# ducha-aiki/affnet

Hardware: AMD Instinct MI355X
Metric: keypoints/sec (detect+AffNet+OriNet+HardNet) per image, 2000 kp @1024x768 (higher is better)
Workload: dtype f32

## Files before the change

affnet_amd/SparseImgRepresenter.py:

```python
import ctypes as C

import torch
import torch.nn as nn

from . import _lib, engine
from ._lib import lib, check, ptr
from .architectures import _HipPatchNet
from .HandCraftedModules import AffineShapeEstimator, OrientationDetector, _HipHandCrafted
from .HardNet import HardTFeatNet
from .pytorch_sift import SIFTNet

_FOLLOW = (SIFTNet, HardTFeatNet)


class ScaleSpaceAffinePatchExtractor(nn.Module):
    def __init__(self, border=16, num_features=500, patch_size=32, mrSize=3.0, nlevels=3, num_Baum_iters=0,
                 init_sigma=1.6, th=None, RespNet=None, OriNet=None, AffNet=None, arith="fp32"):
        super(ScaleSpaceAffinePatchExtractor, self).__init__()
        self.arith = arith
        _lib.arith_code(arith)
        self.mrSize, self.PS, self.b = mrSize, patch_size, border
        self.num, self.nlevels = num_features, nlevels
        self.num_Baum_iters, self.init_sigma = num_Baum_iters, init_sigma
        self.th = th
        if th is not None:
            self.num = -1
        else:
            self.th = 0
        self.RespNet = RespNet
        if not 1 <= nlevels <= 6:
            raise NotImplementedError("nlevels must be 1..6 (levels per octave = nlevels + 2 <= 8)")
        self.OriNet = OriNet if OriNet is not None else OrientationDetector(patch_size=19)
        self.AffNet = AffNet if AffNet is not None else AffineShapeEstimator(patch_size=19)
        self.scale_pyr = self.sigmas = self.pix_dists = None
        self._ctx = None
        self._ctx_key = None
        self._fctx = self._fctx_key = self._pyr_ctx = None
        self.last_ids = None
        self.max_keep = 16384
        self.raw_div = 4
        self.lazy_shape_rows = -1
        self.shape_form = 1

        self.desc_form = 2

    def _context(self, x, allow_batch=False):
        engine.require_cuda(x, "image")
        if x.dim() != 4 or x.size(1) != 1 or x.size(0) < 1 or (x.size(0) != 1 and not allow_batch):
            raise ValueError("expected a (1,1,H,W) image; forward() is batch-size-1 like the reference "
                             "(HandCraftedModules.py:283-284) - use enqueue()/run_batch() for (B,1,H,W) batches")
        pre = int(1.5 * self.num) if self.num_Baum_iters > 0 else self.num
        key = (x.size(0), x.size(2), x.size(3), x.device, pre, self.num, float(self.th), self.mrSize, self.b, self.init_sigma,
               self.nlevels, self.max_keep, self.num_Baum_iters, self.raw_div, self.lazy_shape_rows)
        if self._ctx is not None and self._ctx_key == key and self._ctx.arith != _lib.arith_code(self.arith):
            self._ctx.set_arith(self.arith)
        if self._ctx is None or self._ctx_key != key:
            self._ctx = engine.Context(x.size(2), x.size(3), x.device, self.nlevels, self.init_sigma, self.b, self.mrSize,
                                       float(self.th), self.num, pre, self.max_keep, batch=x.size(0), baum_iters=self.num_Baum_iters, raw_div=self.raw_div,
                                       lazy_shape_rows=self.lazy_shape_rows, arith=self.arith)
            self._ctx_key = key
        if self._ctx.shape_form != int(self.shape_form):
            self._ctx.set_shape_form(self.shape_form)
        if self._ctx.desc_form != int(self.desc_form):
            self._ctx.set_desc_form(self.desc_form)
        return self._ctx

    def _publish_pyramid(self, ctx):
        self._pyr_ctx = ctx
        self.scale_pyr = ctx.pyramid_views()
        self.sigmas = [list(s) for s in ctx.plan.sigmas]
        self.pix_dists = [list(p) for p in ctx.plan.pix_dists]

    def _response_pyramid(self, ctx, img):
        dev = img.device
        st = engine.stream_of(dev)
        check(lib.affnet_pyramid_build(ctx.handle, ptr(img), st), ctx.handle, "affnet_pyramid_build")
        stride = lib.affnet_pyramid_image_stride(ctx.handle)
        base = lib.affnet_pyramid_level_offset(ctx.handle, 0, 0)
        resp = torch.zeros(ctx.batch * stride, dtype=torch.float32, device=dev)
        with torch.no_grad():
            for b in range(ctx.batch):
                pyr = ctx.pyramid_views(b)
                for o, (h, w) in enumerate(ctx.plan.sizes):
                    for l in range(ctx.plan.levels_per_octave):
                        off = b * stride + lib.affnet_pyramid_level_offset(ctx.handle, o, l) - base
                        r = self.RespNet(pyr[o][l], ctx.plan.sigmas[o][l])
                        resp[off:off + h * w].copy_(r.reshape(-1).to(dev, torch.float32))
        return resp

    @staticmethod
    def _native(slot):
        return slot is None or isinstance(slot, (_HipPatchNet, _HipHandCrafted))

    def enqueue(self, x, do_ori=False, desc=None, det_stream=None, input_ready=None):
        ctx = self._context(x, allow_batch=True)
        dev = x.device
        if not (self._native(self.AffNet) and self._native(self.OriNet)):
            raise NotImplementedError("the fused path needs the native AffNetFast / OriNetFast slots (foreign slots: forward())")
        img = x.contiguous().float()
        B, F = x.size(0), ctx.cap_final
        lafs = torch.empty(B, F, 2, 3, dtype=torch.float32, device=dev)
        resp = torch.empty(B, F, dtype=torch.float32, device=dev)
        ids = torch.empty(B, F, 3, dtype=torch.int32, device=dev)
        count = torch.zeros(B, dtype=torch.int32, device=dev)
        dsc = torch.empty(B, F, 128, dtype=torch.float32, device=dev) if desc is not None else None
        nets = self._nets(dev, do_ori, desc)
        follow = isinstance(desc, _FOLLOW)
        if isinstance(desc, HardTFeatNet):
            desc.check_usable()
        fused_dsc = None if follow else dsc
        if self.RespNet is not None:
            rmaps = self._response_pyramid(ctx, img)
            check(lib.affnet_detect_image_responses(ctx.handle, ptr(rmaps), engine.stream_of(dev)), ctx.handle, "affnet_detect_image_responses")
            rc = lib.affnet_describe_detected(ctx.handle, C.byref(nets), int(bool(do_ori)), ptr(lafs), ptr(resp), ptr(ids), ptr(fused_dsc),
                                              ptr(count), engine.stream_of(dev))
            check(rc, ctx.handle, "affnet_describe_detected")
        elif det_stream is None:
            rc = lib.affnet_extract_features(ctx.handle, C.byref(nets), ptr(img), int(bool(do_ori)), ptr(lafs), ptr(resp), ptr(ids),
                                             ptr(fused_dsc), ptr(count), engine.stream_of(dev))
            check(rc, ctx.handle, "affnet_extract_features")
        else:
            cur = torch.cuda.current_stream(dev)
            if input_ready is None:
                det_stream.wait_stream(cur)
            elif input_ready is not False:
                det_stream.wait_event(input_ready)
            if getattr(self, "_busy", None) is not None:
# ... 374 lines not shown
```

affnet_amd/_lib.py:

```python
import ctypes as C
import os

_HERE = os.path.dirname(os.path.abspath(__file__))
LIB_PATH = os.environ.get("AFFNET_HIP_LIB") or os.path.join(_HERE, "libaffnet_hip.so")
PROBES_LIB_PATH = os.path.join(_HERE, "libaffnet_hip_probes.so")

MAX_OCTAVES, MAX_LEVELS, MAX_TAPS = 16, 8, 37
NET_AFFNET, NET_ORINET, NET_HARDNET, NET_AFFNET_FULLCONV = 0, 1, 2, 3
ARITH_FP32_MFMA, ARITH_FP32_SPLIT3, ARITH_FP32_SPLIT2H = 0, 1, 2
ARITH_NAMES = {"fp32": ARITH_FP32_MFMA, "fp32_mfma": ARITH_FP32_MFMA, "fp32_split3": ARITH_FP32_SPLIT3, "split3": ARITH_FP32_SPLIT3,
               "fp32_split2h": ARITH_FP32_SPLIT2H, "split2h": ARITH_FP32_SPLIT2H}


def arith_code(arith):
    if arith is None:
        return ARITH_FP32_MFMA
    if isinstance(arith, str):
        if arith.lower() not in ARITH_NAMES:
            raise ValueError("arith must be one of %s" % sorted(ARITH_NAMES))
        return ARITH_NAMES[arith.lower()]
    if int(arith) not in (ARITH_FP32_MFMA, ARITH_FP32_SPLIT3, ARITH_FP32_SPLIT2H):
        raise ValueError("arith must be AFFNET_ARITH_FP32_MFMA (0), AFFNET_ARITH_FP32_SPLIT3 (1) or AFFNET_ARITH_FP32_SPLIT2H (2)")
    return int(arith)
SHAPE_FORM_DIRECT, SHAPE_FORM_WINOGRAD, SHAPE_FORM_POLYPHASE = 0, 1, 2
DESC_FORM_DIRECT, DESC_FORM_POLYPHASE, DESC_FORM_F43 = 0, 1, 2
OK, ERR_INVALID, ERR_HIP, ERR_CAPACITY, ERR_EMPTY = 0, -1, -2, -3, -4
VERIFY_AFFINE, VERIFY_HOMOGRAPHY, VERIFY_TILE, VERIFY_CHUNK = 0, 1, 128, 128
KNN_MAX_K = 8
IVF_MAX_PROBE = 8
EPI_MAX_ROUNDS, EPI_TILE, EPI_CHUNK, EPI_SOLVE_TILE = 64, 128, 128, 64
GUIDED_PLANAR, GUIDED_EPIPOLAR, GUIDED_MUTUAL = 0, 1, 1
VERIFY_FLAG_PAIR_RANGE = 8


class Config(C.Structure):
    _fields_ = [
        ("height", C.c_int32), ("width", C.c_int32), ("n_octaves", C.c_int32), ("levels_per_octave", C.c_int32),
        ("oct_h", C.c_int32 * MAX_OCTAVES), ("oct_w", C.c_int32 * MAX_OCTAVES),
        ("level_sigma", (C.c_float * MAX_LEVELS) * MAX_OCTAVES),
        ("level_sigma4", (C.c_float * MAX_LEVELS) * MAX_OCTAVES),
        ("level_sigma_px", (C.c_double * MAX_LEVELS) * MAX_OCTAVES),
        ("first_blur_taps", C.c_int32), ("first_blur", C.c_float * (MAX_TAPS * MAX_TAPS)),
        ("level_blur_taps", C.c_int32 * MAX_LEVELS),
        ("level_blur", (C.c_float * (MAX_TAPS * MAX_TAPS)) * MAX_LEVELS),
        ("level_blur0_taps", C.c_int32 * MAX_LEVELS),
        ("level_blur0", (C.c_float * (MAX_TAPS * MAX_TAPS)) * MAX_LEVELS),
        ("lazy_shape_rows", C.c_int32),
        ("onepass", C.c_int32),
        ("mr_size", C.c_float), ("threshold", C.c_float),
        ("num_features", C.c_int32), ("num_prefilter", C.c_int32),
        ("max_raw_per_octave_div", C.c_int32), ("max_keep", C.c_int32), ("batch", C.c_int32), ("baum_iters", C.c_int32),
        ("arith", C.c_int32),
    ]


class Nets(C.Structure):
    _fields_ = [("d_affnet", C.c_void_p), ("d_orinet", C.c_void_p), ("d_hardnet", C.c_void_p),
                ("h_orientation_window", C.c_void_p), ("h_baumberg_window", C.c_void_p)]


_P, _I, _SZ = C.c_void_p, C.c_int, C.c_size_t
SYMBOLS = {
    "affnet_config_fill": (_I, [C.POINTER(Config), _I, _I, _I, C.c_double, _I, C.c_double, C.c_double, _I, _I, _I, _I]),
    "affnet_ctx_create": (_I, [C.POINTER(_P), _I, C.POINTER(Config)]),
    "affnet_ctx_destroy": (None, [_P]),
    "affnet_last_error": (C.c_char_p, [_P]),
    "affnet_version": (C.c_char_p, []),
    "affnet_set_arith": (_I, [_P, _I]),
    "affnet_get_arith": (_I, [_P]),
    "affnet_set_shape_form": (_I, [_P, _I]),
    "affnet_get_shape_form": (_I, [_P]),
    "affnet_set_desc_form": (_I, [_P, _I]),
    "affnet_get_desc_form": (_I, [_P]),
    "affnet_workspace_bytes": (_SZ, [_P]),
    "affnet_bind_workspace": (_I, [_P, _P, _SZ]),
    "affnet_pyramid_level_offset": (C.c_int64, [_P, _I, _I]),
    "affnet_pyramid_image_stride": (C.c_int64, [_P]),
    "affnet_batch": (_I, [_P]),
    "affnet_capacity_prefilter": (_I, [_P]),
    "affnet_capacity_final": (_I, [_P]),
    "affnet_gauss_blur": (_I, [_P, _P, _P, _I, _I, C.POINTER(C.c_float), _I, _P]),
    "affnet_pyramid_build": (_I, [_P, _P, _P]),
    "affnet_hessian_response": (_I, [_P, _P, _P, _I, _I, C.c_float, _P]),
    "affnet_detect": (_I, [_P, _P, _P, _P, _P, _P]),
    "affnet_detect_responses": (_I, [_P, _P, _P, _P, _P, _P, _P]),
    "affnet_laf_grid_sample": (_I, [_P, _P, _I, _I, _P, _I, _I, _P, _P]),
    "affnet_pyr_grid_sample": (_I, [_P, _P, _P, _P, _I, _I, _P, _P]),
    "affnet_cnn32_packed_floats": (_SZ, [_I]),
    "affnet_cnn32_winograd_offset": (C.c_int64, [_I, _I]),
    "affnet_cnn32_pack_weights": (_I, [_I, C.POINTER(_P), C.POINTER(_P), C.POINTER(_P), _P, _P, _P, _P, _P]),
    "affnet_cnn32_forward": (_I, [_P, _I, _P, _P, _P, _I, _P, _P, _P]),
    "affnet_cnn32_forward_pyr": (_I, [_P, _I, _P, _P, _P, _P, _I, _P, _P, _P]),
    "affnet_local_norm": (_I, [_P, _P, _P, _I, _I, _P]),
    "affnet_fullconv_scratch_bytes": (_SZ, [_I, _I]),
    "affnet_fullconv_forward": (_I, [_P, _P, _P, _I, _I, _P, _P, _P]),
    "affnet_nms2d": (_I, [_P, _P, _P, _I, _I, C.c_float, _P]),
    "affnet_shape_filter_select": (_I, [_P, _P, _P, _P, _P, _P, _P, _P, _P, _P, _P]),
    "affnet_apply_rotation": (_I, [_P, _P, _P, _P, _I, _P]),
    "affnet_scale_lafs": (_I, [_P, _P, _P, _P, _I, _I, _I, _I, _P]),
    "affnet_lafs_to_ellipses": (_I, [_P, _P, _P, _I, _P, _P]),
    "affnet_ellipses_to_lafs": (_I, [_P, _P, _P, _I, _P, _P]),
    "affnet_level_select": (_I, [_P, _P, _P, _I, _I, _P, _P, _P]),
    "affnet_handcrafted_forward": (_I, [_P, _I, _P, _I, _P, _P, _P, _P]),
    "affnet_handcrafted_forward_pyr": (_I, [_P, _I, _P, _P, _P, _I, _P, _P, _P]),
    "affnet_sift_host_window": (_I, [_I, C.POINTER(C.c_float)]),
    "affnet_sift_forward": (_I, [_P, _P, _I, _P, C.c_float, _P, _P]),
    "affnet_sift_forward_pyr": (_I, [_P, _P, _P, _P, _I, _P, C.c_float, _P, _P]),
    "affnet_tfeat_packed_floats": (_SZ, []),
    "affnet_tfeat_pack_weights": (_I, [_P, _P, _P, _P, _P, _P, _P]),
    "affnet_tfeat_scratch_floats": (_SZ, [_I]),
    "affnet_tfeat_forward": (_I, [_P, _P, _P, _P, _I, _P, _P, _P]),
    "affnet_tfeat_forward_pyr": (_I, [_P, _P, _P, _P, _P, _I, _P, _P, _P]),
    "affnet_match_scratch_bytes": (_SZ, [_I, _I]),
    "affnet_distance_matrix": (_I, [_P, _P, _I, _P, _I, _I, _P, _P, _P]),
    "affnet_match_snn": (_I, [_P, _P, _I, _P, _I, _I, C.c_float, _P, _P, _P, _P, _P, _P, _P]),
    "affnet_reproject_lafs": (_I, [_P, _P, _I, C.POINTER(C.c_float), _P, _P]),
    "affnet_centre_nn": (_I, [_P, _P, _I, _P, _I, _P, _P, _P]),
    "affnet_verify_scratch_bytes": (_SZ, [_I]),
    "affnet_verify_score": (_I, [_P, _P, _I, _P, _I, _P, _P, _I, C.c_float, _P, _P, _P, _P]),
    "affnet_verify_matches": (_I, [_P, _P, _I, _P, _I, _P, _P, _I, C.c_float, _I, _I, _P, _P, _P, _P, _P, _P]),
    "affnet_match_many_scratch_bytes": (_SZ, [_I, _I, _I]),
    "affnet_match_snn_many": (_I, [_P, _P, _I, _P, _I, _I, _P, _I, _I, _I, C.c_float, _P, _P, _P, _P, _P, _P, _P]),
    "affnet_verify_many_scratch_bytes": (_SZ, [_I, _I]),
    "affnet_verify_matches_many": (_I, [_P, _P, _I, _P, _I, _P, _I, _P, _P, _I, C.c_float, _I, _I, _P, _P, _P, _P, _P, _P]),
    "affnet_epipolar_scratch_bytes": (_SZ, [_I, _I]),
    "affnet_epipolar_score": (_I, [_P, _P, _I, _P, _I, _P, _P, _I, C.c_float, _I, C.c_uint32, _P, _P, _P, _P, _P]),
    "affnet_epipolar_verify": (_I, [_P, _P, _I, _P, _I, _P, _P, _I, C.c_float, _I, C.c_uint32, _I, _P, _P, _P, _P, _P, _P]),
    "affnet_match_guided_scratch_bytes": (_SZ, [_I, _I, _I]),
    "affnet_match_guided": (_I, [_P, _P, _I, _P, _I, _I, _P, _P, _P, _I, C.c_float, C.c_float, C.c_float, _I, _I, _P, _P, _P, _P, _P, _P, _P]),
    "affnet_guided_mask": (_I, [_P, _P, _I, _P, _I, _P, _I, C.c_float, _P, _P, _P]),
    "affnet_knn_chunks": (_I, [_P, _I, _I]),
    "affnet_knn_scratch_bytes": (_SZ, [_I, _I, _I, _I]),
    "affnet_knn": (_I, [_P, _P, _I, _P, _I, _I, _I, _I, _I, _I, _P, _P, _P, _P]),
    "affnet_knn_vote": (_I, [_P, _P, _P, _I, _I, C.c_float, _P, _I, _I, _P, _P]),
    "affnet_quantize_desc": (_I, [_P, _P, _I, _I, C.c_float, _P, _P, _P]),
    "affnet_knn_q8_chunks": (_I, [_P, _I, _I]),
    "affnet_knn_q8_scratch_bytes": (_SZ, [_I, _I, _I, _I]),
    "affnet_knn_q8": (_I, [_P, _P, _P, _I, _P, _P, _I, _I, _I, _I, _I, _I, C.c_float, _P, _P, _P, _P, _P]),
    "affnet_ivf_sqnorm": (_I, [_P, _P, _I, _I, _P, _P]),
    "affnet_ivf_cell_means": (_I, [_P, _P, _I, _I, _P, _P, _I, _P, _P]),
    "affnet_ivf_scratch_bytes": (_SZ, [_I, _I, _I, _I]),
    "affnet_ivf_search": (_I, [_P, _P, _I, _P, _P, _P, _I, _P, _P, _I, _I, _I, _I, _I, _I, _P, _P, _P, _P, _P]),
    "affnet_ivf_q8_scratch_bytes": (_SZ, [_I, _I, _I, _I]),
    "affnet_ivf_search_q8": (_I, [_P, _P, _P, _P, _I, _P, _P, _P, _I, _P, _P, _I, _I, _I, _I, _I, _I, C.c_float, _P, _P, _P, _P, _P, _P]),
    "affnet_extract_features": (_I, [_P, C.POINTER(Nets), _P, _I, _P, _P, _P, _P, _P, _P]),
    "affnet_detect_image": (_I, [_P, _P, _P]),
    "affnet_detect_image_responses": (_I, [_P, _P, _P]),
    "affnet_detect_image_onepass": (_I, [_P, _P, _P, _P]),
    "affnet_detect_image_onepass_responses": (_I, [_P, _P, _P, _P]),
    "affnet_detected_list": (_I, [_P, _P, _P, _P, _P, _P]),
    "affnet_load_frames": (_I, [_P, _P, _I, _P, _P, _P, _I, _I, _P]),
    "affnet_describe_frames": (_I, [_P, C.POINTER(Nets), _P, _P, _P, _P, _I, _I, _P, _P, _P, _P, _P, _P]),
    "affnet_shape_iterate": (_I, [_P, _P, _P, _P, _P, _I, _P, _P]),
    "affnet_affmap_offset": (C.c_int64, [_P, _I]),
    "affnet_affmap_image_stride": (C.c_int64, [_P]),
    "affnet_describe_detected": (_I, [_P, C.POINTER(Nets), _I, _P, _P, _P, _P, _P, _P]),
    "affnet_graph_capture_extract": (_I, [_P, C.POINTER(Nets), _P, _I, _P, _P, _P, _P, _P, _P]),
    "affnet_graph_launch": (_I, [_P, _P]),
    "affnet_profile_enable": (_I, [_P, _I]),
    "affnet_profile_read": (_I, [_P, C.POINTER(C.c_double * 8), C.POINTER(C.c_int32)]),
    "affnet_read_counts": (_I, [_P, C.POINTER(C.c_int32 * 4), _P]),
    "affnet_counter_offset": (C.c_int64, [_P, _I]),
    "affnet_counter_stride": (C.c_int64, [_P]),
    "affnet_host_base_grid": (_I, [_I, C.POINTER(C.c_float)]),
}

DEBUG_SYMBOLS = {
    "affnet_cnn32_debug_timing": (_I, [_P, _P]),
    "affnet_cnn32_debug_layer": (_I, [_P, _I, _P, _P, _I, _P, _P]),
    "affnet_cnn32_debug_winograd_u": (_I, [_P, _I, _P, _I, _P, _P]),
    "affnet_selftest_mfma": (_I, [_P, _P, _P, _P]),
    "affnet_debug_split3_variant": (_I, [_P, _I]),
}

PROBE_SYMBOLS = {
    "affnet_cnn32_probe": (_I, [_P, _I, _I, _I, _I, _P, _P]),
    "affnet_split3_gemm": (_I, [_P, _P, _I, _I, _I, _I, _P, _P]),
    "affnet_split3_rate": (_I, [_I, _I, _I, _P, _P]),
    "affnet_debug_stream": (_I, [_P, _P, _SZ, _I, _I, _I, _P]),
    "affnet_probe_shape_offsets": (_I, [_P, C.POINTER(C.c_int64 * 3)]),
    "affnet_probe_affnet_wino_layer": (_I, [_P, _I, _P, _P, _I, _P, _P]),
    "affnet_probe_affnet_wino_partials": (_I, [_P, _P, _P, _I, _P, _P]),
    "affnet_probe_affnet_poly_layer": (_I, [_P, _I, _P, _P, _I, _P, _P]),
    "affnet_probe_affnet_poly_partials": (_I, [_P, _P, _P, _I, _P, _P]),
    "affnet_probe_trunk16_poly_u": (_I, [_P, _I, _P, _I, _P, _P]),
    "affnet_probe_hardnet_poly_layer": (_I, [_P, _P, _P, _I, _P, _P]),
    "affnet_probe_hardnet_poly_forward": (_I, [_P, _P, _P, _I, _P, _P, _P]),
    "affnet_probe_hardnet_poly_u": (_I, [_P, _P, _I, _P, _P]),
    "affnet_probe_hardnet_f43_layer": (_I, [_P, _P, _P, _I, _P, _P]),
    "affnet_probe_hardnet_f43_forward": (_I, [_P, _P, _P, _I, _P, _P, _P]),
    "affnet_probe_hardnet_f43_u": (_I, [_P, _P, _I, _P, _P]),
}


class AffnetHipError(RuntimeError):
    pass


class AffnetEmptyError(AffnetHipError):
    """AFFNET_ERR_EMPTY: no image of the call produced a detection (the reference raises in torch.cat([]),
    SparseImgRepresenter.py:100)."""


def _load():
    if not os.path.isfile(LIB_PATH):
        if os.path.basename(LIB_PATH) == os.path.basename(PROBES_LIB_PATH):
            raise ImportError("affnet_amd: %s is missing - the tools under tools/ need the probe build of the library: "
                              "AFFNET_PROBES=1 bash affnet_amd/csrc/build.sh" % LIB_PATH)
        raise ImportError(
            "affnet_amd: %s is missing - the HIP extension is the only implementation of this path "
            "(no CPU fallback). Build it: bash affnet_amd/csrc/build.sh" % LIB_PATH)
    lib = C.CDLL(LIB_PATH)
    for table in (SYMBOLS, DEBUG_SYMBOLS):
        for name, (res, args) in table.items():
            fn = getattr(lib, name)
            fn.restype, fn.argtypes = res, args
    for name, (res, args) in PROBE_SYMBOLS.items():
        if hasattr(lib, name):
            fn = getattr(lib, name)
            fn.restype, fn.argtypes = res, args
    return lib


lib = _load()


def check(rc, ctx=None, what=""):
    if rc != OK:
        msg = lib.affnet_last_error(ctx).decode() if ctx else ""
        if rc == ERR_EMPTY:
            raise AffnetEmptyError("%s: %s" % (what or "libaffnet_hip call", msg))
        raise AffnetHipError("%s failed (code %d): %s" % (what or "libaffnet_hip call", rc, msg))


def ptr(t):
    return None if t is None else C.c_void_p(t.data_ptr())


def current_stream(device):
    import torch
    return C.c_void_p(torch.cuda.current_stream(device).cuda_stream)
```

affnet_amd/csrc/cnn32.hip:

```cpp
#include "common.h"

static void aff_fill_pyr_src(const affnet_ctx* ctx, PyrSrc* s) {
    memset(s, 0, sizeof(*s));
    if (ctx->ws) aff_fill_pyr_table(ctx, &s->t);
    aff_base_grid(32, s->base);
}

static int cnn_check(affnet_ctx* ctx, const CnnCall& c, int* rows) {
    *rows = 0;
    if (c.kind < 0 || c.kind > 2) return aff_fail(ctx, AFFNET_ERR_INVALID, "cnn32: unknown net kind %d", c.kind);
    if (!c.packed || !c.out || c.n_max < 0 || (!c.patches && (!c.lafs || !c.ids))) return aff_fail(ctx, AFFNET_ERR_INVALID, "cnn32: null argument");
    if (!c.patches && !ctx->ws) return aff_fail(ctx, AFFNET_ERR_INVALID, "cnn32: sampling from the pyramid needs a bound workspace");
    if (c.dbg_layer < 0 && !c.scratch)
        return aff_fail(ctx, AFFNET_ERR_INVALID, "cnn32: d_scratch is required (HardNet n*(8192+512) floats, AffNet / OriNet n*144 floats)");
    if (c.dbg_layer >= 0 && ctx->arith != AFFNET_ARITH_FP32_MFMA)
        return aff_fail(ctx, AFFNET_ERR_INVALID, "cnn32: layer dumps exist for AFFNET_ARITH_FP32_MFMA only (context is in arithmetic mode %d)", ctx->arith);
    if (c.n_max == 0) return AFFNET_OK;
    if (c.kind == AFFNET_NET_HARDNET && c.n_max > 65535)
        return aff_fail(ctx, AFFNET_ERR_INVALID, "cnn32: n_max=%d (HardNet head: max 65535 rows per image)", c.n_max);
    const int row_count = c.row_count < 0 ? c.n_max - c.row_begin : c.row_count;
    if (c.row_begin < 0 || row_count < 0 || c.row_begin + row_count > c.n_max) return aff_fail(ctx, AFFNET_ERR_INVALID, "cnn32: bad row window");
    *rows = row_count;
    return AFFNET_OK;
}

TrunkKernel aff_trunk_kernel(int kind, int form, bool stamps) {
    typedef TrunkKernel (*Unit)(int, bool);
    static_assert(AFFNET_NET_AFFNET == 0 && AFFNET_NET_ORINET == 1 && AFFNET_NET_HARDNET == 2 && TRUNK_EXACT == 0 && TRUNK_WINO == 1 && TRUNK_SPLIT2 == 2 && TRUNK_SPLIT3 == 3 &&
                  TRUNK_WINO_F43 == 4 && TRUNK_WINO_POLY == 5 && TRUNK_FORMS == 6, "order of the table");
    static const Unit unit[3][TRUNK_FORMS] = {{aff_trunk_affnet, aff_trunk_affnet, aff_trunk_affnet, aff_trunk_affnet, nullptr, aff_trunk_affnet_poly},
                                              {aff_trunk_orinet, nullptr, aff_trunk_orinet, aff_trunk_orinet, nullptr, nullptr},
                                              {aff_trunk_hardnet, aff_trunk_hardnet_poly, aff_trunk_hardnet, aff_trunk_hardnet, aff_trunk_hardnet_f43, nullptr}};
    if (kind < 0 || kind > 2 || form < 0 || form >= TRUNK_FORMS || !unit[kind][form]) return nullptr;
    return unit[kind][form](form, stamps);
}

int aff_trunk_launch(affnet_ctx* ctx, const CnnCall& c, const NetLayout& L, dim3 grid, int wino, const int32_t* reeval, int shape_op) {
    int form = TRUNK_EXACT;
    if (ctx->arith != AFFNET_ARITH_FP32_MFMA) form = ctx->arith == AFFNET_ARITH_FP32_SPLIT2H ? TRUNK_SPLIT2 : TRUNK_SPLIT3;
    else if (c.kind == AFFNET_NET_AFFNET && wino) form = wino == 2 ? TRUNK_WINO_POLY : TRUNK_WINO;
    else if (c.kind == AFFNET_NET_HARDNET && c.desc_form != AFFNET_DESC_FORM_DIRECT) form = c.desc_form == AFFNET_DESC_FORM_F43 ? TRUNK_WINO_F43 : TRUNK_WINO;
    const bool stamps = ctx->dbg_time || c.dbg_layer >= 0;
    const TrunkKernel kernel = aff_trunk_kernel(c.kind, form, stamps);
    if (!kernel) return aff_fail(ctx, AFFNET_ERR_INVALID, "cnn32: no trunk kernel of net %d in form %d is built", c.kind, form);
    CnnArgs a;
    a.packed = c.packed; a.off = to_offsets(L, ctx->arith);
    a.reeval = reeval;
    const int rc = aff_derive_u(ctx, c.kind, form, c.packed, L, c.st, &a.wino_u);
    if (rc) return rc;
    a.patches = c.patches; a.lafs = c.lafs; a.ids = c.ids; a.count = c.count; a.n_max = c.n_max;
    a.out = (c.dbg_layer < 0) ? c.scratch : c.out;
    a.dbg_layer = c.dbg_layer; a.dbg_out = c.dbg_out; a.dbg_time = ctx->dbg_time;
    a.row_begin = c.row_begin; a.skip_cnt = c.skip_cnt; a.skip_n = c.skip_n;
    a.shape_cnt = (c.fuse && shape_op) ? c.fuse->cnt : nullptr; a.shape_op = shape_op;
    a.s3_alt = ctx->split3_variant;
    PyrSrc ps;
    aff_fill_pyr_src(ctx, &ps);
    hipLaunchKernelGGL(kernel, grid, dim3(512), 0, c.st, a, ps);
    AFF_LAUNCH_CHECK(ctx);
    return AFFNET_OK;
}

static int cnn_launch(affnet_ctx* ctx, const CnnCall& c) {
    int rows;
    int rc = cnn_check(ctx, c, &rows);
    if (rc || rows == 0) return rc;
    const NetLayout L = net_layout(c.kind);
    const int B = c.patches ? 1 : ctx->B;
    const bool form1 = c.wino_reeval && c.kind == AFFNET_NET_AFFNET && c.fuse && c.dbg_layer < 0 && ctx->arith == AFFNET_ARITH_FP32_MFMA;
    rc = aff_trunk_launch(ctx, c, L, dim3(rows, B), form1 ? c.wino_reeval : 0, nullptr, c.shape_op);
    if (rc) return rc;
    if (form1) {
        int32_t* flags = reinterpret_cast<int32_t*>(c.scratch + (size_t)B * c.n_max * HEAD_PART_AFF);
        rc = aff_margin_affnet(ctx, c, L, rows, B, flags);
        if (rc) return rc;
        rc = aff_trunk_launch(ctx, c, L, dim3(rows, B), 0, flags, 0);
        if (rc) return rc;
    }
    if (c.dbg_layer < 0 && c.kind != AFFNET_NET_HARDNET) {
        rc = c.kind == AFFNET_NET_AFFNET ? aff_finish_affnet(ctx, c, L, rows, B) : aff_finish_orinet(ctx, c, L, rows, B);
        if (rc) return rc;
    }
    if (c.mark_head) aff_prof_mark(ctx, 7, c.st);
    if (c.dbg_layer < 0 && c.kind == AFFNET_NET_HARDNET) return aff_hardnet_head(ctx, c, L, B);
    return AFFNET_OK;
}

extern "C" int affnet_cnn32_forward(affnet_ctx* ctx, int net_kind, const float* d_packed, const float* d_patches, const int32_t* d_count,
                                    int n_max, float* d_out, float* d_scratch, void* stream) {
    AFF_DEVICE(ctx);
    if (!ctx || !d_patches) return aff_fail(ctx, AFFNET_ERR_INVALID, "cnn32_forward: null argument");
    CnnCall c;
    c.kind = net_kind; c.packed = d_packed; c.patches = d_patches; c.count = d_count; c.n_max = n_max; c.out = d_out; c.scratch = d_scratch; c.st = (hipStream_t)stream;
    return cnn_launch(ctx, c);
}

extern "C" int affnet_cnn32_forward_pyr(affnet_ctx* ctx, int net_kind, const float* d_packed, const float* d_lafs, const int32_t* d_ids,
                                        const int32_t* d_count, int n_max, float* d_out, float* d_scratch, void* stream) {
    AFF_DEVICE(ctx);
    if (!ctx) return AFFNET_ERR_INVALID;
    CnnCall c;
    c.kind = net_kind; c.packed = d_packed; c.lafs = d_lafs; c.ids = d_ids; c.count = d_count; c.n_max = n_max; c.out = d_out; c.scratch = d_scratch; c.st = (hipStream_t)stream;
    return cnn_launch(ctx, c);
}

int aff_affnet_filter_rows(affnet_ctx* ctx, const float* packed, const float* resp, const float* lafs, const int32_t* ids, const int32_t* count,
                           float* out, float* scratch, int row_begin, int row_count, bool lazy, int shape_op, hipStream_t st) {
    ShapeFuse sf;
    sf.resp = resp; sf.lafs = lafs; sf.key = ctx->st_key; sf.good = ctx->st_good; sf.cnt = ctx->cnt;
    CnnCall c;
    c.kind = AFFNET_NET_AFFNET; c.packed = packed; c.lafs = lafs; c.ids = ids; c.count = count; c.n_max = ctx->cap_pre; c.out = out; c.scratch = scratch; c.st = st;
    c.row_begin = row_begin; c.row_count = row_count;
    c.skip_cnt = lazy ? ctx->cnt : nullptr; c.skip_n = ctx->cfg.num_features;
    c.fuse = &sf; c.shape_op = shape_op;
    c.wino_reeval = ctx->shape_form;
    return cnn_launch(ctx, c);
}

int aff_orinet_rotate(affnet_ctx* ctx, const float* packed, float* lafs, const int32_t* ids, const int32_t* count, int n_max, float* out, float* scratch,
                      hipStream_t st, const DenormSel* denorm) {
    CnnCall c;
    c.kind = AFFNET_NET_ORINET; c.packed = packed; c.lafs = lafs; c.ids = ids; c.count = count; c.n_max = n_max; c.out = out; c.scratch = scratch; c.st = st;
    c.rot_lafs = lafs; c.denorm = denorm;
    return cnn_launch(ctx, c);
}

int aff_hardnet_forward_pyr_marked(affnet_ctx* ctx, const float* packed, const float* lafs, const int32_t* ids, const int32_t* count,
                                   int n_max, float* out, float* scratch, hipStream_t st) {
    CnnCall c;
    c.kind = AFFNET_NET_HARDNET; c.packed = packed; c.lafs = lafs; c.ids = ids; c.count = count; c.n_max = n_max; c.out = out; c.scratch = scratch; c.st = st;
    c.mark_head = true;
    c.desc_form = ctx->cfg.onepass ? AFFNET_DESC_FORM_DIRECT : ctx->desc_form;
    return cnn_launch(ctx, c);
}

int aff_hardnet_poly_patches(affnet_ctx* ctx, const float* packed, const float* patches, int n, float* out, float* scratch, int dbg_layer, hipStream_t st, int form) {
    if (ctx->arith != AFFNET_ARITH_FP32_MFMA) return aff_fail(ctx, AFFNET_ERR_INVALID, "hardnet_poly: AFFNET_ARITH_FP32_MFMA only");
    CnnCall c;
    c.kind = AFFNET_NET_HARDNET; c.packed = packed; c.patches = patches; c.n_max = n; c.out = out; c.scratch = scratch; c.st = st;
    c.dbg_layer = dbg_layer; c.dbg_out = dbg_layer >= 0 ? out : nullptr;
    c.desc_form = form;
    return cnn_launch(ctx, c);
}

extern "C" int affnet_debug_split3_variant(affnet_ctx* ctx, int bits) {
    if (!ctx) return AFFNET_ERR_INVALID;
    ctx->split3_variant = bits;
    return AFFNET_OK;
}

extern "C" int affnet_cnn32_debug_timing(affnet_ctx* ctx, unsigned long long* d_stamps) {
    if (!ctx) return AFFNET_ERR_INVALID;
    ctx->dbg_time = d_stamps;
    return AFFNET_OK;
}

extern "C" int affnet_cnn32_debug_layer(affnet_ctx* ctx, int net_kind, const float* d_packed, const float* d_patch, int layer, float* d_out,
                                        void* stream) {
    AFF_DEVICE(ctx);
    if (!ctx || !d_patch || !d_out || layer < 0 || layer > 5) return aff_fail(ctx, AFFNET_ERR_INVALID, "cnn32_debug_layer: bad argument");
    CnnCall c;
    c.kind = net_kind; c.packed = d_packed; c.patches = d_patch; c.n_max = 1; c.out = d_out; c.st = (hipStream_t)stream;
    c.dbg_layer = layer; c.dbg_out = d_out;
    return cnn_launch(ctx, c);
}

extern "C" int affnet_cnn32_debug_winograd_u(affnet_ctx* ctx, int net_kind, const float* d_packed, int layer, float* d_out, void* stream) {
    AFF_DEVICE(ctx);
    if (!ctx || !d_packed || !d_out || (net_kind != AFFNET_NET_AFFNET && net_kind != AFFNET_NET_ORINET) || (layer != 1 && layer != 3 && layer != 5))
        return aff_fail(ctx, AFFNET_ERR_INVALID, "cnn32_debug_winograd_u: AffNet / OriNet, layer 1, 3 or 5");
    const float* u;
    const int rc = aff_derive_u(ctx, net_kind, net_kind == AFFNET_NET_AFFNET ? TRUNK_WINO : TRUNK_EXACT, d_packed, net_layout(net_kind), (hipStream_t)stream, &u);
    if (rc) return rc;
    return aff_copy_async(ctx, d_out, u + Wino16::offset(layer), (size_t)Wino16::floats(layer) * sizeof(float), (hipStream_t)stream);
}
```

affnet_amd/csrc/cnn_mfma.h:

```cpp
#pragma once
#include <math.h>
#include <stdlib.h>

#include <utility>

#include "common.h"
#include "weights_layout.h"

typedef float f32x4 __attribute__((ext_vector_type(4)));

typedef __attribute__((address_space(3))) const f32x4 LdsF4;
__device__ __forceinline__ unsigned lds_byte_addr(const float* p) {
    return (unsigned)(size_t)(__attribute__((address_space(3))) const float*)p;
}
__device__ __forceinline__ f32x4 lds_read4(unsigned byte_addr) { return *(LdsF4*)(size_t)byte_addr; }

typedef unsigned u32x4 __attribute__((ext_vector_type(4)));
__device__ __forceinline__ __amdgpu_buffer_rsrc_t weight_rsrc(const float* base, int n_floats) {
    return __builtin_amdgcn_make_buffer_rsrc(const_cast<float*>(base), 0, n_floats * 4, 0x00020000);
}
__device__ __forceinline__ f32x4 buf_read4(__amdgpu_buffer_rsrc_t r, int lane_byte_off, int uniform_byte_off) {
    return __builtin_bit_cast(f32x4, __builtin_amdgcn_raw_buffer_load_b128(r, lane_byte_off, uniform_byte_off, 0));
}

// ... 1126 lines not shown
    }
    __syncthreads();
#pragma unroll
    for (int k = 0; k < 18; ++k) *reinterpret_cast<f32x4*>(&act[((p * F43_XI + 18 * h + k) * 64 + lane) * 4]) = V[k];
    __syncthreads();
    const unsigned v0 = lds_byte_addr(act) + (18 * h * 64 + lane) * 16;
#pragma unroll
    for (int k = 0; k < 18; ++k) V[k] = lds_read4(v0 + k * 1024);
    f32x4 acc[18];
#pragma unroll
    for (int k = 0; k < 18; ++k) acc[k] = (f32x4){0.f, 0.f, 0.f, 0.f};
#pragma unroll 1
    for (int G = 0; G < NGRP; ++G) {
        const int Gn = G == NGRP - 1 ? G : G + 1;
        unsigned vb = v0 + Gn * F43_XI * 1024;
        asm("" : "+v"(vb));
        __builtin_amdgcn_sched_barrier(0);
#pragma unroll
        for (int k = 0; k < 18; k += 2) {
#pragma unroll
            for (int s4 = 0; s4 < 4; ++s4) {
                acc[k] = __builtin_amdgcn_mfma_f32_16x16x4f32(U[k][s4], V[k][s4], acc[k], 0, 0, 0);
                acc[k + 1] = __builtin_amdgcn_mfma_f32_16x16x4f32(U[k + 1][s4], V[k + 1][s4], acc[k + 1], 0, 0, 0);
            }
            U[k] = wino_load_u<CIN, COUT>(wrsrc, u_lane, k, Gn);
            U[k + 1] = wino_load_u<CIN, COUT>(wrsrc, u_lane, k + 1, Gn);
            V[k] = lds_read4(vb + k * 1024);
            V[k + 1] = lds_read4(vb + (k + 1) * 1024);
            __builtin_amdgcn_sched_barrier(0);
        }
    }
#pragma unroll
    for (int il = 0; il < 3; ++il)
#pragma unroll
        for (int e = 0; e < 4; ++e) {
            float yc[4];
            f43_at_axis(acc[6 * il][e], acc[6 * il + 1][e], acc[6 * il + 2][e], acc[6 * il + 3][e], acc[6 * il + 4][e], acc[6 * il + 5][e], yc[0], yc[1], yc[2], yc[3]);
#pragma unroll
            for (int c = 0; c < 4; ++c) t[il][c][e] = yc[c];
        }
}

__device__ __forceinline__ void f43_combine(float* lds, const f32x4 (&t)[3][4], f32x4 (&y)[8], int wave, int lane) {
    const int h = wave & 1;
    float* xw = lds + F43L::X + (wave * 8 * 64 + lane) * 4;
    const float* xr = lds + F43L::X + ((wave ^ 1) * 8 * 64 + lane) * 4;
    f32x4 k0[4], k1[4];
    if (h == 0) {
#pragma unroll
        for (int c = 0; c < 4; ++c) {
            const f32x4 p = t[1][c] + t[2][c], q = t[1][c] - t[2][c];
            k0[c] = t[0][c] + p; k1[c] = q;
            *reinterpret_cast<f32x4*>(&xw[c * 256]) = p;
            *reinterpret_cast<f32x4*>(&xw[(4 + c) * 256]) = q;
        }
    } else {
#pragma unroll
        for (int c = 0; c < 4; ++c) {
            const f32x4 r = t[0][c] + t[1][c], s = t[0][c] - t[1][c];
            k0[c] = 4.0f * r; k1[c] = 8.0f * s + t[2][c];
            *reinterpret_cast<f32x4*>(&xw[c * 256]) = r;
            *reinterpret_cast<f32x4*>(&xw[(4 + c) * 256]) = 2.0f * s;
        }
    }
    __syncthreads();
#pragma unroll
    for (int c = 0; c < 4; ++c) {
        const f32x4 o0 = *reinterpret_cast<const f32x4*>(&xr[c * 256]), o1 = *reinterpret_cast<const f32x4*>(&xr[(4 + c) * 256]);
        y[c] = k0[c] + o0;
        y[4 + c] = k1[c] + o1;
    }
}

template <typename LO>
__device__ __forceinline__ void f43_store_lds(float* act, f32x4 bias, const f32x4 (&y)[8], int wave, int lane) {
    const int m = lane & 15, oy = 4 * (m >> 2) + 2 * (wave & 1), ox = 4 * (m & 3);
#pragma unroll
    for (int k = 0; k < 8; ++k) {
        const f32x4 v = bias_relu(y[k], bias);
        *reinterpret_cast<f32x4*>(&act[((wave >> 1) * 4 + (lane >> 4)) * LO::PSG + ((oy + (k >> 2) + 1) * LO::WP + ox + (k & 3) + 1) * 4]) = v;
    }
}

template <int NW, int CIN, int COUT, int H, int NB>
__device__ __forceinline__ void wino_prefetch_u_row(const float* __restrict__ Wu, f32x4 (&U)[4], int wave, int lane) {
    const __amdgpu_buffer_rsrc_t r = weight_rsrc(Wu, 16 * CIN * COUT);
    const int u_lane = wino_u_lane<H, COUT, NB>(wave, 0, lane);
#pragma unroll
    for (int k = 0; k < 4; ++k) U[k] = wino_load_u<CIN, COUT>(r, u_lane, k, 0);
}

template <int NW, int CIN, int COUT, typename LI, int NB>
__device__ __forceinline__ void conv3x3_wino_mfma_rows(const float* act, const float* __restrict__ Wu, f32x4 (&U)[4], f32x4 (&y)[NB][4], int wave, int lane) {
    constexpr int H = LI::H, HT = H / 2, NGRP = CIN / 16, NSTEP = NB * 4 * NGRP;
    static_assert(H % 2 == 0 && (HT * HT) % 16 == 0 && COUT % 16 == 0 && CIN % 16 == 0, "Winograd tiling");
    static_assert((HT * HT / 16) * (COUT / 16) == NW * NB, "the waves' passes must tile the layer exactly");
    const int m = lane & 15, kq = lane >> 4;
    const __amdgpu_buffer_rsrc_t wrsrc = weight_rsrc(Wu, 16 * CIN * COUT);
    f32x4 t0[4], t1[4], acc[4];
#pragma unroll
    for (int s = 0; s < NSTEP; ++s) {
        const int q = s / (4 * NGRP), i = (s / NGRP) % 4, G = s % NGRP;
        const int sn = s + 1 < NSTEP ? s + 1 : s;
        const int qn = sn / (4 * NGRP), in = (sn / NGRP) % 4, Gn = sn % NGRP;
        int ty, tx, cb;
        wino_tile<H, COUT, NB>(wave, q, m, ty, tx, cb);
        const int u_next = wino_u_lane<H, COUT, NB>(wave, qn, lane);
        unsigned ab = lds_byte_addr(act) + (((4 * G + kq) * LI::PSG + (2 * ty * LI::WP + 2 * tx) * 4) * 4);
        asm("" : "+v"(ab));
        f32x4 da[4], db[4], V[4];
        wino_read_rows<LI>(ab, i, da, db);
        wino_transform_row(i, da, db, V);
        if (G == 0) {
#pragma unroll
            for (int k = 0; k < 4; ++k) acc[k] = (f32x4){0.f, 0.f, 0.f, 0.f};
        }
        __builtin_amdgcn_sched_barrier(0);
#pragma unroll
        for (int k = 0; k < 4; k += 2) {
#pragma unroll
            for (int s4 = 0; s4 < 4; ++s4) {
                acc[k] = __builtin_amdgcn_mfma_f32_16x16x4f32(U[k][s4], V[k][s4], acc[k], 0, 0, 0);
                acc[k + 1] = __builtin_amdgcn_mfma_f32_16x16x4f32(U[k + 1][s4], V[k + 1][s4], acc[k + 1], 0, 0, 0);
            }
            U[k] = wino_load_u<CIN, COUT>(wrsrc, u_next, 4 * in + k, Gn);
            U[k + 1] = wino_load_u<CIN, COUT>(wrsrc, u_next, 4 * in + k + 1, Gn);
            __builtin_amdgcn_sched_barrier(0);
        }
        if (G == NGRP - 1) {
#pragma unroll
            for (int j = 0; j < 4; ++j)
#pragma unroll
                for (int e = 0; e < 4; ++e) {
                    if (i == 0) t0[j][e] = acc[j][e];
                    else if (i == 1) { t0[j][e] = wadd(t0[j][e], acc[j][e]); t1[j][e] = acc[j][e]; }
                    else if (i == 2) { t0[j][e] = wadd(t0[j][e], acc[j][e]); t1[j][e] = wsub(t1[j][e], acc[j][e]); }
                    else t1[j][e] = wsub(t1[j][e], acc[j][e]);
                }
            if (i == 3) {
#pragma unroll
                for (int e = 0; e < 4; ++e) {
                    y[q][0][e] = wadd(wadd(t0[0][e], t0[1][e]), t0[2][e]);
                    y[q][1][e] = wsub(wsub(t0[1][e], t0[2][e]), t0[3][e]);
                    y[q][2][e] = wadd(wadd(t1[0][e], t1[1][e]), t1[2][e]);
                    y[q][3][e] = wsub(wsub(t1[1][e], t1[2][e]), t1[3][e]);
                }
            }
        }
    }
}

struct Wino5 {
    static constexpr int X = 16 * LayC4::PSG, X_FLOATS = 8 * 4 * 256;
    static constexpr int HEAD = 0;
    static constexpr int U_HALF = 8 * 4 * 16 * 64 * 4;
};
__device__ __forceinline__ void wino5_prefetch_u(const float* __restrict__ Wu, f32x4 (&U)[4], int wave, int lane) {
    const __amdgpu_buffer_rsrc_t r = weight_rsrc(Wu, 16 * 64 * 64);
    const int u_lane = ((lane >> 4) * 64 + (wave >> 1) * 16 + (lane & 15)) * 16 + (wave & 1) * Wino5::U_HALF;
#pragma unroll
    for (int k = 0; k < 4; ++k) U[k] = wino_load_u<64, 64>(r, u_lane, k, 0);
}

template <int NW, typename LI>
__device__ __forceinline__ void conv3x3_wino_mfma_half_rows(const float* act, const float* __restrict__ Wu, f32x4 (&U)[4], f32x4 (&acc)[2][4], int wave, int lane) {
    constexpr int CIN = 64, COUT = 64, NGRP = CIN / 16, NSTEP = 2 * NGRP;
// ... 36 lines not shown
}

__device__ __forceinline__ void wino5_combine(float* lds, const f32x4 (&acc)[2][4], f32x4 (&y)[2], int wave, int lane) {
    const int h = wave & 1;
    float* xw = lds + Wino5::X + (wave * 4 * 64 + lane) * 4;
    const float* xr = lds + Wino5::X + ((wave ^ 1) * 4 * 64 + lane) * 4;
    if (h == 0) {
#pragma unroll
        for (int j = 0; j < 4; ++j) *reinterpret_cast<f32x4*>(&xw[j * 256]) = acc[1][j];
    } else {
#pragma unroll
        for (int j = 0; j < 4; ++j) *reinterpret_cast<f32x4*>(&xw[j * 256]) = acc[0][j];
    }
    __syncthreads();
    f32x4 o[4], t[4];
#pragma unroll
    for (int j = 0; j < 4; ++j) o[j] = *reinterpret_cast<const f32x4*>(&xr[j * 256]);
    if (h == 0) {
#pragma unroll
        for (int j = 0; j < 4; ++j)
#pragma unroll
            for (int e = 0; e < 4; ++e) t[j][e] = wadd(wadd(acc[0][j][e], acc[1][j][e]), o[j][e]);
    } else {
#pragma unroll
        for (int j = 0; j < 4; ++j)
#pragma unroll
            for (int e = 0; e < 4; ++e) t[j][e] = wsub(wsub(o[j][e], acc[0][j][e]), acc[1][j][e]);
    }
#pragma unroll
    for (int e = 0; e < 4; ++e) {
        y[0][e] = wadd(wadd(t[0][e], t[1][e]), t[2][e]);
        y[1][e] = wsub(wsub(t[1][e], t[2][e]), t[3][e]);
    }
}

template <int ROW, int PIX, int GRP>
__device__ __forceinline__ void wino5_store_lds(float* dst, f32x4 bias, const f32x4 (&y)[2], int wave, int lane) {
    const int m = lane & 15, oy = 2 * (m >> 2) + (wave & 1), ox = 2 * (m & 3);
#pragma unroll
    for (int k = 0; k < 2; ++k) {
        const f32x4 v = bias_relu(y[k], bias);
        *reinterpret_cast<f32x4*>(&dst[(oy * ROW + ox + k) * PIX + ((wave >> 1) * 4 + (lane >> 4)) * GRP]) = v;
    }
}

template <int NW, int H, int COUT, int NB>
__device__ __forceinline__ void wino_bias(const float* __restrict__ bias, f32x4 (&bv)[NB], int wave, int lane) {
#pragma unroll
    for (int q = 0; q < NB; ++q) {
        int ty, tx, cb;
        wino_tile<H, COUT, NB>(wave, q, lane & 15, ty, tx, cb);
        bv[q] = *reinterpret_cast<const f32x4*>(&bias[cb * 16 + 4 * (lane >> 4)]);
    }
}

template <int COUT, typename LO, int NB>
__device__ __forceinline__ void wino_store_lds(float* act, const f32x4 (&bias)[NB], const f32x4 (&y)[NB][4], int wave, int lane) {
    const int g = lane >> 4;
#pragma unroll
    for (int q = 0; q < NB; ++q) {
        int ty, tx, cb;
        wino_tile<LO::H, COUT, NB>(wave, q, lane & 15, ty, tx, cb);
#pragma unroll
        for (int k = 0; k < 4; ++k) {
            const int oy = 2 * ty + (k >> 1), ox = 2 * tx + (k & 1);
            const f32x4 v = bias_relu(y[q][k], bias[q]);
            *reinterpret_cast<f32x4*>(&act[(cb * 4 + g) * LO::PSG + ((oy + 1) * LO::WP + ox + 1) * 4]) = v;
        }
    }
}

template <int COUT, int H, int NB>
__device__ __forceinline__ void wino_store_global(float* __restrict__ dst, const f32x4 (&bias)[NB], const f32x4 (&y)[NB][4], int wave, int lane) {
    const int g = lane >> 4;
#pragma unroll
    for (int q = 0; q < NB; ++q) {
        int ty, tx, cb;
        wino_tile<H, COUT, NB>(wave, q, lane & 15, ty, tx, cb);
#pragma unroll
        for (int k = 0; k < 4; ++k) {
            const int p = (2 * ty + (k >> 1)) * H + 2 * tx + (k & 1);
            const f32x4 v = bias_relu(y[q][k], bias[q]);
            *reinterpret_cast<f32x4*>(dst + p * COUT + cb * 16 + 4 * g) = v;
        }
    }
}

constexpr int poly_row_np(int r) { return (r < 3 || (r >= 6 && r < 8)) ? 3 : 2; }
constexpr int poly_row_xi0(int r) { return r < 3 ? 3 * r : (r < 6 ? 9 + 2 * (r - 3) : (r < 8 ? 15 + 3 * (r - 6) : 21 + 2 * (r - 8))); }
constexpr bool poly_row_oddy(int r) { return r < 6; }
constexpr int poly_row_yi(int r) { return r < 3 ? r : (r < 6 ? r - 3 : (r < 8 ? r - 6 : r - 8)); }
constexpr int poly_row_ra(int r) { return poly_row_oddy(r) ? (poly_row_yi(r) == 0 ? 0 : 2) : 1 + 2 * poly_row_yi(r); }
constexpr int poly_row_rb(int r) { return (poly_row_oddy(r) && poly_row_yi(r) != 1) ? (poly_row_yi(r) == 0 ? 2 : 4) : -1; }
constexpr int poly_row_reads(int r) { return poly_row_np(r) * (poly_row_rb(r) >= 0 ? 2 : 1); }
constexpr int poly_row_valu(int r) { return 4 * ((poly_row_rb(r) >= 0 ? poly_row_np(r) : 0) + (poly_row_np(r) == 3 ? 2 : 0)); }

template <int... I, typename F>
__device__ __forceinline__ void static_for_seq(std::integer_sequence<int, I...>, F&& f) { (f(IntC<I>{}), ...); }
template <int N, typename F>
__device__ __forceinline__ void static_for(F&& f) { static_for_seq(std::make_integer_sequence<int, N>{}, f); }

template <typename LI, int R>
__device__ __forceinline__ void poly_read_row(unsigned ab, f32x4 (&da)[3], f32x4 (&db)[3]) {
    constexpr int NC = poly_row_np(R), C0 = NC == 3 ? 0 : 1, RA = poly_row_ra(R), RB = poly_row_rb(R);
#pragma unroll
    for (int c = 0; c < NC; ++c) {
        da[c] = lds_read4(ab + (RA * LI::WP + C0 + 2 * c) * 16);
        if constexpr (RB >= 0) db[c] = lds_read4(ab + (RB * LI::WP + C0 + 2 * c) * 16);
    }
}

template <int R>
__device__ __forceinline__ void poly_transform_row(const f32x4 (&da)[3], const f32x4 (&db)[3], f32x4 (&V)[3]) {
    constexpr int NC = poly_row_np(R), RB = poly_row_rb(R);
#pragma unroll
    for (int e = 0; e < 4; ++e) {
        float t[3];
#pragma unroll
        for (int c = 0; c < NC; ++c) t[c] = RB >= 0 ? wsub(da[c][e], db[c][e]) : da[c][e];
        if constexpr (NC == 3) { V[0][e] = wsub(t[0], t[1]); V[1][e] = t[1]; V[2][e] = wsub(t[1], t[2]); }
        else { V[0][e] = t[0]; V[1][e] = t[1]; }
    }
}

template <int NW, int CIN, int COUT, int HOUT, int NB, int NCB>
__device__ __forceinline__ void poly_prefetch_u(const float* __restrict__ Wu, f32x4 (&Ua)[NCB][3], f32x4 (&Ub)[NCB][3], int wave, int lane) {
    constexpr int NGRP = CIN / 16;
    const __amdgpu_buffer_rsrc_t r = weight_rsrc(Wu, POLY_XI * CIN * COUT);
    const int u_lane = wino_u_lane<HOUT, COUT, NB>(wave, 0, lane);
    constexpr int R1 = 1 / NGRP, G1 = 1 % NGRP;
#pragma unroll
    for (int k = 0; k < 3; ++k)
#pragma unroll
        for (int c = 0; c < NCB; ++c) {
            Ua[c][k] = wino_load_u<CIN, COUT>(r, u_lane, k, 0, c);
            if (k < poly_row_np(R1)) Ub[c][k] = wino_load_u<CIN, COUT>(r, u_lane, poly_row_xi0(R1) + k, G1, c);
        }
}

template <int NW, int CIN, int COUT, typename LI, int NB, int NCB>
__device__ __forceinline__ void conv3x3_poly_mfma_rows(const float* act, const float* __restrict__ Wu, f32x4 (&Ua)[NCB][3], f32x4 (&Ub)[NCB][3], f32x4 (&y)[NB][4],
                                                       int wave, int lane) {
    constexpr int HOUT = LI::H / 2, HT = HOUT / 2, NGRP = CIN / 16, NSTEP = (NB / NCB) * 10 * NGRP;
    static_assert(LI::H % 4 == 0 && (HT * HT) % 16 == 0 && COUT % 16 == 0 && CIN % 16 == 0, "polyphase tiling");
    static_assert((HT * HT / 16) * (COUT / 16) == NW * NB, "the waves' passes must tile the layer exactly");
    static_assert((NCB == 1 || NCB == 2) && NB % NCB == 0 && (COUT / 16) % NCB == 0 && NSTEP % 2 == 0, "the passes of a unit must share their tile block");
    const int m = lane & 15, kq = lane >> 4;
    const __amdgpu_buffer_rsrc_t wrsrc = weight_rsrc(Wu, POLY_XI * CIN * COUT);
    f32x4 t0[NCB][5], t1[NCB][5], acc[NCB][3], Va[3], Vb[3];
    auto window_addr = [&](int u, int G) {
        int ty, tx, cb;
        wino_tile<HOUT, COUT, NB>(wave, NCB * u, m, ty, tx, cb);
        unsigned ab = lds_byte_addr(act) + (((4 * G + kq) * LI::PSG + (4 * ty * LI::WP + 4 * tx) * 4) * 4);
        asm("" : "+v"(ab));
        return ab;
    };
    auto step = [&](auto sc, const f32x4 (&V)[3], f32x4 (&Vn)[3], f32x4 (&U)[NCB][3]) {
        constexpr int S = decltype(sc)::v;
        constexpr int u = S / (10 * NGRP), R = (S / NGRP) % 10, G = S % NGRP;
        constexpr bool more = S + 1 < NSTEP;
        constexpr int Sn = more ? S + 1 : S, un = Sn / (10 * NGRP), Rn = (Sn / NGRP) % 10, Gn = Sn % NGRP;
        constexpr int S2 = S + 2 < NSTEP ? S + 2 : S, u2 = S2 / (10 * NGRP), R2 = (S2 / NGRP) % 10, G2 = S2 % NGRP;
        constexpr int NP = poly_row_np(R), NP2 = poly_row_np(R2), XI2 = poly_row_xi0(R2);
        constexpr int NM = NP * 4 * NCB, NRn = more ? poly_row_reads(Rn) : 0, VPM = NCB == 2 ? 2 : 4, NVM = more ? (poly_row_valu(Rn) + VPM - 1) / VPM : 0;
        static_assert(NM >= NRn + NVM, "the next step's reads and transform fit between this step's MFMAs");
        const int u_next = wino_u_lane<HOUT, COUT, NB>(wave, NCB * u2, lane);
// ... 181 lines not shown
```

affnet_amd/csrc/cnn_trunk.h:

```cpp
#pragma once
#include <math.h>

#include <type_traits>

#include "common.h"

#include "cnn_mfma.h"

template <int TM>
__device__ __forceinline__ void head_partials(const float* __restrict__ hw, const f32x4 (&bias)[1], const f32x4 (&acc)[TM][1],
                                              float* __restrict__ part, int wave, int lane) {
    constexpr int MT = 4, MG = MT / TM;
    const int mg = wave % MG, ng = wave / MG;
    const int n = lane & 15, g = lane >> 4;
    const int c4 = ng * 16 + 4 * g;
    f32x4 v[TM];
#pragma unroll
    for (int i = 0; i < TM; ++i) v[i] = bias_relu(acc[i][0], bias[0]);
    const __amdgpu_buffer_rsrc_t r = weight_rsrc(hw, 3 * 4096);
    f32x4 w[3][TM];
#pragma unroll
    for (int o = 0; o < 3; ++o)
#pragma unroll
        for (int i = 0; i < TM; ++i) w[o][i] = buf_read4(r, (n * 64 + c4) * 4, (o * 4096 + (mg * TM + i) * 16 * 64) * 4);
// ... 62 lines not shown
    }
}
template <int TM>
__device__ __forceinline__ void ori_head_pbase(const OriHeadLane& L, int (&pbase)[TM]) {
#pragma unroll
    for (int i = 0; i < TM; ++i) {
        const int p = (L.mg * TM + i) * 16 + L.n;
        pbase[i] = ((p >> 3) * 10 + (p & 7)) * ORI_HP + L.c4;
    }
}
template <int TM>
__device__ __forceinline__ void ori_head_reduce(const f32x4 (&w)[2][TM], const int (&pbase)[TM], float* __restrict__ part, const float* act, int wave, int lane) {
    __syncthreads();
#pragma unroll
    for (int q = 0; q < 9; ++q) {
        float s0 = 0.f, s1 = 0.f;
#pragma unroll
        for (int i = 0; i < TM; ++i) {
            const f32x4 av = *reinterpret_cast<const f32x4*>(&act[pbase[i] + ((q / 3) * 10 + q % 3) * ORI_HP]);
#pragma unroll
            for (int j = 0; j < 4; ++j) { s0 = fmaf(av[j], w[0][i][j], s0); s1 = fmaf(av[j], w[1][i][j], s1); }
        }
        s0 = wave_sum(s0);
        s1 = wave_sum(s1);
        if (lane == 0) { part[wave * 18 + q] = s0; part[wave * 18 + 9 + q] = s1; }
    }
}
template <int TM, int NTHR>
__device__ __forceinline__ void head_partials_ori_lds(const float* __restrict__ hw, const f32x4 (&bias)[1], const f32x4 (&acc)[TM][1],
                                                      float* __restrict__ part, float* act, int wave, int lane, int tid) {
    constexpr int MT = 4, MG = MT / TM;
    const int mg = wave % MG, ng = wave / MG;
    const int n = lane & 15, g = lane >> 4;
    const int c4 = ng * 16 + 4 * g;
    f32x4 v[TM];
#pragma unroll
    for (int i = 0; i < TM; ++i) v[i] = bias_relu(acc[i][0], bias[0]);
    const __amdgpu_buffer_rsrc_t r = weight_rsrc(hw, 2 * 4096);
    f32x4 w[2][TM];
#pragma unroll
    for (int o = 0; o < 2; ++o)
#pragma unroll
        for (int i = 0; i < TM; ++i) w[o][i] = buf_read4(r, (n * 64 + c4) * 4, (o * 4096 + (mg * TM + i) * 16 * 64) * 4);
    __syncthreads();
    ori_head_zero_halo<NTHR>(act, tid);
    int pbase[TM];
#pragma unroll
    for (int i = 0; i < TM; ++i) {
        const int p = (mg * TM + i) * 16 + n;
        pbase[i] = ((p >> 3) * 10 + (p & 7)) * ORI_HP + c4;
        *reinterpret_cast<f32x4*>(&act[pbase[i] + 11 * ORI_HP]) = v[i];
    }
    ori_head_reduce<TM>(w, pbase, part, act, wave, lane);
}

#define CNN_STAMP(k)                                                                                     \
    do {                                                                                                 \
        if (STAMPS && a.dbg_time && lane == 0) a.dbg_time[((size_t)pidx * NW + wave) * 32 + (k)] = __builtin_readcyclecounter(); \
    } while (0)

template <int CB>
struct TrunkLds {
    static constexpr int ACT = (CB / 4) * LayC0::PSG;
    static constexpr int PATCH = WP32 * WP32;
    static constexpr int RED = 256;
    static constexpr int TOTAL = ACT + PATCH + RED;
};

template <int KIND, int NW>
struct TrunkShape {
    static constexpr int CB = (KIND == AFFNET_NET_HARDNET) ? 32 : 16;
    static constexpr int NTHR = NW * 64;
    static constexpr int T1M = (CB == 16) ? 8 : 64 / NW, T1N = CB / 16;
    static constexpr int T2M = (CB == 16) ? 4 : 64 / NW, T2N = 1;
    static constexpr int T4M = (CB == 16) ? 2 : 32 / NW, T4N = 1;
    static constexpr int AREG = (NW == 8 && CB == 32) ? 128 : 48;
    static constexpr int G2 = pick_groups(CB, T2M, T2N, 32, AREG), G3 = pick_groups(2 * CB, T2M, T2N, 32, AREG);
    static constexpr int G4 = pick_groups(2 * CB, T4M, T4N, 32, AREG), G5 = pick_groups(4 * CB, T4M, T4N, 32, AREG);
};

template <int KIND, int S3>
struct TrunkTraits {
    static_assert(S3 == TRUNK_EXACT || S3 == TRUNK_SPLIT2 || S3 == TRUNK_SPLIT3 || (S3 == TRUNK_WINO && KIND != AFFNET_NET_ORINET) ||
                  (S3 == TRUNK_WINO_F43 && KIND == AFFNET_NET_HARDNET) || (S3 == TRUNK_WINO_POLY && KIND == AFFNET_NET_AFFNET), "no such trunk form of this net (common.h: TRUNK_*)");
    static constexpr bool EXACT = S3 != TRUNK_SPLIT2 && S3 != TRUNK_SPLIT3;
    static constexpr bool WINO13 = (S3 == TRUNK_EXACT && KIND == AFFNET_NET_ORINET) || ((S3 == TRUNK_WINO || S3 == TRUNK_WINO_POLY) && KIND == AFFNET_NET_AFFNET);
    static constexpr bool POLY16 = (S3 == TRUNK_EXACT && KIND == AFFNET_NET_ORINET) || (S3 == TRUNK_WINO_POLY && KIND == AFFNET_NET_AFFNET);
    static constexpr bool POLY = (S3 == TRUNK_WINO || S3 == TRUNK_WINO_F43) && KIND == AFFNET_NET_HARDNET, F43_3 = S3 == TRUNK_WINO_F43 && KIND == AFFNET_NET_HARDNET;
};

template <int C, typename L, int NTHR>
__device__ __forceinline__ void dump_planes(const float* act, float* dst) {
    constexpr int H = L::H;
    for (int i = threadIdx.x; i < C * H * H; i += NTHR) {
        const int c = i / (H * H), r = i - c * H * H, y = r / H, x = r - y * H;
        dst[i] = act[L::at(c, y, x)];
    }
}

template <int CB>
struct SplitLays {
    typedef LayQ<16, 32, 34, CB, 0, 3> LQH;
    typedef LayQ<16, 32, 34, CB, 16, 3> LQH2;
    using LR0 = LayR<32, 32, 34, CB, 0>;
    using LR0H = LayR<16, 32, 34, CB, 0, 34>;
    using LR1 = LayR<32, 32, 34, CB, 16>;
    using LR1H = LayR<16, 32, 34, CB, 16, 34>;
    static_assert(LR0::BYTES <= TrunkLds<CB>::ACT * 4 && LR1::BYTES <= TrunkLds<CB>::ACT * 4 && LR0H::GS == LR0::GS && LR1H::GS == LR1::GS, "whole-patch split layouts");
    static_assert(LQH::BYTES <= TrunkLds<CB>::ACT * 4 && LQH2::BYTES <= TrunkLds<CB>::ACT * 4, "pre-split layouts must fit the activation buffer");
};

template <int KIND, int NW, bool STAMPS, int S3 = 0>
__global__ __launch_bounds__(NW * 64, (KIND == AFFNET_NET_HARDNET) ? NW / 4 : 4) void cnn32_trunk_kernel(CnnArgs a, PyrSrc ps) {
    using F = TrunkTraits<KIND, S3>;
    constexpr bool EXACT = F::EXACT, WINO13 = F::WINO13, POLY16 = F::POLY16, POLY = F::POLY, F43_3 = F::F43_3;
    using S = TrunkShape<KIND, NW>;
    constexpr int CB = S::CB, NTHR = S::NTHR;
    static_assert((CB / 4) * LayC1::PSG <= TrunkLds<CB>::ACT && (CB / 2) * LayC3::PSG <= TrunkLds<CB>::ACT, "LDS layout");
    __shared__ __attribute__((aligned(16))) float lds[TrunkLds<CB>::TOTAL];
    float* act = lds;
    float* patch = lds + TrunkLds<CB>::ACT;
    float* red = patch + TrunkLds<CB>::PATCH;
    const int n = a.count ? min(a.count[blockIdx.y], a.n_max) : a.n_max;
    const int prow = blockIdx.x + a.row_begin;
    if (KIND == AFFNET_NET_AFFNET && a.shape_cnt && blockIdx.x == 0 && threadIdx.x == 0) {
        int32_t* c = a.shape_cnt + (size_t)blockIdx.y * CNT_TOTAL;
        if (a.shape_op == 1) { c[CNT_SURVIVED] = 0; c[CNT_SURVIVED1] = 0; c[CNT_AFF_EVAL] = 0; c[CNT_AFF_REEVAL] = 0; }
        else if (a.shape_op == 2) c[CNT_SURVIVED1] = c[CNT_SURVIVED];
    }
    if (prow >= n || lazy_skip(a.skip_cnt, a.skip_n, blockIdx.y, CNT_SURVIVED)) return;
    const size_t pidx = (size_t)blockIdx.y * a.n_max + prow;
    if (KIND == AFFNET_NET_AFFNET && a.reeval && a.reeval[pidx] == 0) return;
    const int tid = threadIdx.x, wave = tid >> 6, lane = tid & 63;
    if (KIND == AFFNET_NET_HARDNET) __builtin_amdgcn_s_setprio(3);
    CNN_STAMP(0);
    if (STAMPS && a.dbg_time && lane == 0) {
        a.dbg_time[((size_t)pidx * NW + wave) * 32 + 14] = __builtin_amdgcn_s_getreg((31 << 11) | 4);
        a.dbg_time[((size_t)pidx * NW + wave) * 32 + 15] = __builtin_amdgcn_s_getreg((31 << 11) | 20);
    }
    float w0[3][S::T1N];
    f32x4 bias0[S::T1N];
    conv0_load_w<NW, CB, S::T1M, S::T1N>(a.packed + a.off.w[0], a.packed + a.off.b[0], w0, bias0, wave, lane);
    f32x4 b1[1][S::T1N];
    f32x4 Ur[4];
    if constexpr (S3 == TRUNK_EXACT && KIND == AFFNET_NET_AFFNET) prefetch_b0<NW, CB, 32, S::T1M, S::T1N, 1>(a.packed + a.off.w[1], b1, wave, lane);
    if constexpr (WINO13) wino_prefetch_u_row<NW, CB, CB, 32, Wino16::NB1>(a.wino_u, Ur, wave, lane);

    constexpr int PPT = 1024 / NTHR;
    constexpr int RPT = 32 / PPT;
    float v[PPT];
    if (a.patches) {
        const float* src = a.patches + pidx * 1024;
#pragma unroll
        for (int q = 0; q < PPT; ++q) v[q] = src[tid + q * NTHR];
    } else {
        int o = a.ids[3 * pidx], l = a.ids[3 * pidx + 1];
        o = o < 0 ? 0 : (o >= ps.t.n_octaves ? ps.t.n_octaves - 1 : o);
        l = l < 0 ? 0 : (l >= ps.t.n_levels ? ps.t.n_levels - 1 : l);
        const float* img = ps.t.lvl[o][l] + blockIdx.y * ps.t.img_stride;
        const int h = ps.t.h[o], w = ps.t.w[o];
        const float* L = a.lafs + 6 * pidx;
        const float m = (float)(h < w ? h : w);
        const float t00 = L[0] * m, t01 = L[1] * m, t02 = L[2] * (float)w;
        const float t10 = L[3] * m, t11 = L[4] * m, t12 = L[5] * (float)h;
#pragma unroll
        for (int q = 0; q < PPT; ++q)
            v[q] = aff_sample_bilinear(img, h, w, t00, t01, t02, t10, t11, t12, ps.base[tid & 31], ps.base[(tid >> 5) + q * RPT]);
    }
    CNN_STAMP(16);
    if (tid < 4 * 33) {
        const int e = tid;
        const int y = e < 34 ? 0 : (e < 68 ? 33 : 1 + ((e - 68) >> 1)), x = e < 34 ? e : (e < 68 ? e - 34 : ((e - 68) & 1) * 33);
        patch[y * WP32 + x] = 0.0f;
    }
    if constexpr (EXACT) zero_halo<LayC0, NTHR>(act, CB);
    else if constexpr (S3 == TRUNK_SPLIT2) zero_halo_q<typename SplitLays<CB>::LR0, NTHR>(act);
    else zero_halo_q<typename SplitLays<CB>::LQH, NTHR>(act);
    float sum = 0.f;
#pragma unroll
    for (int q = 0; q < PPT; ++q) sum += v[q];
    const float mean = block_sum<NW>(sum, red) * (1.0f / 1024.0f);
    CNN_STAMP(17);
    float sq = 0.f;
#pragma unroll
    for (int q = 0; q < PPT; ++q) { v[q] -= mean; sq += v[q] * v[q]; }
    const float var = block_sum<NW>(sq, red + NW) * (1.0f / 1023.0f);
    const float sd = sqrtf(var) + 1e-7f;
    CNN_STAMP(18);
#pragma unroll
    for (int q = 0; q < PPT; ++q) patch[((tid >> 5) + q * RPT + 1) * WP32 + (tid & 31) + 1] = v[q] / sd;
    __syncthreads();
    CNN_STAMP(1);

    if constexpr (EXACT && KIND == AFFNET_NET_HARDNET) {
        constexpr int T1M = S::T1M, T1N = S::T1N, T2M = S::T2M, T2N = S::T2N, T4M = S::T4M, T4N = S::T4N;
        constexpr int NB1 = (16 * 16 / 16) * (CB / 16) / NW, NB3 = (8 * 8 / 16) * (2 * CB / 16) / NW, NB5 = (4 * 4 / 16) * (4 * CB / 16) / NW;
        constexpr int NBP2 = (8 * 8 / 16) * (2 * CB / 16) / NW, NBP4 = (4 * 4 / 16) * (4 * CB / 16) / NW;

// ... 32 lines not shown
            zero_halo<LayC1, NTHR>(act, CB);
            wino_store_lds<CB, LayC1, NB1>(act, bw, y, wave, lane);
            CNN_STAMP(22);
            __syncthreads();
            CNN_STAMP(4);
        }
        if (STAMPS && a.dbg_layer == 1) { dump_planes<CB, LayC1, NTHR>(act, a.dbg_out); return; }

        if constexpr (POLY) {
            f32x4 y[NBP2][4], bw[NBP2];
            __builtin_amdgcn_s_setprio(0);
            conv3x3_poly_mfma_rows<NW, CB, 2 * CB, LayC1, NBP2, 2>(act, a.wino_u + Poly32::offset(2), P2a, P2b, y, wave, lane);
            __builtin_amdgcn_s_setprio(3);
            CNN_STAMP(5);
            if constexpr (F43_3) f43_prefetch_u<2 * CB, 2 * CB>(a.wino_u + F43::BASE + F43::offset(3), Uf, wave, lane);
            else wino_prefetch_u_pair<NW, 2 * CB, 2 * CB, 16, NB3>(a.packed + a.off.w_wino[1], Up, wave, lane);
            wino_bias<NW, 16, 2 * CB, NBP2>(a.packed + a.off.b[2], bw, wave, lane);
            __syncthreads();
            zero_halo<LayC2, NTHR>(act, 2 * CB);
            wino_store_lds<2 * CB, LayC2, NBP2>(act, bw, y, wave, lane);
            __syncthreads();
            CNN_STAMP(6);
        } else {
            f32x4 acc[T2M][T2N];
            __builtin_amdgcn_s_setprio(0);
            conv3x3_mfma<NW, CB, 2 * CB, LayC1, 2, T2M, T2N, S::G2>(act, a.packed + a.off.w[2], b2, acc, wave, lane);
            __builtin_amdgcn_s_setprio(3);
            CNN_STAMP(5);
            wino_prefetch_u_pair<NW, 2 * CB, 2 * CB, 16, NB3>(a.packed + a.off.w_wino[1], Up, wave, lane);
            __syncthreads();
            zero_halo<LayC2, NTHR>(act, 2 * CB);
            store_tiles_lds<2 * CB, LayC2, T2M, T2N>(act, bias2, acc, wave, lane);
            __syncthreads();
            CNN_STAMP(6);
        }
        if (STAMPS && a.dbg_layer == 2) { dump_planes<2 * CB, LayC2, NTHR>(act, a.dbg_out); return; }

        f32x4 b4[S::G4][T4N];
        f32x4 bias4[T4N];
        f32x4 P4a[1][3], P4b[1][3];
        if constexpr (F43_3) {
            static_assert(F43L::V_FLOATS <= TrunkLds<CB>::ACT && F43L::X + F43L::X_FLOATS <= F43L::V_FLOATS, "conv3: V of the layer fits the activation buffer");
            f32x4 tf[3][4], y[8];
            __builtin_amdgcn_s_setprio(0);
            conv3x3_f43_mfma_shared_v<NW, 2 * CB, 2 * CB, LayC2>(act, a.wino_u + F43::BASE + F43::offset(3), Uf, tf, wave, lane);
            __builtin_amdgcn_s_setprio(3);
            CNN_STAMP(23);
            poly_prefetch_u<NW, 2 * CB, 4 * CB, 8, NBP4, 1>(a.wino_u + Poly32::offset(4), P4a, P4b, wave, lane);
            const f32x4 bf = *reinterpret_cast<const f32x4*>(&a.packed[a.off.b[3] + (wave >> 1) * 16 + 4 * (lane >> 4)]);
            __syncthreads();
            f43_combine(act, tf, y, wave, lane);
            CNN_STAMP(7);
            __syncthreads();
            zero_halo<LayC3, NTHR>(act, 2 * CB);
            f43_store_lds<LayC3>(act, bf, y, wave, lane);
            __syncthreads();
            CNN_STAMP(8);
        } else {
            f32x4 y[NB3][4], bw[NB3];
            __builtin_amdgcn_s_setprio(0);
            conv3x3_wino_mfma_pair_rows<NW, 2 * CB, 2 * CB, LayC2, NB3>(act, a.packed + a.off.w_wino[1], Up, y, wave, lane);
            __builtin_amdgcn_s_setprio(3);
            CNN_STAMP(7);
            if constexpr (POLY) poly_prefetch_u<NW, 2 * CB, 4 * CB, 8, NBP4, 1>(a.wino_u + Poly32::offset(4), P4a, P4b, wave, lane);
            else {
                prefetch_b0<NW, 4 * CB, 8, T4M, T4N, S::G4>(a.packed + a.off.w[4], b4, wave, lane);
                prefetch_bias<NW, 8, T4M, T4N>(a.packed + a.off.b[4], bias4, wave, lane);
            }
            wino_bias<NW, 16, 2 * CB, NB3>(a.packed + a.off.b[3], bw, wave, lane);
            __syncthreads();
            zero_halo<LayC3, NTHR>(act, 2 * CB);
            wino_store_lds<2 * CB, LayC3, NB3>(act, bw, y, wave, lane);
            __syncthreads();
            CNN_STAMP(8);
        }
        if (STAMPS && a.dbg_layer == 3) { dump_planes<2 * CB, LayC3, NTHR>(act, a.dbg_out); return; }

        if constexpr (POLY) {
            f32x4 y[NBP4][4], bw[NBP4];
            __builtin_amdgcn_s_setprio(0);
            conv3x3_poly_mfma_rows<NW, 2 * CB, 4 * CB, LayC3, NBP4, 1>(act, a.wino_u + Poly32::offset(4), P4a, P4b, y, wave, lane);
            __builtin_amdgcn_s_setprio(3);
            CNN_STAMP(9);
            wino_prefetch_u<NW, 4 * CB, 4 * CB, 8, NB5>(a.packed + a.off.w_wino[2], Uw, wave, lane);
            wino_bias<NW, 8, 4 * CB, NBP4>(a.packed + a.off.b[4], bw, wave, lane);
            __syncthreads();
            zero_halo<LayC4, NTHR>(act, 4 * CB);
            wino_store_lds<4 * CB, LayC4, NBP4>(act, bw, y, wave, lane);
            __syncthreads();
            CNN_STAMP(10);
        } else {
            f32x4 acc[T4M][T4N];
            __builtin_amdgcn_s_setprio(0);
            conv3x3_mfma<NW, 2 * CB, 4 * CB, LayC3, 2, T4M, T4N, S::G4>(act, a.packed + a.off.w[4], b4, acc, wave, lane);
            __builtin_amdgcn_s_setprio(3);
            CNN_STAMP(9);
            wino_prefetch_u<NW, 4 * CB, 4 * CB, 8, NB5>(a.packed + a.off.w_wino[2], Uw, wave, lane);
            __syncthreads();
            zero_halo<LayC4, NTHR>(act, 4 * CB);
            store_tiles_lds<4 * CB, LayC4, T4M, T4N>(act, bias4, acc, wave, lane);
            __syncthreads();
            CNN_STAMP(10);
        }
        if (STAMPS && a.dbg_layer == 4) { dump_planes<4 * CB, LayC4, NTHR>(act, a.dbg_out); return; }

        f32x4 y[NB5][4], bw[NB5];
        __builtin_amdgcn_s_setprio(0);
        static_assert(NB5 == 1 && (4 * CB / 16) * 4096 <= TrunkLds<CB>::ACT, "conv5: one pass per wave, V of the layer fits the activation buffer");
        conv3x3_wino_mfma_shared_v<NW, 4 * CB, 4 * CB, LayC4>(act, a.packed + a.off.w_wino[2], Uw, y, wave, lane);
        __builtin_amdgcn_s_setprio(3);
        CNN_STAMP(11);
        wino_bias<NW, 8, 4 * CB, NB5>(a.packed + a.off.b[5], bw, wave, lane);
        if (!STAMPS || a.dbg_layer < 0) {
            wino_store_global<4 * CB, 8, NB5>(a.out + pidx * (64 * 4 * CB), bw, y, wave, lane);
            CNN_STAMP(13);
            return;
        }
        __syncthreads();
        wino_store_lds<4 * CB, LayC5, NB5>(act, bw, y, wave, lane);
        __syncthreads();
        CNN_STAMP(12);
        if (STAMPS && a.dbg_layer == 5) { dump_planes<4 * CB, LayC5, NTHR>(act, a.dbg_out); return; }
    } else if constexpr (EXACT) {
        constexpr int T1M = S::T1M, T1N = S::T1N, T2M = S::T2M, T2N = S::T2N, T4M = S::T4M, T4N = S::T4N;
        static_assert(NW == 8 && CB == 16, "Wino16 describes the 16-channel trunks on 8 waves");
        constexpr int NB1 = Wino16::NB1, NB3 = Wino16::NB3;
        static_assert(WINO13 || T1M * 8 > S::AREG, "conv1: two A sets of T1M float4 do not fit -> rolling single set (conv3x3_mfma_roll)");
        f32x4 b4[S::G4][T4N];
        f32x4 bias4[T4N];
        f32x4 bias1[T1N];
        f32x4 b3[S::G3][T2N];
        f32x4 bias3[T2N];
        f32x4 Upa[3], Upb[3];
        static_assert(!POLY16 || WINO13, "the polyphase stride-2 layers sit between the Winograd stride-1 layers");
        {
            f32x4 acc[T1M][T1N];
            conv0_mfma<NW, CB, T1M, T1N>(patch, w0, bias0, acc, wave, lane);
            CNN_STAMP(19);
            if constexpr (!WINO13) prefetch_bias<NW, 32, T1M, T1N>(a.packed + a.off.b[1], bias1, wave, lane);
            store_tiles_lds<CB, LayC0, T1M, T1N, false>(act, bias0, acc, wave, lane);
            CNN_STAMP(20);
            __syncthreads();
        }
        if (STAMPS && a.dbg_layer == 0) { dump_planes<CB, LayC0, NTHR>(act, a.dbg_out); return; }
        CNN_STAMP(2);

        f32x4 b2[S::G2][T2N];
        f32x4 bias2[T2N];
        if constexpr (WINO13) {
            f32x4 y[NB1][4], bw[NB1];
            conv3x3_wino_mfma_rows<NW, CB, CB, LayC0, NB1>(act, a.wino_u, Ur, y, wave, lane);
            CNN_STAMP(3);
            if constexpr (POLY16) poly16_prefetch_u<CB, 2 * CB>(a.wino_u + Wino16::offset(2), Upa, Upb, wave & 1, 0, lane);
            else {
                prefetch_b0<NW, 2 * CB, 16, T2M, T2N, S::G2>(a.packed + a.off.w[2], b2, wave, lane);
                prefetch_bias<NW, 16, T2M, T2N>(a.packed + a.off.b[2], bias2, wave, lane);
            }
            wino_bias<NW, 32, CB, NB1>(a.packed + a.off.b[1], bw, wave, lane);
            __syncthreads();
            CNN_STAMP(21);
            zero_halo<LayC1, NTHR>(act, CB);
            wino_store_lds<CB, LayC1, NB1>(act, bw, y, wave, lane);
            CNN_STAMP(22);
            __syncthreads();
            CNN_STAMP(4);
        } else {
            f32x4 acc[T1M][T1N];
            conv3x3_mfma_roll<NW, CB, CB, LayC0, 1, T1M, T1N>(act, a.packed + a.off.w[1], b1, acc, wave, lane);
            CNN_STAMP(3);
            prefetch_b0<NW, 2 * CB, 16, T2M, T2N, S::G2>(a.packed + a.off.w[2], b2, wave, lane);
            prefetch_bias<NW, 16, T2M, T2N>(a.packed + a.off.b[2], bias2, wave, lane);
            __syncthreads();
            CNN_STAMP(21);
            zero_halo<LayC1, NTHR>(act, CB);
            store_tiles_lds<CB, LayC1, T1M, T1N>(act, bias1, acc, wave, lane);
            CNN_STAMP(22);
            __syncthreads();
            CNN_STAMP(4);
        }
        if (STAMPS && a.dbg_layer == 1) { dump_planes<CB, LayC1, NTHR>(act, a.dbg_out); return; }

        if constexpr (POLY16) {
            f32x4 y[1][4], bw[1];
            int ty, tx, cb;
            wino_tile<16, 2 * CB, 1>(wave, 0, lane & 15, ty, tx, cb);
            static_assert((16 / 2) * (16 / 2) / 16 * (2 * CB / 16) == NW, "conv2: one unit per wave");
            conv3x3_poly16_mfma_rows<CB, 2 * CB, LayC1>(act, a.wino_u + Wino16::offset(2), Upa, Upb, y[0], ty, tx, cb, 0, lane);
            CNN_STAMP(5);
            wino_prefetch_u_row<NW, 2 * CB, 2 * CB, 16, NB3>(a.wino_u + Wino16::offset(3), Ur, wave, lane);
            wino_bias<NW, 16, 2 * CB, 1>(a.packed + a.off.b[2], bw, wave, lane);
            __syncthreads();
            zero_halo<LayC2, NTHR>(act, 2 * CB);
            wino_store_lds<2 * CB, LayC2, 1>(act, bw, y, wave, lane);
            __syncthreads();
            CNN_STAMP(6);
        } else {
            f32x4 acc[T2M][T2N];
            conv3x3_mfma<NW, CB, 2 * CB, LayC1, 2, T2M, T2N, S::G2>(act, a.packed + a.off.w[2], b2, acc, wave, lane);
            CNN_STAMP(5);
            if constexpr (WINO13) wino_prefetch_u_row<NW, 2 * CB, 2 * CB, 16, NB3>(a.wino_u + Wino16::offset(3), Ur, wave, lane);
            else {
                prefetch_b0<NW, 2 * CB, 16, T2M, T2N, S::G3>(a.packed + a.off.w[3], b3, wave, lane);
                prefetch_bias<NW, 16, T2M, T2N>(a.packed + a.off.b[3], bias3, wave, lane);
            }
            __syncthreads();
// ... 389 lines not shown
```

affnet_amd/csrc/common.h:

```cpp
#pragma once
#include <hip/hip_runtime.h>
#include <stdint.h>
#include <stdio.h>
#include <string.h>

#include <string>
#include <type_traits>
#include <vector>

#include "../../include/affnet_hip.h"
#include "../../include/affnet_hip_debug.h"
#include "weights_layout.h"

#define AFF_WAVE 64

enum {
    CNT_RAW0 = 0,
    CNT_CAND = AFFNET_MAX_OCTAVES,
    CNT_OVERFLOW,
    CNT_SEL,
    CNT_EQ_TAKEN,
    CNT_SEL_MODE,
    CNT_SEL_THRESH,
    CNT_SEL_NEED_EQ,
    CNT_DET,
    CNT_SHAPED,
    CNT_SURVIVED,
    CNT_CAND2,
    CNT_AFF_EVAL,
    CNT_SURVIVED1,
    CNT_SEL_EQ_TOTAL,
    CNT_SEL_TIE_LO, CNT_SEL_TIE_HI,
    CNT_AFF_REEVAL,
    CNT_POS0 = AFFNET_MAX_OCTAVES + 24,
    CNT_HYP0 = AFFNET_MAX_OCTAVES + 24 + (AFFNET_MAX_LEVELS - 2) * AFFNET_MAX_OCTAVES,
    CNT_TOTAL = AFFNET_MAX_OCTAVES + 24 + (AFFNET_MAX_LEVELS - 2) * AFFNET_MAX_OCTAVES + 8 * AFFNET_MAX_OCTAVES
};

#define OVF_FRAMES_COUNT 16
#define OVF_FRAMES_NONFINITE 32

#define SEL_HIST_BINS 2048

struct RawMax {
    int32_t pix;
    int32_t lvl;
    float val;
    float s, y, x;
    float prev[2];
};

struct OctaveGeom {
    int32_t h, w;
    int64_t pyr_off;
    int64_t map_off;
    int64_t raw_off;
    int32_t raw_cap;
};

struct affnet_ctx {
    int device = 0;
    affnet_config cfg;
    int B = 1;
    size_t pyr_stride = 0;
    size_t map_stride = 0;
    size_t raw_stride = 0;
    std::string err;
    OctaveGeom oct[AFFNET_MAX_OCTAVES];
    size_t off_pyr = 0, off_map = 0, off_raw = 0, off_cnt = 0, off_hist = 0, off_cand = 0, off_sel = 0, off_stage = 0;
    size_t off_affmap = 0, off_dense = 0, off_cand2 = 0, off_lvltab = 0;
    size_t aff_stride = 0;
    size_t aff_off[AFFNET_MAX_OCTAVES] = {0};
    size_t dense_stride = 0;
    float* affmap = nullptr; float* dense = nullptr;
    float* cand2_resp = nullptr; float* cand2_syx = nullptr; int32_t* cand2_ids = nullptr;
    int32_t* lvltab = nullptr;
    size_t ws_bytes = 0;
    size_t pyr_floats = 0, map_bytes = 0, raw_total = 0, cand_cap = 0;
    int cap_pre = 0, cap_final = 0;
    char* ws = nullptr;
    float* pyr = nullptr;
    uint8_t* omap = nullptr;
    RawMax* raw = nullptr;
    int32_t* cnt = nullptr;
    uint32_t* sel_hist = nullptr;
    float* cand_resp = nullptr; float* cand_syx = nullptr; int32_t* cand_ids = nullptr;
    float* sel_resp = nullptr; float* sel_syx = nullptr; int32_t* sel_ids = nullptr;
    float* st_det_resp = nullptr; float* st_det_lafs = nullptr; int32_t* st_det_ids = nullptr;
    int32_t* st_det_count = nullptr;
    float* st_A = nullptr; float* st_key = nullptr; int32_t* st_good = nullptr;
    float* st_A2 = nullptr; float* st_lafs_iter = nullptr;
    float* st_R = nullptr; float* st_lafs_norm = nullptr; int32_t* st_lvl_ids = nullptr;
    float* st_hard_scratch = nullptr;
    float* st_lafs_shaped = nullptr;
    int32_t* st_rank = nullptr;
    bool prof_on = false;
    std::vector<hipEvent_t> prof_ev;
    int prof_calls = 0;
    unsigned long long* dbg_time = nullptr;
    int shape_form = AFFNET_SHAPE_FORM_WINOGRAD;
    int arith = AFFNET_ARITH_FP32_MFMA;
    int split3_variant = 0;
    hipGraph_t graph = nullptr;
    hipGraphExec_t graph_exec = nullptr;
    float* derived_u = nullptr;
    int desc_form = AFFNET_DESC_FORM_F43;
    ~affnet_ctx() {
        if (derived_u) (void)hipFree(derived_u);
        if (graph_exec) (void)hipGraphExecDestroy(graph_exec);
        if (graph) (void)hipGraphDestroy(graph);
        for (auto& e : prof_ev) (void)hipEventDestroy(e);
    }
};

struct AffDeviceGuard {
    int prev = -1;
    bool switched = false;
    explicit AffDeviceGuard(const affnet_ctx* ctx) {
        if (!ctx) return;
        if (hipGetDevice(&prev) != hipSuccess) { (void)hipGetLastError(); prev = -1; return; }
        if (prev != ctx->device) switched = hipSetDevice(ctx->device) == hipSuccess;
    }
    ~AffDeviceGuard() {
        if (switched) (void)hipSetDevice(prev);
    }
    AffDeviceGuard(const AffDeviceGuard&) = delete;
    AffDeviceGuard& operator=(const AffDeviceGuard&) = delete;
};
#define AFF_DEVICE(ctx) AffDeviceGuard aff_device_guard_(ctx)

#define PROF_RING 256
#define PROF_EVENTS (AFFNET_PROFILE_STAGES + 2)

#define AFF_HIP(ctx, expr)                                                                         \
    do {                                                                                           \
        hipError_t e_ = (expr);                                                                    \
        if (e_ != hipSuccess)                                                                      \
            return aff_fail(ctx, AFFNET_ERR_HIP, "%s failed: %s (%s:%d)", #expr, hipGetErrorString(e_), \
                            __FILE__, __LINE__);                                                   \
    } while (0)

#define AFF_LAUNCH_CHECK(ctx)                                                                      \
    do {                                                                                           \
        hipError_t e_ = hipGetLastError();                                                         \
        if (e_ != hipSuccess)                                                                      \
            return aff_fail(ctx, AFFNET_ERR_HIP, "kernel launch failed: %s (%s:%d)",                \
                            hipGetErrorString(e_), __FILE__, __LINE__);                            \
    } while (0)

struct AffZeroSegs {
    unsigned char* p[8];
    size_t bytes[8];
    int n = 0;
    bool overflow = false;
    void add(void* ptr, size_t nbytes) {
        if (!ptr || !nbytes) return;
        if (n >= 8) { overflow = true; return; }
        p[n] = (unsigned char*)ptr; bytes[n] = nbytes; ++n;
    }
};

static inline size_t aff_align(size_t x, size_t a = 256) { return (x + a - 1) / a * a; }
static inline int aff_cdiv(int a, int b) { return (a + b - 1) / b; }

struct AffPairRow { int row1, n1, row2, n2; };
__device__ __forceinline__ bool aff_pair_row(const int32_t* __restrict__ pairs, int p, int rows1, int rows2, int n1_max, int n2_max, AffPairRow& r) {
    r.row1 = pairs[4 * (size_t)p]; r.n1 = pairs[4 * (size_t)p + 1]; r.row2 = pairs[4 * (size_t)p + 2]; r.n2 = pairs[4 * (size_t)p + 3];
    return r.row1 >= 0 && r.n1 >= 0 && r.row2 >= 0 && r.n2 >= 0 && (long long)r.row1 + r.n1 <= rows1 && (long long)r.row2 + r.n2 <= rows2 &&
           r.n1 <= n1_max && r.n2 <= n2_max;
}

struct PyrTable {
    const float* lvl[AFFNET_MAX_OCTAVES][AFFNET_MAX_LEVELS];
    int h[AFFNET_MAX_OCTAVES], w[AFFNET_MAX_OCTAVES];
    int n_octaves, n_levels;
    size_t img_stride;
};

struct LevelTable { double sig[AFFNET_MAX_OCTAVES * AFFNET_MAX_LEVELS]; int n_oct, n_lvl; };
struct DenormSel {
    float* out_px; int32_t* ids; float* lafs_norm;
    float c_a, c_x, c_y, ps, ca, cx, cy;
    LevelTable lt;
};


#define HEAD_PART_AFF 32
#define HEAD_PART_ORI 144
#define HEAD_KSPLIT 4
#define HEAD_KC 128
#define HEAD_AS (HEAD_KC + 4)

struct PyrSrc {
    PyrTable t;
    float base[32];
};

struct CnnArgs {
    const float* packed;
    NetOffsets off;
    const float* wino_u;
    const int32_t* reeval;
    const float* patches;
    const float* lafs;
    const int32_t* ids;
    const int32_t* count;
    int n_max;
    float* out;
    int dbg_layer;
    int s3_alt;
    float* dbg_out;
    unsigned long long* dbg_time;
    int row_begin;
    const int32_t* skip_cnt;
    int skip_n;
    int32_t* shape_cnt;
    int shape_op;
};

constexpr int TRUNK_EXACT = 0;
constexpr int TRUNK_WINO = 1;
constexpr int TRUNK_SPLIT2 = 2;
constexpr int TRUNK_SPLIT3 = 3;
constexpr int TRUNK_WINO_F43 = 4;
constexpr int TRUNK_WINO_POLY = 5;
constexpr int TRUNK_FORMS = 6;

__device__ __forceinline__ bool lazy_skip(const int32_t* skip_cnt, int skip_n, int image, int which = CNT_SURVIVED1) {
    if (!skip_cnt) return false;
    const int32_t* c = skip_cnt + (size_t)image * CNT_TOTAL;
    return c[CNT_SEL_MODE] == 1 && c[which] >= skip_n;
}

struct ShapeFuse {
    const float* resp; const float* lafs; float* key; int32_t* good; int32_t* cnt;
};

struct CnnCall {
    int kind = -1;
    const float* packed = nullptr;
    const float* patches = nullptr;
    const float* lafs = nullptr; const int32_t* ids = nullptr;
    const int32_t* count = nullptr; int n_max = 0;
    float* out = nullptr; float* scratch = nullptr;
    hipStream_t st = nullptr;
    int dbg_layer = -1; float* dbg_out = nullptr;
    bool mark_head = false;
    int row_begin = 0, row_count = -1;
    const int32_t* skip_cnt = nullptr; int skip_n = 0;
    const ShapeFuse* fuse = nullptr; int shape_op = 0;
    int desc_form = AFFNET_DESC_FORM_DIRECT;
    int wino_reeval = 0;
    float* rot_lafs = nullptr; const DenormSel* denorm = nullptr;
};

typedef void (*TrunkKernel)(CnnArgs, PyrSrc);

int aff_fail(affnet_ctx* ctx, int code, const char* fmt, ...);
int aff_zero_async(affnet_ctx* ctx, void* dst, size_t bytes, hipStream_t st);
int aff_zero_multi_async(affnet_ctx* ctx, const AffZeroSegs& z, hipStream_t st);
int aff_copy_async(affnet_ctx* ctx, void* dst, const void* src, size_t bytes, hipStream_t st);
int aff_copy2d_async(affnet_ctx* ctx, void* dst, size_t dpitch, const void* src, size_t spitch, size_t width_bytes, size_t rows, hipStream_t st);
void aff_base_grid(int ps, float* base);

void aff_prof_mark(affnet_ctx* ctx, int idx, hipStream_t st);

int aff_detect_impl(affnet_ctx* ctx, const float* d_responses, float* d_resp, float* d_lafs, int32_t* d_ids, int32_t* d_count, void* stream);
int aff_detect_onepass_impl(affnet_ctx* ctx, const float* d_packed_fullconv, const float* d_responses, hipStream_t st);

int aff_fullconv_launch(affnet_ctx* ctx, const float* packed, const float* img, size_t img_stride, int h, int w, float* out, size_t out_stride,
                        float* scratch, size_t scratch_stride, int B, hipStream_t st);

int aff_handcrafted_launch(affnet_ctx* ctx, int kind, const float* patches, const float* lafs, const int32_t* ids, const int32_t* count,
                           int n_max, const float* h_weights, float* out, float* out_angle, hipStream_t st);

void aff_fill_pyr_table(const affnet_ctx* ctx, PyrTable* t);
int aff_shape_select(affnet_ctx* ctx, const float* d_resp_in, const float* d_lafs_in, const int32_t* d_ids_in, const float* d_A,
                     const int32_t* d_count_in, float* d_resp_out, float* d_lafs_out, int32_t* d_ids_out, int32_t* d_count_out, hipStream_t st);
int aff_shape_iterate(affnet_ctx* ctx, const float* A, float* base, const float* lafs, const int32_t* count, int mode, float* lafs_out,
                      hipStream_t st);
void aff_denorm_sel_fill(affnet_ctx* ctx, int ps, float* d_lafs_px, int32_t* d_ids, float* d_lafs_norm, DenormSel* ds);
int aff_denorm_level_select(affnet_ctx* ctx, const float* d_lafs_norm_in, float* d_lafs_px, const int32_t* d_count, int n_max, int ps, int32_t* d_ids,
                            float* d_lafs_norm, hipStream_t st);

int aff_affnet_filter_rows(affnet_ctx* ctx, const float* packed, const float* resp, const float* lafs, const int32_t* ids, const int32_t* count,
                           float* out, float* scratch, int row_begin, int row_count, bool lazy, int shape_op, hipStream_t st);
int aff_orinet_rotate(affnet_ctx* ctx, const float* packed, float* lafs, const int32_t* ids, const int32_t* count, int n_max, float* out, float* scratch,
                      hipStream_t st, const DenormSel* denorm);
int aff_hardnet_forward_pyr_marked(affnet_ctx* ctx, const float* packed, const float* lafs, const int32_t* ids, const int32_t* count,
                                   int n_max, float* out, float* scratch, hipStream_t st);

int aff_hardnet_poly_patches(affnet_ctx* ctx, const float* packed, const float* patches, int n, float* out, float* scratch, int dbg_layer, hipStream_t st,
                             int form = AFFNET_DESC_FORM_POLYPHASE);
TrunkKernel aff_trunk_kernel(int kind, int form, bool stamps);
int aff_trunk_launch(affnet_ctx* ctx, const CnnCall& c, const NetLayout& L, dim3 grid, int wino, const int32_t* reeval, int shape_op);

TrunkKernel aff_trunk_affnet(int form, bool stamps), aff_trunk_affnet_poly(int form, bool stamps), aff_trunk_orinet(int form, bool stamps);
TrunkKernel aff_trunk_hardnet(int form, bool stamps), aff_trunk_hardnet_poly(int form, bool stamps), aff_trunk_hardnet_f43(int form, bool stamps);
int aff_derived_u_ensure(affnet_ctx* ctx);
int aff_derive_u(affnet_ctx* ctx, int kind, int form, const float* packed, const NetLayout& L, hipStream_t st, const float** region);

int aff_finish_affnet(affnet_ctx* ctx, const CnnCall& c, const NetLayout& L, int rows, int B);
int aff_margin_affnet(affnet_ctx* ctx, const CnnCall& c, const NetLayout& L, int rows, int B, int32_t* flags);
int aff_finish_orinet(affnet_ctx* ctx, const CnnCall& c, const NetLayout& L, int rows, int B);
int aff_hardnet_head(affnet_ctx* ctx, const CnnCall& c, const NetLayout& L, int B);

void aff_sqnorm_launch(hipStream_t st, const float* x, int n, int dim, float* out);
void aff_knn_merge_launch(hipStream_t st, const float* part_d, const int32_t* part_i, int n1, int n_lists, int k, float* out_d, int32_t* out_i);
void aff_knn_q8_merge_launch(hipStream_t st, const int32_t* part_d, const int32_t* part_i, int n1, int n_lists, int k, float scale, int32_t* out_d2,
                             float* out_f, int32_t* out_i);

struct AffSkip { int lo, hi; };
static inline AffSkip aff_skip_range(int skip_row, int skip_n, int n2) {
    const long long lo64 = skip_row < 0 ? 0 : skip_row, hi64 = (long long)skip_row + skip_n;
    return {(int)(lo64 < n2 ? lo64 : n2), (int)(hi64 < 0 ? 0 : (hi64 < n2 ? hi64 : n2))};
}

static inline int aff_topk_cap(int k) { return k == 1 ? 1 : (k == 2 ? 2 : (k <= 4 ? 4 : 8)); }
template <typename F>
static inline void aff_topk_dispatch(int k, F f) {
    switch (aff_topk_cap(k)) {
        case 1: f(std::integral_constant<int, 1>()); break;
        case 2: f(std::integral_constant<int, 2>()); break;
        case 4: f(std::integral_constant<int, 4>()); break;
        default: f(std::integral_constant<int, 8>()); break;
    }
}

static inline int aff_chunk_choice(const affnet_ctx* ctx, long long row_blocks, long long units, int workgroups_per_cu, int min_units, int max_chunks) {
    int cus = 256;
    if (ctx) {
        int v = 0;
        if (hipDeviceGetAttribute(&v, hipDeviceAttributeMultiprocessorCount, ctx->device) == hipSuccess && v > 0) cus = v;
        else (void)hipGetLastError();
    }
    const long long want = ((long long)workgroups_per_cu * cus + row_blocks - 1) / row_blocks, most = units / min_units;
    long long nc = want < most ? want : most;
    if (nc > max_chunks) nc = max_chunks;
    return nc < 1 ? 1 : (int)nc;
}

struct AffTile {
    int x0, y0, tw, th;
};

__device__ __forceinline__ AffTile aff_tile_box(float t00, float t01, float t02, float t10, float t11, float t12, int ps, int cap) {
    const float um = (float)(ps - 1) / (float)ps;
    const float hx = (fabsf(t00) + fabsf(t01)) * um, hy = (fabsf(t10) + fabsf(t11)) * um;
    const float cx = t02 - 0.5f, cy = t12 - 0.5f;
    AffTile t;
    t.tw = 0; t.th = 0; t.x0 = 0; t.y0 = 0;
    if (!(hx < 4096.0f && hy < 4096.0f && fabsf(cx) < 1.0e6f && fabsf(cy) < 1.0e6f)) return t;
    const int x0 = (int)floorf(cx - hx) - 1, x1 = (int)floorf(cx + hx) + 2;
    const int y0 = (int)floorf(cy - hy) - 1, y1 = (int)floorf(cy + hy) + 2;
    const int tw = x1 - x0 + 1, th = y1 - y0 + 1;
    if (tw * th > cap || tw * th > 2 * ps * ps) return t;
    t.x0 = x0; t.y0 = y0; t.tw = tw; t.th = th;
    return t;
}

template <int NTHR>
__device__ __forceinline__ void aff_tile_load(float* tile, const AffTile t, const float* __restrict__ img, int h, int w, int tid) {
    const int n = t.tw * t.th;
    for (int i = tid; i < n; i += NTHR) {
        const int ty = i / t.tw, tx = i - ty * t.tw;
        const int gy = t.y0 + ty, gx = t.x0 + tx;
        tile[i] = (gy >= 0 && gy < h && gx >= 0 && gx < w) ? img[(size_t)gy * w + gx] : 0.0f;
    }
}

__device__ __forceinline__ float aff_sample_bilinear(const float* __restrict__ img, int h, int w,
                                                     float t00, float t01, float t02, float t10,
                                                     float t11, float t12, float u, float v) {
    float gx = fmaf(1.0f, t02, fmaf(v, t01, u * t00));
    float gy = fmaf(1.0f, t12, fmaf(v, t11, u * t10));
    const float fw = (float)w, fh = (float)h;
    gx = 2.0f * gx / fw - 1.0f;
    gy = 2.0f * gy / fh - 1.0f;
    const float ix = fmaf(gx + 1.0f, fw * 0.5f, -0.5f);
    const float iy = fmaf(gy + 1.0f, fh * 0.5f, -0.5f);
    const float x0f = floorf(ix), y0f = floorf(iy);
// ... 46 lines not shown
```

affnet_amd/csrc/context.hip:

```cpp
#include <stdarg.h>

#include "common.h"

int aff_fail(affnet_ctx* ctx, int code, const char* fmt, ...) {
    char buf[1024];
    va_list ap;
    va_start(ap, fmt);
    vsnprintf(buf, sizeof(buf), fmt, ap);
    va_end(ap);
    if (ctx) ctx->err = buf;
    return code;
}

__global__ __launch_bounds__(256) void aff_zero_kernel(unsigned char* __restrict__ p, size_t bytes) {
    const size_t head = ((16 - ((size_t)p & 15)) & 15) < bytes ? ((16 - ((size_t)p & 15)) & 15) : bytes;
    const size_t n16 = (bytes - head) / 16, tail0 = head + n16 * 16;
    uint4* q = reinterpret_cast<uint4*>(p + head);
    for (size_t i = (size_t)blockIdx.x * 256 + threadIdx.x; i < n16; i += (size_t)gridDim.x * 256) q[i] = make_uint4(0u, 0u, 0u, 0u);
    if (blockIdx.x == 0) {
        for (size_t i = threadIdx.x; i < head; i += 256) p[i] = 0;
        for (size_t i = tail0 + threadIdx.x; i < bytes; i += 256) p[i] = 0;
    }
}

// ... 120 lines not shown
        g.h = c.oct_h[o]; g.w = c.oct_w[o];
        g.pyr_off = (int64_t)pyr; pyr += (size_t)c.levels_per_octave * g.h * g.w;
        g.map_off = (int64_t)mapb; mapb += aff_align((size_t)g.h * g.w, 16);
        int cap = (int)((size_t)g.h * g.w / div); if (cap < 256) cap = 256;
        g.raw_off = (int64_t)raw; g.raw_cap = cap; raw += cap;
    }
    ctx->B = c.batch > 0 ? c.batch : 1;
    const size_t B = (size_t)ctx->B;
    ctx->pyr_floats = pyr; ctx->map_bytes = mapb; ctx->raw_total = raw; ctx->cand_cap = raw;
    ctx->pyr_stride = aff_align(pyr * sizeof(float)) / sizeof(float);
    ctx->map_stride = aff_align(mapb);
    ctx->raw_stride = raw;
    const int keep = c.max_keep > 0 ? c.max_keep : 65536;
    ctx->cap_pre = c.num_prefilter > 0 ? c.num_prefilter : keep;
    ctx->cap_final = c.num_features > 0 ? c.num_features : ctx->cap_pre;
    if (ctx->cap_final > ctx->cap_pre) ctx->cap_final = ctx->cap_pre;
    size_t off = 0;
    ctx->off_pyr = off; off += B * ctx->pyr_stride * sizeof(float);
    ctx->off_map = off; off += B * ctx->map_stride;
    ctx->off_raw = off; off += aff_align(B * raw * sizeof(RawMax));
    ctx->off_cnt = off; off += aff_align(B * CNT_TOTAL * sizeof(int32_t));
    ctx->off_hist = off; off += aff_align(B * SEL_HIST_BINS * sizeof(uint32_t));
    ctx->off_cand = off; off += aff_align(B * ctx->cand_cap * 7 * sizeof(float));
    ctx->off_sel = off; off += aff_align(B * (size_t)ctx->cap_pre * 7 * sizeof(float));
    ctx->off_stage = off;
    const size_t P = B * (size_t)ctx->cap_pre, F = B * (size_t)ctx->cap_final;
    off += aff_align(P * 10 * sizeof(float));
    off += aff_align(P * 4 * sizeof(float));
    off += aff_align(P * 10 * sizeof(float));
    off += aff_align(P * 2 * sizeof(float));
    off += aff_align(P * sizeof(int32_t));
    off += aff_align(B * sizeof(int32_t));
    off += aff_align(F * 6 * sizeof(float));
    off += aff_align(F * 4 * sizeof(float));
    off += aff_align(F * 9 * sizeof(float));
    {
        const size_t hard = F * (8192 + 4 * 128), aff = P * 144;
        off += aff_align((hard > aff ? hard : aff) * sizeof(float));
    }
    if (c.onepass) {
        if (c.num_prefilter != c.num_features) { *out = ctx; return aff_fail(ctx, AFFNET_ERR_INVALID, "onepass: num_prefilter must equal num_features"); }
        size_t aff = 0;
        for (int o = 0; o < c.n_octaves; ++o) {
            if (c.oct_h[o] < 34 || c.oct_w[o] < 34) {
                *out = ctx;
                return aff_fail(ctx, AFFNET_ERR_INVALID, "onepass: octave %d is %dx%d, LocalNorm2d(33) needs >= 34 px in this library (17 in the reference: use "
                                "border >= 15 like its scripts, so that the pyramid stops earlier)", o, c.oct_w[o], c.oct_h[o]);
            }
            ctx->aff_off[o] = aff; aff += aff_align((size_t)4 * c.oct_h[o] * c.oct_w[o] * sizeof(float)) / sizeof(float);
        }
        ctx->aff_stride = aff;
        ctx->dense_stride = affnet_fullconv_scratch_bytes(c.oct_h[0], c.oct_w[0]) / sizeof(float);
        ctx->off_affmap = off; off += aff_align(B * aff * sizeof(float));
        ctx->off_dense = off; off += aff_align(B * ctx->dense_stride * sizeof(float));
        ctx->off_cand2 = off; off += aff_align(B * ctx->cand_cap * 7 * sizeof(float));
        ctx->off_lvltab = off; off += aff_align(B * (size_t)AFFNET_MAX_OCTAVES * AFFNET_MAX_LEVELS * 4 * sizeof(int32_t));
    }
    ctx->ws_bytes = off;
    *out = ctx;
    return AFFNET_OK;
}

extern "C" void affnet_ctx_destroy(affnet_ctx* ctx) { delete ctx; }

extern "C" int affnet_set_arith(affnet_ctx* ctx, int arith) {
    if (!ctx) return AFFNET_ERR_INVALID;
    if (arith < AFFNET_ARITH_FP32_MFMA || arith > AFFNET_ARITH_FP32_SPLIT2H) return aff_fail(ctx, AFFNET_ERR_INVALID, "arith=%d (AFFNET_ARITH_*)", arith);
    ctx->arith = arith;
    ctx->cfg.arith = arith;
    return AFFNET_OK;
}
extern "C" int affnet_get_arith(const affnet_ctx* ctx) { return ctx ? ctx->arith : AFFNET_ERR_INVALID; }

extern "C" int affnet_set_shape_form(affnet_ctx* ctx, int form) {
    if (!ctx) return AFFNET_ERR_INVALID;
    if (form != AFFNET_SHAPE_FORM_DIRECT && form != AFFNET_SHAPE_FORM_WINOGRAD && form != AFFNET_SHAPE_FORM_POLYPHASE) return aff_fail(ctx, AFFNET_ERR_INVALID, "shape form=%d (AFFNET_SHAPE_FORM_*)", form);
    ctx->shape_form = form;
    return AFFNET_OK;
}
extern "C" int affnet_get_shape_form(const affnet_ctx* ctx) { return ctx ? ctx->shape_form : AFFNET_ERR_INVALID; }

extern "C" int affnet_set_desc_form(affnet_ctx* ctx, int form) {
    if (!ctx) return AFFNET_ERR_INVALID;
    if (form != AFFNET_DESC_FORM_DIRECT && form != AFFNET_DESC_FORM_POLYPHASE && form != AFFNET_DESC_FORM_F43) return aff_fail(ctx, AFFNET_ERR_INVALID, "descriptor form=%d (AFFNET_DESC_FORM_*)", form);
    ctx->desc_form = form;
    return AFFNET_OK;
}
extern "C" int affnet_get_desc_form(const affnet_ctx* ctx) { return ctx ? ctx->desc_form : AFFNET_ERR_INVALID; }

extern "C" size_t affnet_workspace_bytes(const affnet_ctx* ctx) { return ctx ? ctx->ws_bytes : 0; }

extern "C" int affnet_capacity_prefilter(const affnet_ctx* ctx) { return ctx ? ctx->cap_pre : 0; }
extern "C" int affnet_capacity_final(const affnet_ctx* ctx) { return ctx ? ctx->cap_final : 0; }

extern "C" int64_t affnet_pyramid_level_offset(const affnet_ctx* ctx, int octave, int level) {
    if (!ctx || octave < 0 || octave >= ctx->cfg.n_octaves || level < 0 || level >= ctx->cfg.levels_per_octave) return -1;
    const OctaveGeom& g = ctx->oct[octave];
    return (int64_t)(ctx->off_pyr / sizeof(float)) + g.pyr_off + (int64_t)level * g.h * g.w;
}

extern "C" int64_t affnet_pyramid_image_stride(const affnet_ctx* ctx) { return ctx ? (int64_t)ctx->pyr_stride : 0; }

extern "C" int64_t affnet_counter_offset(const affnet_ctx* ctx, int which) {
    if (!ctx || ctx->ws_bytes == 0 || which < 0 || which > 4) return -1;
    const int idx = which == 0 ? CNT_OVERFLOW : (which == 1 ? CNT_DET : (which == 2 ? CNT_SHAPED : (which == 3 ? CNT_AFF_EVAL : CNT_AFF_REEVAL)));
    return (int64_t)(ctx->off_cnt / sizeof(int32_t)) + idx;
}
extern "C" int64_t affnet_counter_stride(const affnet_ctx* ctx) { return ctx ? (int64_t)CNT_TOTAL : 0; }

extern "C" int64_t affnet_affmap_offset(const affnet_ctx* ctx, int octave) {
    if (!ctx || !ctx->cfg.onepass || octave < 0 || octave >= ctx->cfg.n_octaves) return -1;
    return (int64_t)(ctx->off_affmap / sizeof(float)) + (int64_t)ctx->aff_off[octave];
}
extern "C" int64_t affnet_affmap_image_stride(const affnet_ctx* ctx) { return (ctx && ctx->cfg.onepass) ? (int64_t)ctx->aff_stride : 0; }
extern "C" int affnet_batch(const affnet_ctx* ctx) { return ctx ? ctx->B : 0; }

extern "C" int affnet_bind_workspace(affnet_ctx* ctx, void* d_workspace, size_t bytes) {
    if (!ctx) return AFFNET_ERR_INVALID;
    if (!d_workspace || bytes < ctx->ws_bytes)
        return aff_fail(ctx, AFFNET_ERR_INVALID, "workspace too small: %zu < %zu", bytes, ctx->ws_bytes);
    if (((uintptr_t)d_workspace & 255) != 0) return aff_fail(ctx, AFFNET_ERR_INVALID, "workspace must be 256-byte aligned");
    {
        hipPointerAttribute_t at;
        if (hipPointerGetAttributes(&at, d_workspace) == hipSuccess) {
            if (at.type == hipMemoryTypeDevice && at.device != ctx->device)
                return aff_fail(ctx, AFFNET_ERR_INVALID, "workspace belongs to device %d, the context to device %d", at.device, ctx->device);
        } else {
            (void)hipGetLastError();
        }
    }
    char* b = (char*)d_workspace;
    ctx->ws = b;
    ctx->pyr = (float*)(b + ctx->off_pyr);
    ctx->omap = (uint8_t*)(b + ctx->off_map);
    ctx->raw = (RawMax*)(b + ctx->off_raw);
    ctx->cnt = (int32_t*)(b + ctx->off_cnt);
    ctx->sel_hist = (uint32_t*)(b + ctx->off_hist);
    const size_t B = (size_t)ctx->B;
    float* cand = (float*)(b + ctx->off_cand);
    const size_t CC = B * ctx->cand_cap;
    ctx->cand_resp = cand; ctx->cand_syx = cand + CC; ctx->cand_ids = (int32_t*)(cand + 4 * CC);
    float* sel = (float*)(b + ctx->off_sel);
    const size_t P = B * (size_t)ctx->cap_pre, F = B * (size_t)ctx->cap_final;
    ctx->sel_resp = sel; ctx->sel_syx = sel + P; ctx->sel_ids = (int32_t*)(sel + 4 * P);
    char* s = b + ctx->off_stage;
    ctx->st_det_resp = (float*)s; ctx->st_det_lafs = (float*)s + P; ctx->st_det_ids = (int32_t*)((float*)s + 7 * P);
    s += aff_align(P * 10 * sizeof(float));
    ctx->st_A = (float*)s; s += aff_align(P * 4 * sizeof(float));
    ctx->st_A2 = (float*)s; ctx->st_lafs_iter = (float*)s + 4 * P; s += aff_align(P * 10 * sizeof(float));
    ctx->st_key = (float*)s; ctx->st_good = (int32_t*)((float*)s + P); s += aff_align(P * 2 * sizeof(float));
    ctx->st_rank = (int32_t*)s; s += aff_align(P * sizeof(int32_t));
    ctx->st_det_count = (int32_t*)s; s += aff_align(B * sizeof(int32_t));
    ctx->st_lafs_shaped = (float*)s; s += aff_align(F * 6 * sizeof(float));
    ctx->st_R = (float*)s; s += aff_align(F * 4 * sizeof(float));
    ctx->st_lafs_norm = (float*)s; ctx->st_lvl_ids = (int32_t*)((float*)s + 6 * F); s += aff_align(F * 9 * sizeof(float));
    ctx->st_hard_scratch = (float*)s;
    if (ctx->cfg.onepass) {
        ctx->affmap = (float*)(b + ctx->off_affmap);
        ctx->dense = (float*)(b + ctx->off_dense);
        float* c2 = (float*)(b + ctx->off_cand2);
        ctx->cand2_resp = c2; ctx->cand2_syx = c2 + CC; ctx->cand2_ids = (int32_t*)(c2 + 4 * CC);
        ctx->lvltab = (int32_t*)(b + ctx->off_lvltab);
    }
    return AFFNET_OK;
}

extern "C" int affnet_read_counts(affnet_ctx* ctx, int32_t out[4], void* stream) {
// ... 24 lines not shown
```

affnet_amd/csrc/debug.hip:

```cpp
#include "common.h"

#include "../../include/affnet_hip_probes.h"

template <typename T>
__global__ __launch_bounds__(256) void stream_read_kernel(const T* __restrict__ src, float* __restrict__ dst, size_t n_items) {
    float acc = 0.f;
    for (size_t i = (size_t)blockIdx.x * 256 + threadIdx.x; i < n_items; i += (size_t)gridDim.x * 256) {
        const T v = src[i];
        const float* f = reinterpret_cast<const float*>(&v);
#pragma unroll
        for (int k = 0; k < (int)(sizeof(T) / 4); ++k) acc += f[k];
    }
    if (acc == 123.456f) dst[blockIdx.x] = acc;
    if (threadIdx.x == 0 && blockIdx.x == 0) dst[0] = acc;
}

template <typename T>
__global__ __launch_bounds__(256) void stream_write_kernel(T* __restrict__ dst, size_t n_items) {
    T v;
    float* f = reinterpret_cast<float*>(&v);
#pragma unroll
    for (int k = 0; k < (int)(sizeof(T) / 4); ++k) f[k] = (float)(threadIdx.x + k);
    for (size_t i = (size_t)blockIdx.x * 256 + threadIdx.x; i < n_items; i += (size_t)gridDim.x * 256) dst[i] = v;
}
// ... 51 lines not shown
    if (ctx->arith != AFFNET_ARITH_FP32_MFMA) return aff_fail(ctx, AFFNET_ERR_INVALID, "probe_affnet_wino: AFFNET_ARITH_FP32_MFMA only");
    CnnCall c;
    c.kind = AFFNET_NET_AFFNET; c.packed = d_packed; c.patches = d_patches; c.n_max = n; c.st = st;
    c.out = d_out; c.scratch = d_out;
    c.dbg_layer = layer; c.dbg_out = d_out;
    return aff_trunk_launch(ctx, c, net_layout(AFFNET_NET_AFFNET), dim3(n, 1), poly ? 2 : 1, nullptr, 0);
}

extern "C" int affnet_probe_affnet_wino_layer(affnet_ctx* ctx, int net_kind, const float* d_packed, const float* d_patch, int layer, float* d_out, void* stream) {
    AFF_DEVICE(ctx);
    if (!ctx || !d_packed || !d_patch || !d_out || net_kind != AFFNET_NET_AFFNET || layer < 0 || layer > 5)
        return aff_fail(ctx, AFFNET_ERR_INVALID, "probe_affnet_wino_layer: AffNet, layer 0 .. 5");
    return probe_affnet_wino(ctx, d_packed, d_patch, 1, d_out, layer, (hipStream_t)stream);
}

extern "C" int affnet_probe_affnet_wino_partials(affnet_ctx* ctx, const float* d_packed, const float* d_patches, int n, float* d_partials, void* stream) {
    AFF_DEVICE(ctx);
    if (!ctx || !d_packed || !d_patches || !d_partials || n < 1 || n > 65535) return aff_fail(ctx, AFFNET_ERR_INVALID, "probe_affnet_wino_partials: bad argument");
    return probe_affnet_wino(ctx, d_packed, d_patches, n, d_partials, -1, (hipStream_t)stream);
}

extern "C" int affnet_probe_affnet_poly_layer(affnet_ctx* ctx, int net_kind, const float* d_packed, const float* d_patch, int layer, float* d_out, void* stream) {
    AFF_DEVICE(ctx);
    if (!ctx || !d_packed || !d_patch || !d_out || net_kind != AFFNET_NET_AFFNET || layer < 0 || layer > 5)
        return aff_fail(ctx, AFFNET_ERR_INVALID, "probe_affnet_poly_layer: AffNet, layer 0 .. 5");
    return probe_affnet_wino(ctx, d_packed, d_patch, 1, d_out, layer, (hipStream_t)stream, true);
}

extern "C" int affnet_probe_affnet_poly_partials(affnet_ctx* ctx, const float* d_packed, const float* d_patches, int n, float* d_partials, void* stream) {
    AFF_DEVICE(ctx);
    if (!ctx || !d_packed || !d_patches || !d_partials || n < 1 || n > 65535) return aff_fail(ctx, AFFNET_ERR_INVALID, "probe_affnet_poly_partials: bad argument");
    return probe_affnet_wino(ctx, d_packed, d_patches, n, d_partials, -1, (hipStream_t)stream, true);
}

static int probe_derived_u(affnet_ctx* ctx, int kind, int form, const float* d_packed, int offset, int floats, float* d_out, void* stream) {
    const float* u;
    const int rc = aff_derive_u(ctx, kind, form, d_packed, net_layout(kind), (hipStream_t)stream, &u);
    if (rc) return rc;
    return aff_copy_async(ctx, d_out, u + offset, (size_t)floats * sizeof(float), (hipStream_t)stream);
}

extern "C" int affnet_probe_trunk16_poly_u(affnet_ctx* ctx, int net_kind, const float* d_packed, int layer, float* d_out, void* stream) {
    AFF_DEVICE(ctx);
    if (!ctx || !d_packed || !d_out || (net_kind != AFFNET_NET_AFFNET && net_kind != AFFNET_NET_ORINET) || (layer != 2 && layer != 4))
        return aff_fail(ctx, AFFNET_ERR_INVALID, "probe_trunk16_poly_u: AffNet / OriNet, layer 2 or 4");
    return probe_derived_u(ctx, net_kind, net_kind == AFFNET_NET_AFFNET ? TRUNK_WINO_POLY : TRUNK_EXACT, d_packed, Wino16::offset(layer), Wino16::floats(layer), d_out, stream);
}

extern "C" int affnet_probe_hardnet_poly_layer(affnet_ctx* ctx, const float* d_packed, const float* d_patch, int layer, float* d_out, void* stream) {
    AFF_DEVICE(ctx);
    if (!ctx || !d_packed || !d_patch || !d_out || layer < 0 || layer > 5) return aff_fail(ctx, AFFNET_ERR_INVALID, "probe_hardnet_poly_layer: layer 0 .. 5");
    return aff_hardnet_poly_patches(ctx, d_packed, d_patch, 1, d_out, nullptr, layer, (hipStream_t)stream);
}

extern "C" int affnet_probe_hardnet_poly_forward(affnet_ctx* ctx, const float* d_packed, const float* d_patches, int n, float* d_out, float* d_scratch, void* stream) {
    AFF_DEVICE(ctx);
    if (!ctx || !d_packed || !d_patches || !d_out || !d_scratch || n < 1 || n > 65535) return aff_fail(ctx, AFFNET_ERR_INVALID, "probe_hardnet_poly_forward: bad argument");
    return aff_hardnet_poly_patches(ctx, d_packed, d_patches, n, d_out, d_scratch, -1, (hipStream_t)stream);
}

extern "C" int affnet_probe_hardnet_poly_u(affnet_ctx* ctx, const float* d_packed, int layer, float* d_out, void* stream) {
    AFF_DEVICE(ctx);
    if (!ctx || !d_packed || !d_out || (layer != 2 && layer != 4)) return aff_fail(ctx, AFFNET_ERR_INVALID, "probe_hardnet_poly_u: layer 2 or 4");
    return probe_derived_u(ctx, AFFNET_NET_HARDNET, TRUNK_WINO, d_packed, Poly32::offset(layer), Poly32::floats(layer), d_out, stream);
}

extern "C" int affnet_probe_hardnet_f43_layer(affnet_ctx* ctx, const float* d_packed, const float* d_patch, int layer, float* d_out, void* stream) {
    AFF_DEVICE(ctx);
    if (!ctx || !d_packed || !d_patch || !d_out || layer < 0 || layer > 5) return aff_fail(ctx, AFFNET_ERR_INVALID, "probe_hardnet_f43_layer: layer 0 .. 5");
    return aff_hardnet_poly_patches(ctx, d_packed, d_patch, 1, d_out, nullptr, layer, (hipStream_t)stream, AFFNET_DESC_FORM_F43);
}

extern "C" int affnet_probe_hardnet_f43_forward(affnet_ctx* ctx, const float* d_packed, const float* d_patches, int n, float* d_out, float* d_scratch, void* stream) {
    AFF_DEVICE(ctx);
    if (!ctx || !d_packed || !d_patches || !d_out || !d_scratch || n < 1 || n > 65535) return aff_fail(ctx, AFFNET_ERR_INVALID, "probe_hardnet_f43_forward: bad argument");
    return aff_hardnet_poly_patches(ctx, d_packed, d_patches, n, d_out, d_scratch, -1, (hipStream_t)stream, AFFNET_DESC_FORM_F43);
}

extern "C" int affnet_probe_hardnet_f43_u(affnet_ctx* ctx, const float* d_packed, int layer, float* d_out, void* stream) {
    AFF_DEVICE(ctx);
    if (!ctx || !d_packed || !d_out || (layer != 1 && layer != 3)) return aff_fail(ctx, AFFNET_ERR_INVALID, "probe_hardnet_f43_u: layer 1 or 3");
    return probe_derived_u(ctx, AFFNET_NET_HARDNET, TRUNK_WINO_F43, d_packed, F43::BASE + F43::offset(layer), F43::floats(layer), d_out, stream);
}
```

affnet_amd/csrc/derive_u.hip:

```cpp
#include "common.h"

__global__ __launch_bounds__(256) void derive_u_kernel(const float* __restrict__ packed, NetOffsets off, DerivedTable t, float* __restrict__ U) {
    derive_u_pair(t, blockIdx.x * 256 + threadIdx.x, packed, off.w, U);
}

int aff_derived_u_ensure(affnet_ctx* ctx) {
    if (ctx->derived_u) return AFFNET_OK;
    AFF_HIP(ctx, hipMalloc((void**)&ctx->derived_u, (size_t)DerivedU::FLOATS * sizeof(float)));
    return AFFNET_OK;
}

static DerivedTable table_of(int kind, int form) {
    if (kind == AFFNET_NET_HARDNET) return form == TRUNK_WINO ? derived_hardnet_poly() : (form == TRUNK_WINO_F43 ? derived_hardnet_form2() : DerivedTable{});
    const bool wino = kind == AFFNET_NET_ORINET ? form == TRUNK_EXACT : (form == TRUNK_WINO || form == TRUNK_WINO_POLY);
    return wino ? derived_trunk16() : DerivedTable{};
}

int aff_derive_u(affnet_ctx* ctx, int kind, int form, const float* packed, const NetLayout& L, hipStream_t st, const float** region) {
    *region = nullptr;
    const DerivedTable t = table_of(kind, form);
    if (t.n == 0) return AFFNET_OK;
    const int rc = aff_derived_u_ensure(ctx);
    if (rc) return rc;
    float* dst = ctx->derived_u + DerivedU::region(kind);
    hipLaunchKernelGGL(derive_u_kernel, dim3(t.pairs / 256), dim3(256), 0, st, packed, to_offsets(L), t, dst);
    AFF_LAUNCH_CHECK(ctx);
    *region = dst;
    return AFFNET_OK;
}
```

affnet_amd/csrc/pack_check.cpp:

```cpp
#include <math.h>
#include <stdio.h>
#include <string.h>

#include <initializer_list>
#include <memory>

#include "../../include/affnet_hip.h"
#include "weights_layout.h"

#define CHECK(cond) do { if (!(cond)) { fprintf(stderr, "pack_check: line %d: %s\n", __LINE__, #cond); return 1; } } while (0)

struct State {
    std::unique_ptr<float[]> conv[6], mean[6], var[6], head_w, head_b, hbm, hbv, out;
    const float *conv_p[6], *mean_p[6], *var_p[6];
    size_t conv_n[6], total;
};

static uint32_t lcg = 12345u;
static float rnd() { lcg = lcg * 1664525u + 1013904223u; return (float)(lcg >> 8) / (float)(1 << 24) - 0.5f; }
static std::unique_ptr<float[]> filled(size_t n, float scale, float offset) {
    std::unique_ptr<float[]> p(new float[n]);
    for (size_t i = 0; i < n; ++i) p[i] = rnd() * scale + offset;
    return p;
}

static void make_state(int kind, State& s) {
    const int cb = kind == AFFNET_NET_HARDNET ? 32 : 16, ch[7] = {1, cb, cb, 2 * cb, 2 * cb, 4 * cb, 4 * cb};
    for (int i = 0; i < 6; ++i) {
        s.conv_n[i] = (size_t)ch[i + 1] * ch[i] * 9;
        s.conv[i] = filled(s.conv_n[i], 0.2f, 0.f); s.mean[i] = filled(ch[i + 1], 1.f, 0.f); s.var[i] = filled(ch[i + 1], 1.f, 1.f);
        s.conv_p[i] = s.conv[i].get(); s.mean_p[i] = s.mean[i].get(); s.var_p[i] = s.var[i].get();
    }
    const int no = kind == AFFNET_NET_ORINET ? 2 : 3;
    if (kind == AFFNET_NET_HARDNET) { s.head_w = filled((size_t)128 * 128 * 64, 0.02f, 0.f); s.hbm = filled(128, 1.f, 0.f); s.hbv = filled(128, 1.f, 1.f); }
    else { s.head_w = filled((size_t)no * 64 * 64, 0.1f, 0.f); s.head_b = filled(no, 1.f, 0.f); }
    s.total = affnet_cnn32_packed_floats(kind);
    s.out.reset(new float[s.total]);
}

static int pack(int kind, State& s) {
    return affnet_cnn32_pack_weights(kind, s.conv_p, s.mean_p, s.var_p, s.head_w.get(), s.head_b.get(), s.hbm.get(), s.hbv.get(), s.out.get());
}

static int check_kind(int kind) {
    State s;
    make_state(kind, s);
    CHECK(s.total > 0 && pack(kind, s) == AFFNET_OK);
    size_t nonfinite = 0;
    for (size_t i = 0; i < s.total; ++i) nonfinite += !isfinite(s.out[i]);
    CHECK(nonfinite == 0);
    int64_t want = -1;
    for (int layer = -1; layer <= 6; ++layer) {
        const bool has = kind == AFFNET_NET_HARDNET && (layer == 1 || layer == 3 || layer == 5);
        const int64_t got = affnet_cnn32_winograd_offset(kind, layer);
        if (!has) { CHECK(got == -1); continue; }
        if (want < 0) want = (int64_t)s.total - 16 * (32 * 32 + 64 * 64 + 128 * 128);
        CHECK(got == want);
        want += 16 * (layer == 1 ? 32 * 32 : layer == 3 ? 64 * 64 : 128 * 128);
    }
    CHECK(affnet_cnn32_winograd_offset(-1, 1) == -1 && affnet_cnn32_winograd_offset(4, 1) == -1 && affnet_cnn32_packed_floats(-1) == 0 && affnet_cnn32_packed_floats(4) == 0);
    float* const o = s.out.get();
    const float *hw = s.head_w.get(), *hb = s.head_b.get(), *m = s.hbm.get(), *v = s.hbv.get();
    CHECK(affnet_cnn32_pack_weights(kind, nullptr, s.mean_p, s.var_p, hw, hb, m, v, o) == AFFNET_ERR_INVALID);
    CHECK(affnet_cnn32_pack_weights(kind, s.conv_p, nullptr, s.var_p, hw, hb, m, v, o) == AFFNET_ERR_INVALID);
    CHECK(affnet_cnn32_pack_weights(kind, s.conv_p, s.mean_p, nullptr, hw, hb, m, v, o) == AFFNET_ERR_INVALID);
    CHECK(affnet_cnn32_pack_weights(kind, s.conv_p, s.mean_p, s.var_p, nullptr, hb, m, v, o) == AFFNET_ERR_INVALID);
    CHECK(affnet_cnn32_pack_weights(kind, s.conv_p, s.mean_p, s.var_p, hw, hb, m, v, nullptr) == AFFNET_ERR_INVALID);
    CHECK(affnet_cnn32_pack_weights(-1, s.conv_p, s.mean_p, s.var_p, hw, hb, m, v, o) == AFFNET_ERR_INVALID);
    CHECK(affnet_cnn32_pack_weights(4, s.conv_p, s.mean_p, s.var_p, hw, hb, m, v, o) == AFFNET_ERR_INVALID);
    if (kind == AFFNET_NET_HARDNET) {
        CHECK(affnet_cnn32_pack_weights(kind, s.conv_p, s.mean_p, s.var_p, hw, hb, nullptr, v, o) == AFFNET_ERR_INVALID);
        CHECK(affnet_cnn32_pack_weights(kind, s.conv_p, s.mean_p, s.var_p, hw, hb, m, nullptr, o) == AFFNET_ERR_INVALID);
    } else {
        CHECK(affnet_cnn32_pack_weights(kind, s.conv_p, s.mean_p, s.var_p, hw, nullptr, m, v, o) == AFFNET_ERR_INVALID);
    }
    int edges = 0;
    const float saved = s.conv[3][7], saved_var = s.var[2][1];
    for (const float x : {INFINITY, NAN}) { s.conv[3][7] = x; CHECK(pack(kind, s) == AFFNET_OK); ++edges; }
    s.conv[3][7] = saved;
    s.var[2][1] = 0.f; CHECK(pack(kind, s) == AFFNET_OK); ++edges;
    s.var[2][1] = saved_var;
    for (const float scale : {0.f, 1e-30f, 1e30f}) {
        for (int i = 0; i < 6; ++i)
            for (size_t j = 0; j < s.conv_n[i]; ++j) s.conv[i][j] = scale * ((j & 1) ? -1.f : 1.f);
        CHECK(pack(kind, s) == AFFNET_OK); ++edges;
    }
    printf("kind %d: %zu floats packed, %d edge cases and the rejected arguments as documented\n", kind, s.total, edges);
    return 0;
}

static_assert(Wino16::offset(1) == 0 && Wino16::offset(3) == 4096 && Wino16::offset(5) == 20480 && Wino16::offset(2) == 86016 && Wino16::offset(4) == 98816 && Wino16::FLOATS == 150016 && Wino16::PAIRS == 7936, "Wino16");
static_assert(Poly32::offset(2) == 0 && Poly32::offset(4) == 51200 && Poly32::FLOATS == 256000 && Poly32::PAIRS == 10240, "Poly32");
static_assert(F43::BASE == 256000 && F43::offset(1) == 0 && F43::offset(3) == 36864 && F43::FLOATS == 184320 && F43::PAIRS == 5120, "F43");

static int check_derived(const char* name, int kind, const DerivedTable& t, int want_sections, size_t want_floats) {
    const NetLayout L = net_layout(kind); const NetOffsets off = to_offsets(L);
    CHECK(L.total == affnet_cnn32_packed_floats(kind) && t.n == want_sections && t.n <= DERIVED_MAX && (size_t)t.floats == want_floats && t.pairs % 256 == 0);
    const std::unique_ptr<float[]> blob = filled(L.total, 0.2f, 0.f), U(new float[want_floats]), want(new float[want_floats]);
    const std::unique_ptr<unsigned char[]> owned(new unsigned char[want_floats]());
    const float sentinel = -12345.f;
    for (size_t i = 0; i < want_floats; ++i) U[i] = sentinel;
    size_t pairs = 0, floats = 0;
    for (int i = 0; i < t.n; ++i) {
        const DerivedSection& s = t.s[i];
        const int xi = s.family == DERIVED_WINO ? 16 : s.family == DERIVED_POLY ? 25 : 36;
        CHECK(s.layer >= 1 && s.layer <= 5 && s.cin == L.cin[s.layer] && s.cout == L.cout[s.layer] && (size_t)s.pair0 == pairs && s.family >= 0 && s.family <= DERIVED_F43);
        for (int c = 0; c < s.cin; ++c)
            for (int n = 0; n < s.cout; ++n, ++pairs) {
                float g[9], u[36];
                for (int tap = 0; tap < 9; ++tap) g[tap] = blob[L.w_off[s.layer] + w_tap_index(tap, c, n, s.cin, s.cout)];
                if (s.family == DERIVED_WINO) wino_weight_transform(g, u);
                else if (s.family == DERIVED_POLY) poly_weight_transform(g, u);
                else f43_weight_transform(g, u);
                const size_t e = s.pair0 + w_tap_index(0, c, n, s.cin, s.cout);
                CHECK(e < (size_t)t.pairs);
                for (int p = 0; p < xi; ++p, ++floats) {
                    const size_t d = s.dst + w_tap_index(p, c, n, s.cin, s.cout);
                    CHECK(d < want_floats && !owned[d] && U[d] == sentinel);
                    owned[d] = 1; want[d] = u[p];
                }
                derive_u_pair(t, (int)e, blob.get(), off.w, U.get());
            }
    }
    for (int e = t.pairs; e < t.pairs + 256; ++e) derive_u_pair(t, e, blob.get(), off.w, U.get());
    CHECK(pairs == (size_t)t.pairs && floats == want_floats && memcmp(U.get(), want.get(), want_floats * sizeof(float)) == 0);
    printf("derived %s: %d sections, %d pairs, %zu floats: every float written once, by its own pair, with its transform\n", name, t.n, t.pairs, want_floats);
    return 0;
}

static int check_regions() {
    const size_t t16 = derived_trunk16().floats, poly = derived_hardnet_poly().floats, f43 = derived_hardnet_f43().floats;
    CHECK(DerivedU::AFFNET == 0 && DerivedU::ORINET == t16 && DerivedU::HARDNET == 2 * t16 && DerivedU::HARDNET_F43 == 2 * t16 + poly && DerivedU::FLOATS == 2 * t16 + poly + f43);
    CHECK(DerivedU::region(AFFNET_NET_AFFNET) == DerivedU::AFFNET && DerivedU::region(AFFNET_NET_ORINET) == DerivedU::ORINET && DerivedU::region(AFFNET_NET_HARDNET) == DerivedU::HARDNET);
    CHECK(derived_hardnet_form2().floats == poly + f43);
    return 0;
}

int main() {
    for (int kind = 0; kind <= AFFNET_NET_AFFNET_FULLCONV; ++kind)
        if (check_kind(kind)) return 1;
    if (check_derived("AffNet", AFFNET_NET_AFFNET, derived_trunk16(), 5, 150016) || check_derived("OriNet", AFFNET_NET_ORINET, derived_trunk16(), 5, 150016) ||
        check_derived("HardNet polyphase", AFFNET_NET_HARDNET, derived_hardnet_poly(), 2, 256000) || check_derived("HardNet F(4x4, 3x3)", AFFNET_NET_HARDNET, derived_hardnet_f43(), 2, 184320) ||
        check_derived("HardNet form 2", AFFNET_NET_HARDNET, derived_hardnet_form2(), 4, 256000 + 184320) || check_regions())
        return 1;
    return 0;
}
```

affnet_amd/csrc/weights_layout.h:

```cpp
#pragma once
#include <stddef.h>
#include <stdint.h>

#include "../../include/affnet_hip.h"

#ifdef __HIPCC__
#define AFF_HOST_DEVICE __host__ __device__
#else
#define AFF_HOST_DEVICE
#endif

#define HEAD_K 8192
#define H2_TAIL 4
#define S3_LAYER_MASK 0x3E

constexpr size_t w_tap_index(int p, int c, int n, int cin, int cout) {
    return ((((size_t)p * (cin / 16) + c / 16) * 4 + (c / 4) % 4) * cout + n) * 4 + c % 4;
}

constexpr size_t w_split_index(int tap, int c, int term, int n, int cin, int cout, int terms) {
    const int step = cin == 16 ? tap / 2 : tap * (cin / 32) + c / 32;
    const int kq = cin == 16 ? (tap % 2) * 2 + c / 8 : (c % 32) / 8;
    return ((((size_t)step * terms + term) * 4 + kq) * cout + n) * 8 + c % 8;
}
// ... 87 lines not shown
    size_t off = 0;
    L.c1_w = off; off += (size_t)TFEAT_K1 * 32;
    L.c1_b = off; off += 32;
    L.c2_w = off; off += (size_t)36 * 32 * 64;
    L.c2_b = off; off += 64;
    L.head_w = off; off += (size_t)TFEAT_HEAD_K * 128;
    L.head_b = off; off += 128;
    L.total = off;
    return L;
}

AFF_HOST_DEVICE inline void wino_g_axis(float g0, float g1, float g2, float* o, int stride) {
    const float s = g0 + g2;
    o[0] = g0; o[stride] = 0.5f * (s + g1); o[2 * stride] = 0.5f * (s - g1); o[3 * stride] = g2;
}
AFF_HOST_DEVICE inline void wino_weight_transform(const float g[9], float U[16]) {
    float t[12];
#pragma unroll
    for (int ky = 0; ky < 3; ++ky) wino_g_axis(g[3 * ky], g[3 * ky + 1], g[3 * ky + 2], t + 4 * ky, 1);
#pragma unroll
    for (int j = 0; j < 4; ++j) wino_g_axis(t[j], t[4 + j], t[8 + j], U + j, 4);
}

#define POLY_XI 25
AFF_HOST_DEVICE inline void poly_weight_transform(const float g[9], float U[POLY_XI]) {
    float t[3][3];
#pragma unroll
    for (int ky = 0; ky < 3; ++ky) { t[ky][0] = g[3 * ky]; t[ky][1] = g[3 * ky] + g[3 * ky + 2]; t[ky][2] = g[3 * ky + 2]; }
#pragma unroll
    for (int j = 0; j < 3; ++j) {
        const float s = t[0][j] + t[2][j];
        U[j] = t[0][j]; U[3 + j] = s; U[6 + j] = t[2][j];
        U[15 + j] = t[1][j]; U[18 + j] = t[1][j];
    }
    const float se = g[1] + g[7];
#pragma unroll
    for (int j = 0; j < 2; ++j) {
        U[9 + j] = g[1]; U[11 + j] = se; U[13 + j] = g[7];
        U[21 + j] = g[4]; U[23 + j] = g[4];
    }
}

#define F43_XI 36
AFF_HOST_DEVICE inline void f43_g_axis(float g0, float g1, float g2, float* o, int stride) {
    const float c6 = 1.0f / 6.0f, c12 = 1.0f / 12.0f, c24 = 1.0f / 24.0f;
    const float s = g0 + g2;
    const float p = c24 * g0 + c6 * g2, q = c12 * g1;
    o[0] = 0.25f * g0; o[stride] = -c6 * (s + g1); o[2 * stride] = -c6 * (s - g1);
    o[3 * stride] = p + q; o[4 * stride] = p - q; o[5 * stride] = g2;
}
AFF_HOST_DEVICE inline void f43_weight_transform(const float g[9], float U[F43_XI]) {
    float t[18];
#pragma unroll
    for (int ky = 0; ky < 3; ++ky) f43_g_axis(g[3 * ky], g[3 * ky + 1], g[3 * ky + 2], t + 6 * ky, 1);
#pragma unroll
    for (int j = 0; j < 6; ++j) f43_g_axis(t[j], t[6 + j], t[12 + j], U + j, 6);
}

enum { DERIVED_WINO = 0, DERIVED_POLY = 1, DERIVED_F43 = 2 };
constexpr int derived_xi(int family) { return family == DERIVED_WINO ? 16 : (family == DERIVED_POLY ? POLY_XI : F43_XI); }
struct DerivedSection {
    int layer, cin, cout;
    int family;
    int pair0;
    int dst;
};
constexpr int derived_floats(const DerivedSection& s) { return derived_xi(s.family) * s.cin * s.cout; }
#define DERIVED_MAX 5
struct DerivedTable {
    int n, pairs, floats;
    DerivedSection s[DERIVED_MAX];
};
constexpr DerivedTable derived_add(DerivedTable t, int cb, int layer, int family) {
    const DerivedSection s = {layer, cb << ((layer - 1) / 2), cb << (layer / 2), family, t.pairs, t.floats};
    t.s[t.n++] = s; t.pairs += s.cin * s.cout; t.floats += derived_floats(s);
    return t;
}
constexpr DerivedTable derived_trunk16() {
    return derived_add(derived_add(derived_add(derived_add(derived_add(DerivedTable{}, 16, 1, DERIVED_WINO), 16, 3, DERIVED_WINO), 16, 5, DERIVED_WINO), 16, 2, DERIVED_POLY), 16, 4, DERIVED_POLY);
}
constexpr DerivedTable derived_hardnet_poly() { return derived_add(derived_add(DerivedTable{}, 32, 2, DERIVED_POLY), 32, 4, DERIVED_POLY); }
constexpr DerivedTable derived_hardnet_f43() { return derived_add(derived_add(DerivedTable{}, 32, 1, DERIVED_F43), 32, 3, DERIVED_F43); }
constexpr DerivedTable derived_hardnet_form2() { return derived_add(derived_add(derived_hardnet_poly(), 32, 1, DERIVED_F43), 32, 3, DERIVED_F43); }
constexpr DerivedSection derived_layer(const DerivedTable& t, int layer) {
    for (int i = 0; i < t.n; ++i)
        if (t.s[i].layer == layer) return t.s[i];
    return DerivedSection{-1, 0, 0, 0, 0, 0};
}
constexpr DerivedSection derived_section(const DerivedTable& t, int e) {
    DerivedSection s = t.s[0];
    for (int i = 1; i < DERIVED_MAX; ++i)
        if (i < t.n && e >= t.s[i].pair0) s = t.s[i];
    return s;
}
constexpr bool derived_by_workgroups(const DerivedTable& t, int i = 0) {
    return i == t.n || (t.s[i].pair0 % 256 == 0 && t.s[i].cin * t.s[i].cout % 256 == 0 && derived_by_workgroups(t, i + 1));
}
static_assert(derived_by_workgroups(derived_trunk16()) && derived_by_workgroups(derived_hardnet_poly()) && derived_by_workgroups(derived_hardnet_f43()) &&
              derived_by_workgroups(derived_hardnet_form2()), "a 256-thread workgroup of derive_u_kernel stays within one section");

template <DerivedTable (*T)()>
struct DerivedView {
    static constexpr int FLOATS = T().floats, PAIRS = T().pairs;
    static constexpr int offset(int layer) { return derived_layer(T(), layer).dst; }
    static constexpr int floats(int layer) { return derived_floats(derived_layer(T(), layer)); }
};
struct Wino16 : DerivedView<derived_trunk16> { static constexpr int NB1 = 2, NB3 = 1; };
typedef DerivedView<derived_hardnet_poly> Poly32;
struct F43 : DerivedView<derived_hardnet_f43> { static constexpr int BASE = Poly32::FLOATS; };
static_assert(derived_hardnet_form2().s[2].dst == F43::BASE + F43::offset(1) && derived_hardnet_form2().s[3].dst == F43::BASE + F43::offset(3) &&
              derived_hardnet_form2().floats == F43::BASE + F43::FLOATS, "form 2's table = Poly32 with F43 at F43::BASE");

struct DerivedU {
    static constexpr int AFFNET = 0, ORINET = AFFNET + Wino16::FLOATS;
    static constexpr int HARDNET = ORINET + Wino16::FLOATS;
    static constexpr int HARDNET_F43 = HARDNET + F43::BASE;
    static constexpr int FLOATS = HARDNET_F43 + F43::FLOATS;
    static constexpr int region(int kind) { return kind == AFFNET_NET_AFFNET ? AFFNET : (kind == AFFNET_NET_ORINET ? ORINET : HARDNET); }
};
static_assert(DerivedU::AFFNET == 0 && DerivedU::ORINET - DerivedU::AFFNET == derived_trunk16().floats && DerivedU::HARDNET - DerivedU::ORINET == derived_trunk16().floats &&
              DerivedU::FLOATS - DerivedU::HARDNET == derived_hardnet_form2().floats && DerivedU::FLOATS == 2 * Wino16::FLOATS + Poly32::FLOATS + F43::FLOATS,
              "the regions are disjoint, in this order, and fill the buffer");
static_assert(DerivedU::ORINET % 64 == 0 && DerivedU::HARDNET % 64 == 0 && DerivedU::HARDNET_F43 % 64 == 0, "every region starts on a 256-byte boundary, as an allocation of its own would");
static_assert(w_tap_index(7, 21, 13, 32, 64) == 7 * 32 * 64 + w_tap_index(0, 21, 13, 32, 64) && w_tap_index(35, 63, 63, 64, 64) == 35 * 64 * 64 + w_tap_index(0, 63, 63, 64, 64),
              "a position is a plane of cin * cout floats");
AFF_HOST_DEVICE inline void derive_u_pair(const DerivedTable& t, int e, const float* packed, const int (&w_off)[6], float* U) {
    if (e >= t.pairs) return;
    const DerivedSection s = derived_section(t, e & ~255);
    const int plane = s.cin * s.cout;
    const float* src = packed + w_off[s.layer] + (e - s.pair0);
    float* dst = U + s.dst + (e - s.pair0);
    float g[9];
#pragma unroll
    for (int tap = 0; tap < 9; ++tap) g[tap] = src[(size_t)tap * plane];
    float u[F43_XI];
    if (s.family == DERIVED_WINO) wino_weight_transform(g, u);
    else if (s.family == DERIVED_POLY) poly_weight_transform(g, u);
    else f43_weight_transform(g, u);
#pragma unroll
    for (int xi = 0; xi < F43_XI; ++xi)
        if (xi < derived_xi(s.family)) dst[(size_t)xi * plane] = u[xi];
}
```

affnet_amd/engine.py:

```python
import ctypes as C

import numpy as np
import torch

from . import _lib
from ._lib import lib, check, ptr
from .host_plan import PyramidPlan

_UTILITY = {}


def require_cuda(t, what="tensor"):
    if not (isinstance(t, torch.Tensor) and t.is_cuda):
        raise RuntimeError("affnet_amd: %s must live on the MI355X (tensor.cuda()); this implementation has no CPU path" % what)


def utility_ctx(device, arith=0):
    idx = device.index if device.index is not None else torch.cuda.current_device()
    key = (idx, _lib.arith_code(arith))
    if key not in _UTILITY:
        h = C.c_void_p()
        check(lib.affnet_ctx_create(C.byref(h), idx, None), None, "affnet_ctx_create(utility)")
        check(lib.affnet_set_arith(h, key[1]), h, "affnet_set_arith")
        _UTILITY[key] = h
    h = _UTILITY[key]
    if lib.affnet_get_arith(h) != key[1]:
        check(lib.affnet_set_arith(h, key[1]), h, "affnet_set_arith")
    return h


def stream_of(device):
    return C.c_void_p(torch.cuda.current_stream(device).cuda_stream)


class Context(object):

    def __init__(self, height, width, device, n_levels, init_sigma, border, mr_size, threshold,
                 num_features, num_prefilter, max_keep=16384, batch=1, baum_iters=0, raw_div=4, onepass=False, lazy_shape_rows=-1, arith=0):
        self.plan = PyramidPlan(height, width, n_levels, init_sigma, border)
        self.batch = int(batch)
        self.onepass = bool(onepass)
        self.cfg = self.plan.fill_config(mr_size, threshold, num_features, num_prefilter, max_keep, raw_div=raw_div, batch=self.batch, baum_iters=baum_iters,
                                         onepass=onepass, lazy_shape_rows=lazy_shape_rows, arith=arith)
        self.arith = _lib.arith_code(arith)
        self.shape_form = _lib.SHAPE_FORM_WINOGRAD
        self.desc_form = _lib.DESC_FORM_F43
        self.device = device
        self.handle = C.c_void_p()
        idx = device.index if device.index is not None else torch.cuda.current_device()
        rc = lib.affnet_ctx_create(C.byref(self.handle), idx, C.byref(self.cfg))
        check(rc, self.handle, "affnet_ctx_create")
        nbytes = lib.affnet_workspace_bytes(self.handle)
        self.workspace = torch.empty(nbytes, dtype=torch.uint8, device=device)
        check(lib.affnet_bind_workspace(self.handle, ptr(self.workspace), nbytes), self.handle, "affnet_bind_workspace")
        self.cap_pre = lib.affnet_capacity_prefilter(self.handle)
        self.cap_final = lib.affnet_capacity_final(self.handle)
        self._ws_f32 = self.workspace.view(torch.float32)

    def set_arith(self, arith):
        self.arith = _lib.arith_code(arith)
        check(lib.affnet_set_arith(self.handle, self.arith), self.handle, "affnet_set_arith")

    def set_shape_form(self, form):
        check(lib.affnet_set_shape_form(self.handle, int(form)), self.handle, "affnet_set_shape_form")
        self.shape_form = int(form)

    def set_desc_form(self, form):
        check(lib.affnet_set_desc_form(self.handle, int(form)), self.handle, "affnet_set_desc_form")
        self.desc_form = int(form)

    def pyramid_views(self, image=0):
        pyr = []
        base = image * lib.affnet_pyramid_image_stride(self.handle)
        for o, (h, w) in enumerate(self.plan.sizes):
            levels = []
            for l in range(self.plan.levels_per_octave):
                off = base + lib.affnet_pyramid_level_offset(self.handle, o, l)
                levels.append(self._ws_f32[off:off + h * w].view(1, 1, h, w))
            pyr.append(levels)
        return pyr

    def affmap_views(self, image=0):
        base = image * lib.affnet_affmap_image_stride(self.handle)
        out = []
        for o, (h, w) in enumerate(self.plan.sizes):
            off = base + lib.affnet_affmap_offset(self.handle, o)
            out.append(self._ws_f32[off:off + 4 * h * w].view(1, 4, h, w))
        return out

    def counter_view(self, which=0):
        off, stride = lib.affnet_counter_offset(self.handle, which), lib.affnet_counter_stride(self.handle)
        return self.workspace.view(torch.int32)[off:off + stride * self.batch:stride]

    def read_counts(self, allow_empty=False):
        out = (C.c_int32 * 4)()
        rc = lib.affnet_read_counts(self.handle, C.byref(out), stream_of(self.device))
        if not (allow_empty and rc == _lib.ERR_EMPTY):
            check(rc, self.handle, "affnet_read_counts")
        return list(out)

    def __del__(self):
        try:
            if self.handle:
                lib.affnet_ctx_destroy(self.handle)
                self.handle = None
        except Exception:
            pass


def pack_state_dict(kind, sd, winograd=False):
    conv_idx, bn_idx = (0, 3, 6, 9, 12, 15), (1, 4, 7, 10, 13, 16)

    def f32(name):
        return sd[name].detach().to("cpu", torch.float32).contiguous()

    keep = []
    convs = [f32("features.%d.weight" % i) for i in conv_idx]
    means = [f32("features.%d.running_mean" % i) for i in bn_idx]
    vars_ = [f32("features.%d.running_var" % i) for i in bn_idx]
    head_w = f32("features.19.weight")
    head_b = f32("features.19.bias") if "features.19.bias" in sd else None
    if kind == _lib.NET_AFFNET_FULLCONV and head_b is None:
        raise ValueError("AffNetFastFullConv: features.19.bias missing from the state dict")
    hbm = f32("features.20.running_mean") if kind == _lib.NET_HARDNET else None
    hbv = f32("features.20.running_var") if kind == _lib.NET_HARDNET else None
    keep += convs + means + vars_ + [head_w, head_b, hbm, hbv]
    arr = lambda ts: (C.c_void_p * 6)(*[t.data_ptr() for t in ts])
    n = lib.affnet_cnn32_packed_floats(kind)
    out = torch.empty(n, dtype=torch.float32)
# ... 77 lines not shown
```

include/affnet_hip.h:

```cpp
#ifndef AFFNET_HIP_H
#define AFFNET_HIP_H

#include <stddef.h>
#include <stdint.h>

#ifdef __cplusplus
extern "C" {
#endif

#define AFFNET_OK 0
#define AFFNET_ERR_INVALID (-1)
#define AFFNET_ERR_HIP (-2)
#define AFFNET_ERR_CAPACITY (-3)
#define AFFNET_ERR_EMPTY (-4)

#define AFFNET_MAX_OCTAVES 16
#define AFFNET_MAX_LEVELS 8
#define AFFNET_MAX_TAPS 37

#define AFFNET_NET_AFFNET 0
#define AFFNET_NET_ORINET 1
#define AFFNET_NET_HARDNET 2
#define AFFNET_NET_AFFNET_FULLCONV 3

#define AFFNET_ARITH_FP32_MFMA 0
#define AFFNET_ARITH_FP32_SPLIT3 1
#define AFFNET_ARITH_FP32_SPLIT2H 2

typedef struct affnet_ctx affnet_ctx;

typedef struct affnet_config {
    int32_t height, width;
    int32_t n_octaves;
    int32_t levels_per_octave;
    int32_t oct_h[AFFNET_MAX_OCTAVES];
    int32_t oct_w[AFFNET_MAX_OCTAVES];
    float level_sigma[AFFNET_MAX_OCTAVES][AFFNET_MAX_LEVELS];
    float level_sigma4[AFFNET_MAX_OCTAVES][AFFNET_MAX_LEVELS];
    double level_sigma_px[AFFNET_MAX_OCTAVES][AFFNET_MAX_LEVELS];
    int32_t first_blur_taps;
    float first_blur[AFFNET_MAX_TAPS * AFFNET_MAX_TAPS];
    int32_t level_blur_taps[AFFNET_MAX_LEVELS];
    float level_blur[AFFNET_MAX_LEVELS][AFFNET_MAX_TAPS * AFFNET_MAX_TAPS];
    int32_t level_blur0_taps[AFFNET_MAX_LEVELS];
    float level_blur0[AFFNET_MAX_LEVELS][AFFNET_MAX_TAPS * AFFNET_MAX_TAPS];
    int32_t lazy_shape_rows;
    int32_t onepass;
    float mr_size;
    float threshold;
    int32_t num_features;
    int32_t num_prefilter;
    int32_t max_raw_per_octave_div;
    int32_t max_keep;
    int32_t batch;
    int32_t baum_iters;
    int32_t arith;
} affnet_config;

int affnet_config_fill(affnet_config* cfg, int height, int width, int n_levels, double init_sigma, int border, double mr_size,
                       double threshold, int num_features, int num_prefilter, int batch, int baum_iters);


int affnet_ctx_create(affnet_ctx** out, int device, const affnet_config* cfg);
void affnet_ctx_destroy(affnet_ctx* ctx);
const char* affnet_last_error(const affnet_ctx* ctx);
const char* affnet_version(void);
int affnet_set_arith(affnet_ctx* ctx, int arith);
int affnet_get_arith(const affnet_ctx* ctx);

#define AFFNET_SHAPE_FORM_DIRECT 0
#define AFFNET_SHAPE_FORM_WINOGRAD 1
#define AFFNET_SHAPE_FORM_POLYPHASE 2
int affnet_set_shape_form(affnet_ctx* ctx, int form);
int affnet_get_shape_form(const affnet_ctx* ctx);

#define AFFNET_DESC_FORM_DIRECT 0
#define AFFNET_DESC_FORM_POLYPHASE 1
#define AFFNET_DESC_FORM_F43 2
int affnet_set_desc_form(affnet_ctx* ctx, int form);
int affnet_get_desc_form(const affnet_ctx* ctx);

size_t affnet_workspace_bytes(const affnet_ctx* ctx);
int affnet_bind_workspace(affnet_ctx* ctx, void* d_workspace, size_t bytes);
int64_t affnet_pyramid_level_offset(const affnet_ctx* ctx, int octave, int level);
int64_t affnet_pyramid_image_stride(const affnet_ctx* ctx);
int affnet_batch(const affnet_ctx* ctx);
int affnet_capacity_prefilter(const affnet_ctx* ctx);
int affnet_capacity_final(const affnet_ctx* ctx);


int affnet_gauss_blur(affnet_ctx* ctx, const float* d_in, float* d_out, int h, int w,
                      const float* h_taps, int k, void* stream);

int affnet_pyramid_build(affnet_ctx* ctx, const float* d_img, void* stream);

int affnet_hessian_response(affnet_ctx* ctx, const float* d_in, float* d_out, int h, int w,
                            float sigma4, void* stream);

int affnet_detect(affnet_ctx* ctx, float* d_resp, float* d_lafs, int32_t* d_ids,
                  int32_t* d_count, void* stream);

int affnet_detect_responses(affnet_ctx* ctx, const float* d_responses, float* d_resp, float* d_lafs, int32_t* d_ids,
                            int32_t* d_count, void* stream);

int affnet_laf_grid_sample(affnet_ctx* ctx, const float* d_img, int h, int w,
                           const float* d_lafs, int n, int ps, float* d_out, void* stream);

int affnet_pyr_grid_sample(affnet_ctx* ctx, const float* d_lafs, const int32_t* d_ids,
                           const int32_t* d_count, int n_max, int ps, float* d_out, void* stream);


size_t affnet_cnn32_packed_floats(int net_kind);
int64_t affnet_cnn32_winograd_offset(int net_kind, int layer);
int affnet_cnn32_pack_weights(int net_kind, const float* const* conv_w, const float* const* bn_mean,
                              const float* const* bn_var, const float* head_w, const float* head_b,
                              const float* head_bn_mean, const float* head_bn_var, float* h_out);

int affnet_cnn32_forward(affnet_ctx* ctx, int net_kind, const float* d_packed, const float* d_patches,
                         const int32_t* d_count, int n_max, float* d_out, float* d_scratch, void* stream);

int affnet_cnn32_forward_pyr(affnet_ctx* ctx, int net_kind, const float* d_packed, const float* d_lafs,
                             const int32_t* d_ids, const int32_t* d_count, int n_max, float* d_out,
                             float* d_scratch, void* stream);


int affnet_local_norm(affnet_ctx* ctx, const float* d_in, float* d_out, int h, int w, void* stream);

size_t affnet_fullconv_scratch_bytes(int h, int w);

int affnet_fullconv_forward(affnet_ctx* ctx, const float* d_packed, const float* d_img, int h, int w, float* d_out, float* d_scratch,
                            void* stream);

int affnet_nms2d(affnet_ctx* ctx, const float* d_in, float* d_out, int h, int w, float threshold, void* stream);


#define AFFNET_HC_ORIENTATION 0
#define AFFNET_HC_BAUMBERG 1

int affnet_handcrafted_forward(affnet_ctx* ctx, int kind, const float* d_patches, int n, const float* h_weights, float* d_out,
                               float* d_angles, void* stream);
int affnet_handcrafted_forward_pyr(affnet_ctx* ctx, int kind, const float* d_lafs, const int32_t* d_ids, const int32_t* d_count,
                                   int n_max, const float* h_weights, float* d_out, void* stream);


int affnet_sift_host_window(int patch_size, float* h_out);
int affnet_sift_forward(affnet_ctx* ctx, const float* d_patches, int n, const float* d_window, float clipval, float* d_desc, void* stream);
int affnet_sift_forward_pyr(affnet_ctx* ctx, const float* d_lafs_norm, const int32_t* d_ids, const int32_t* d_count, int n_max,
                            const float* d_window, float clipval, float* d_desc, void* stream);


size_t affnet_tfeat_packed_floats(void);
int affnet_tfeat_pack_weights(const float* conv1_w, const float* conv1_b, const float* conv2_w, const float* conv2_b, const float* cls_w,
                              const float* cls_b, float* h_out);
size_t affnet_tfeat_scratch_floats(int rows);
int affnet_tfeat_forward(affnet_ctx* ctx, const float* d_packed, const float* d_patches, const int32_t* d_count, int n_max, float* d_desc,
                         float* d_scratch, void* stream);
int affnet_tfeat_forward_pyr(affnet_ctx* ctx, const float* d_packed, const float* d_lafs_norm, const int32_t* d_ids, const int32_t* d_count,
                             int n_max, float* d_desc, float* d_scratch, void* stream);


int affnet_shape_filter_select(affnet_ctx* ctx, const float* d_resp_in, const float* d_lafs_in,
// ... 196 lines not shown
```

include/affnet_hip_probes.h:

```cpp
#ifndef AFFNET_HIP_PROBES_H
#define AFFNET_HIP_PROBES_H

#include "affnet_hip.h"

#ifdef __cplusplus
extern "C" {
#endif

int affnet_cnn32_probe(const float* d_packed, int layer, int probe, int reps, int n_blocks, float* d_out, void* stream);

int affnet_debug_stream(const void* d_src, void* d_dst, size_t n_bytes, int width, int mode, int halo, void* stream);

int affnet_split3_gemm(const float* d_A, const float* d_Bt, int M, int N, int K, int mode, float* d_C, void* stream);
int affnet_split3_rate(int reps, int terms, int n_blocks, float* d_out, void* stream);

int affnet_probe_shape_offsets(const affnet_ctx* ctx, int64_t out[3]);

int affnet_probe_affnet_wino_layer(affnet_ctx* ctx, int net_kind, const float* d_packed, const float* d_patch, int layer, float* d_out, void* stream);

int affnet_probe_affnet_wino_partials(affnet_ctx* ctx, const float* d_packed, const float* d_patches, int n, float* d_partials, void* stream);

int affnet_probe_affnet_poly_layer(affnet_ctx* ctx, int net_kind, const float* d_packed, const float* d_patch, int layer, float* d_out, void* stream);
int affnet_probe_affnet_poly_partials(affnet_ctx* ctx, const float* d_packed, const float* d_patches, int n, float* d_partials, void* stream);
int affnet_probe_trunk16_poly_u(affnet_ctx* ctx, int net_kind, const float* d_packed, int layer, float* d_out, void* stream);

int affnet_probe_hardnet_poly_layer(affnet_ctx* ctx, const float* d_packed, const float* d_patch, int layer, float* d_out, void* stream);
int affnet_probe_hardnet_poly_forward(affnet_ctx* ctx, const float* d_packed, const float* d_patches, int n, float* d_out, float* d_scratch, void* stream);
int affnet_probe_hardnet_poly_u(affnet_ctx* ctx, const float* d_packed, int layer, float* d_out, void* stream);

int affnet_probe_hardnet_f43_layer(affnet_ctx* ctx, const float* d_packed, const float* d_patch, int layer, float* d_out, void* stream);
int affnet_probe_hardnet_f43_forward(affnet_ctx* ctx, const float* d_packed, const float* d_patches, int n, float* d_out, float* d_scratch, void* stream);
int affnet_probe_hardnet_f43_u(affnet_ctx* ctx, const float* d_packed, int layer, float* d_out, void* stream);

#ifdef __cplusplus
}
#endif
#endif
```

Baseline: 1.675 million.

## Split HardNet conv5 into a separate F(4x4,3x3) Winograd kernel across patch groups

Result: faster. 1.743 million, median of 6 (+4.1%).

```diff
diff --git a/affnet_amd/SparseImgRepresenter.py b/affnet_amd/SparseImgRepresenter.py
--- a/affnet_amd/SparseImgRepresenter.py
+++ b/affnet_amd/SparseImgRepresenter.py
@@ -42,7 +42,7 @@
         self.lazy_shape_rows = -1
         self.shape_form = 1
 
-        self.desc_form = 2
+        self.desc_form = 3
 
     def _context(self, x, allow_batch=False):
         engine.require_cuda(x, "image")
diff --git a/affnet_amd/_lib.py b/affnet_amd/_lib.py
--- a/affnet_amd/_lib.py
+++ b/affnet_amd/_lib.py
@@ -23,7 +23,7 @@
         raise ValueError("arith must be AFFNET_ARITH_FP32_MFMA (0), AFFNET_ARITH_FP32_SPLIT3 (1) or AFFNET_ARITH_FP32_SPLIT2H (2)")
     return int(arith)
 SHAPE_FORM_DIRECT, SHAPE_FORM_WINOGRAD, SHAPE_FORM_POLYPHASE = 0, 1, 2
-DESC_FORM_DIRECT, DESC_FORM_POLYPHASE, DESC_FORM_F43 = 0, 1, 2
+DESC_FORM_DIRECT, DESC_FORM_POLYPHASE, DESC_FORM_F43, DESC_FORM_F43_CONV5 = 0, 1, 2, 3
 OK, ERR_INVALID, ERR_HIP, ERR_CAPACITY, ERR_EMPTY = 0, -1, -2, -3, -4
 VERIFY_AFFINE, VERIFY_HOMOGRAPHY, VERIFY_TILE, VERIFY_CHUNK = 0, 1, 128, 128
 KNN_MAX_K = 8
@@ -190,6 +190,10 @@
     "affnet_probe_hardnet_f43_layer": (_I, [_P, _P, _P, _I, _P, _P]),
     "affnet_probe_hardnet_f43_forward": (_I, [_P, _P, _P, _I, _P, _P, _P]),
     "affnet_probe_hardnet_f43_u": (_I, [_P, _P, _I, _P, _P]),
+    "affnet_probe_hardnet_c5_trunk_layer": (_I, [_P, _P, _P, _I, _P, _P]),
+    "affnet_probe_hardnet_c5_forward": (_I, [_P, _P, _P, _I, _P, _P, _P]),
+    "affnet_probe_hardnet_c5_layer": (_I, [_P, _P, _P, _I, _P]),
+    "affnet_probe_hardnet_c5_u": (_I, [_P, _P, _P, _P]),
 }
 
 
diff --git a/affnet_amd/csrc/cnn32.hip b/affnet_amd/csrc/cnn32.hip
--- a/affnet_amd/csrc/cnn32.hip
+++ b/affnet_amd/csrc/cnn32.hip
@@ -27,10 +27,10 @@
 TrunkKernel aff_trunk_kernel(int kind, int form, bool stamps) {
     typedef TrunkKernel (*Unit)(int, bool);
     static_assert(AFFNET_NET_AFFNET == 0 && AFFNET_NET_ORINET == 1 && AFFNET_NET_HARDNET == 2 && TRUNK_EXACT == 0 && TRUNK_WINO == 1 && TRUNK_SPLIT2 == 2 && TRUNK_SPLIT3 == 3 &&
-                  TRUNK_WINO_F43 == 4 && TRUNK_WINO_POLY == 5 && TRUNK_FORMS == 6, "order of the table");
-    static const Unit unit[3][TRUNK_FORMS] = {{aff_trunk_affnet, aff_trunk_affnet, aff_trunk_affnet, aff_trunk_affnet, nullptr, aff_trunk_affnet_poly},
-                                              {aff_trunk_orinet, nullptr, aff_trunk_orinet, aff_trunk_orinet, nullptr, nullptr},
-                                              {aff_trunk_hardnet, aff_trunk_hardnet_poly, aff_trunk_hardnet, aff_trunk_hardnet, aff_trunk_hardnet_f43, nullptr}};
+                  TRUNK_WINO_F43 == 4 && TRUNK_WINO_POLY == 5 && TRUNK_WINO_F43_C5 == 6 && TRUNK_FORMS == 7, "order of the table");
+    static const Unit unit[3][TRUNK_FORMS] = {{aff_trunk_affnet, aff_trunk_affnet, aff_trunk_affnet, aff_trunk_affnet, nullptr, aff_trunk_affnet_poly, nullptr},
+                                              {aff_trunk_orinet, nullptr, aff_trunk_orinet, aff_trunk_orinet, nullptr, nullptr, nullptr},
+                                              {aff_trunk_hardnet, aff_trunk_hardnet_poly, aff_trunk_hardnet, aff_trunk_hardnet, aff_trunk_hardnet_f43, nullptr, aff_trunk_hardnet_c5}};
     if (kind < 0 || kind > 2 || form < 0 || form >= TRUNK_FORMS || !unit[kind][form]) return nullptr;
     return unit[kind][form](form, stamps);
 }
@@ -39,7 +39,8 @@
     int form = TRUNK_EXACT;
     if (ctx->arith != AFFNET_ARITH_FP32_MFMA) form = ctx->arith == AFFNET_ARITH_FP32_SPLIT2H ? TRUNK_SPLIT2 : TRUNK_SPLIT3;
     else if (c.kind == AFFNET_NET_AFFNET && wino) form = wino == 2 ? TRUNK_WINO_POLY : TRUNK_WINO;
-    else if (c.kind == AFFNET_NET_HARDNET && c.desc_form != AFFNET_DESC_FORM_DIRECT) form = c.desc_form == AFFNET_DESC_FORM_F43 ? TRUNK_WINO_F43 : TRUNK_WINO;
+    else if (c.kind == AFFNET_NET_HARDNET && c.desc_form != AFFNET_DESC_FORM_DIRECT)
+        form = c.desc_form == AFFNET_DESC_FORM_F43_CONV5 ? TRUNK_WINO_F43_C5 : (c.desc_form == AFFNET_DESC_FORM_F43 ? TRUNK_WINO_F43 : TRUNK_WINO);
     const bool stamps = ctx->dbg_time || c.dbg_layer >= 0;
     const TrunkKernel kernel = aff_trunk_kernel(c.kind, form, stamps);
     if (!kernel) return aff_fail(ctx, AFFNET_ERR_INVALID, "cnn32: no trunk kernel of net %d in form %d is built", c.kind, form);
@@ -58,6 +59,13 @@
     aff_fill_pyr_src(ctx, &ps);
     hipLaunchKernelGGL(kernel, grid, dim3(512), 0, c.st, a, ps);
     AFF_LAUNCH_CHECK(ctx);
+    if (form == TRUNK_WINO_F43_C5 && c.dbg_layer < 0) {
+        Conv5Args v;
+        v.io = a.out; v.U = a.wino_u + F43C5::BASE; v.bias = c.packed + L.b_off[5];
+        v.count = c.count; v.n_max = c.n_max; v.row_begin = c.row_begin; v.row_end = c.row_begin + (int)grid.x;
+        v.skip_cnt = c.skip_cnt; v.skip_n = c.skip_n; v.dbg_time = ctx->dbg_time;
+        return aff_hardnet_conv5_f43(ctx, v, aff_cdiv((int)grid.x, 4), (int)grid.y, stamps, c.st);
+    }
     return AFFNET_OK;
 }
 
@@ -136,6 +144,7 @@
 
 int aff_hardnet_poly_patches(affnet_ctx* ctx, const float* packed, const float* patches, int n, float* out, float* scratch, int dbg_layer, hipStream_t st, int form) {
     if (ctx->arith != AFFNET_ARITH_FP32_MFMA) return aff_fail(ctx, AFFNET_ERR_INVALID, "hardnet_poly: AFFNET_ARITH_FP32_MFMA only");
+    if (form == AFFNET_DESC_FORM_F43_CONV5 && dbg_layer > 4) return aff_fail(ctx, AFFNET_ERR_INVALID, "hardnet_poly: the trunk of form 3 ends behind layer 4 (conv5: affnet_probe_hardnet_c5_layer)");
     CnnCall c;
     c.kind = AFFNET_NET_HARDNET; c.packed = packed; c.patches = patches; c.n_max = n; c.out = out; c.scratch = scratch; c.st = st;
     c.dbg_layer = dbg_layer; c.dbg_out = dbg_layer >= 0 ? out : nullptr;
diff --git a/affnet_amd/csrc/cnn_mfma.h b/affnet_amd/csrc/cnn_mfma.h
--- a/affnet_amd/csrc/cnn_mfma.h
+++ b/affnet_amd/csrc/cnn_mfma.h
@@ -1232,6 +1232,52 @@
     }
 }
 
+struct F43C5L {
+    static constexpr int WPI = 10;
+    static constexpr int CGS = WPI * WPI * 4;
+    static constexpr int PS = 8 * CGS + 4;
+    static constexpr int IN = 0, IN_FLOATS = 4 * PS;
+    static constexpr int V = IN_FLOATS, V_FLOATS = 2 * F43_XI * 256;
+    static constexpr int TOTAL = V + V_FLOATS;
+};
+static_assert(F43C5L::V % 4 == 0 && F43C5L::PS % 4 == 0 && F43C5L::TOTAL * 4 <= 160 * 1024, "16-byte aligned sections within the CU's LDS");
+
+__device__ __forceinline__ void f43c5_transform(const float* in, float* v) {
+    float t[6][6];
+#pragma unroll
+    for (int c = 0; c < 6; ++c) {
+        float d[6];
+#pragma unroll
+        for (int r = 0; r < 6; ++r) d[r] = in[(r * F43C5L::WPI + c) * 4];
+        f43_bt_lo(d[0], d[1], d[2], d[3], d[4], t[0][c], t[1][c], t[2][c]);
+        f43_bt_hi(d[1], d[2], d[3], d[4], d[5], t[3][c], t[4][c], t[5][c]);
+    }
+#pragma unroll
+    for (int i = 0; i < 6; ++i) {
+        float o[6];
+        f43_bt_lo(t[i][0], t[i][1], t[i][2], t[i][3], t[i][4], o[0], o[1], o[2]);
+        f43_bt_hi(t[i][1], t[i][2], t[i][3], t[i][4], t[i][5], o[3], o[4], o[5]);
+#pragma unroll
+        for (int j = 0; j < 6; ++j) v[(6 * i + j) * 256] = o[j];
+    }
+}
+
+__device__ __forceinline__ void f43c5_output(const f32x4 (&acc)[F43_XI], f32x4 (&y)[16]) {
+#pragma unroll
+    for (int e = 0; e < 4; ++e) {
+        float t[6][4];
+#pragma unroll
+        for (int i = 0; i < 6; ++i) f43_at_axis(acc[6 * i][e], acc[6 * i + 1][e], acc[6 * i + 2][e], acc[6 * i + 3][e], acc[6 * i + 4][e], acc[6 * i + 5][e], t[i][0], t[i][1], t[i][2], t[i][3]);
+#pragma unroll
+        for (int c = 0; c < 4; ++c) {
+            float yr[4];
+            f43_at_axis(t[0][c], t[1][c], t[2][c], t[3][c], t[4][c], t[5][c], yr[0], yr[1], yr[2], yr[3]);
+#pragma unroll
+            for (int dy = 0; dy < 4; ++dy) y[4 * dy + c][e] = yr[dy];
+        }
+    }
+}
+
 template <int NW, int CIN, int COUT, int H, int NB>
 __device__ __forceinline__ void wino_prefetch_u_row(const float* __restrict__ Wu, f32x4 (&U)[4], int wave, int lane) {
     const __amdgpu_buffer_rsrc_t r = weight_rsrc(Wu, 16 * CIN * COUT);
@@ -1434,6 +1480,22 @@
             const int p = (2 * ty + (k >> 1)) * H + 2 * tx + (k & 1);
             const f32x4 v = bias_relu(y[q][k], bias[q]);
             *reinterpret_cast<f32x4*>(dst + p * COUT + cb * 16 + 4 * g) = v;
+        }
+    }
+}
+
+template <int COUT, int H, int NB>
+__device__ __forceinline__ void wino_store_global_c4(float* __restrict__ dst, const f32x4 (&bias)[NB], const f32x4 (&y)[NB][4], int wave, int lane) {
+    const int g = lane >> 4;
+#pragma unroll
+    for (int q = 0; q < NB; ++q) {
+        int ty, tx, cb;
+        wino_tile<H, COUT, NB>(wave, q, lane & 15, ty, tx, cb);
+#pragma unroll
+        for (int k = 0; k < 4; ++k) {
+            const int p = (2 * ty + (k >> 1)) * H + 2 * tx + (k & 1);
+            const f32x4 v = bias_relu(y[q][k], bias[q]);
+            *reinterpret_cast<f32x4*>(dst + ((cb * 4 + g) * (H * H) + p) * 4) = v;
         }
     }
 }
diff --git a/affnet_amd/csrc/cnn_trunk.h b/affnet_amd/csrc/cnn_trunk.h
--- a/affnet_amd/csrc/cnn_trunk.h
+++ b/affnet_amd/csrc/cnn_trunk.h
@@ -168,11 +168,12 @@
 template <int KIND, int S3>
 struct TrunkTraits {
     static_assert(S3 == TRUNK_EXACT || S3 == TRUNK_SPLIT2 || S3 == TRUNK_SPLIT3 || (S3 == TRUNK_WINO && KIND != AFFNET_NET_ORINET) ||
-                  (S3 == TRUNK_WINO_F43 && KIND == AFFNET_NET_HARDNET) || (S3 == TRUNK_WINO_POLY && KIND == AFFNET_NET_AFFNET), "no such trunk form of this net (common.h: TRUNK_*)");
+                  ((S3 == TRUNK_WINO_F43 || S3 == TRUNK_WINO_F43_C5) && KIND == AFFNET_NET_HARDNET) || (S3 == TRUNK_WINO_POLY && KIND == AFFNET_NET_AFFNET), "no such trunk form of this net (common.h: TRUNK_*)");
     static constexpr bool EXACT = S3 != TRUNK_SPLIT2 && S3 != TRUNK_SPLIT3;
     static constexpr bool WINO13 = (S3 == TRUNK_EXACT && KIND == AFFNET_NET_ORINET) || ((S3 == TRUNK_WINO || S3 == TRUNK_WINO_POLY) && KIND == AFFNET_NET_AFFNET);
     static constexpr bool POLY16 = (S3 == TRUNK_EXACT && KIND == AFFNET_NET_ORINET) || (S3 == TRUNK_WINO_POLY && KIND == AFFNET_NET_AFFNET);
-    static constexpr bool POLY = (S3 == TRUNK_WINO || S3 == TRUNK_WINO_F43) && KIND == AFFNET_NET_HARDNET, F43_3 = S3 == TRUNK_WINO_F43 && KIND == AFFNET_NET_HARDNET;
+    static constexpr bool CUT5 = S3 == TRUNK_WINO_F43_C5 && KIND == AFFNET_NET_HARDNET;
+    static constexpr bool POLY = (S3 == TRUNK_WINO || S3 == TRUNK_WINO_F43 || CUT5) && KIND == AFFNET_NET_HARDNET, F43_3 = (S3 == TRUNK_WINO_F43 || CUT5) && KIND == AFFNET_NET_HARDNET;
 };
 
 template <int C, typename L, int NTHR>
@@ -199,7 +200,7 @@
 template <int KIND, int NW, bool STAMPS, int S3 = 0>
 __global__ __launch_bounds__(NW * 64, (KIND == AFFNET_NET_HARDNET) ? NW / 4 : 4) void cnn32_trunk_kernel(CnnArgs a, PyrSrc ps) {
     using F = TrunkTraits<KIND, S3>;
-    constexpr bool EXACT = F::EXACT, WINO13 = F::WINO13, POLY16 = F::POLY16, POLY = F::POLY, F43_3 = F::F43_3;
+    constexpr bool EXACT = F::EXACT, WINO13 = F::WINO13, POLY16 = F::POLY16, POLY = F::POLY, F43_3 = F::F43_3, CUT5 = F::CUT5;
     using S = TrunkShape<KIND, NW>;
     constexpr int CB = S::CB, NTHR = S::NTHR;
     static_assert((CB / 4) * LayC1::PSG <= TrunkLds<CB>::ACT && (CB / 2) * LayC3::PSG <= TrunkLds<CB>::ACT, "LDS layout");
@@ -398,8 +399,15 @@
             conv3x3_poly_mfma_rows<NW, 2 * CB, 4 * CB, LayC3, NBP4, 1>(act, a.wino_u + Poly32::offset(4), P4a, P4b, y, wave, lane);
             __builtin_amdgcn_s_setprio(3);
             CNN_STAMP(9);
-            wino_prefetch_u<NW, 4 * CB, 4 * CB, 8, NB5>(a.packed + a.off.w_wino[2], Uw, wave, lane);
+            if constexpr (!CUT5) wino_prefetch_u<NW, 4 * CB, 4 * CB, 8, NB5>(a.packed + a.off.w_wino[2], Uw, wave, lane);
             wino_bias<NW, 8, 4 * CB, NBP4>(a.packed + a.off.b[4], bw, wave, lane);
+            if constexpr (CUT5) {
+                if (!STAMPS || a.dbg_layer < 0) {
+                    wino_store_global_c4<4 * CB, 8, NBP4>(a.out + pidx * (64 * 4 * CB), bw, y, wave, lane);
+                    CNN_STAMP(13);
+                    return;
+                }
+            }
             __syncthreads();
             zero_halo<LayC4, NTHR>(act, 4 * CB);
             wino_store_lds<4 * CB, LayC4, NBP4>(act, bw, y, wave, lane);
@@ -420,23 +428,25 @@
         }
         if (STAMPS && a.dbg_layer == 4) { dump_planes<4 * CB, LayC4, NTHR>(act, a.dbg_out); return; }
 
-        f32x4 y[NB5][4], bw[NB5];
-        __builtin_amdgcn_s_setprio(0);
-        static_assert(NB5 == 1 && (4 * CB / 16) * 4096 <= TrunkLds<CB>::ACT, "conv5: one pass per wave, V of the layer fits the activation buffer");
-        conv3x3_wino_mfma_shared_v<NW, 4 * CB, 4 * CB, LayC4>(act, a.packed + a.off.w_wino[2], Uw, y, wave, lane);
-        __builtin_amdgcn_s_setprio(3);
-        CNN_STAMP(11);
-        wino_bias<NW, 8, 4 * CB, NB5>(a.packed + a.off.b[5], bw, wave, lane);
-        if (!STAMPS || a.dbg_layer < 0) {
-            wino_store_global<4 * CB, 8, NB5>(a.out + pidx * (64 * 4 * CB), bw, y, wave, lane);
-            CNN_STAMP(13);
-            return;
-        }
-        __syncthreads();
-        wino_store_lds<4 * CB, LayC5, NB5>(act, bw, y, wave, lane);
-        __syncthreads();
-        CNN_STAMP(12);
-        if (STAMPS && a.dbg_layer == 5) { dump_planes<4 * CB, LayC5, NTHR>(act, a.dbg_out); return; }
+        if constexpr (!CUT5) {
+            f32x4 y[NB5][4], bw[NB5];
+            __builtin_amdgcn_s_setprio(0);
+            static_assert(NB5 == 1 && (4 * CB / 16) * 4096 <= TrunkLds<CB>::ACT, "conv5: one pass per wave, V of the layer fits the activation buffer");
+            conv3x3_wino_mfma_shared_v<NW, 4 * CB, 4 * CB, LayC4>(act, a.packed + a.off.w_wino[2], Uw, y, wave, lane);
+            __builtin_amdgcn_s_setprio(3);
+            CNN_STAMP(11);
+            wino_bias<NW, 8, 4 * CB, NB5>(a.packed + a.off.b[5], bw, wave, lane);
+            if (!STAMPS || a.dbg_layer < 0) {
+                wino_store_global<4 * CB, 8, NB5>(a.out + pidx * (64 * 4 * CB), bw, y, wave, lane);
+                CNN_STAMP(13);
+                return;
+            }
+            __syncthreads();
+            wino_store_lds<4 * CB, LayC5, NB5>(act, bw, y, wave, lane);
+            __syncthreads();
+            CNN_STAMP(12);
+            if (STAMPS && a.dbg_layer == 5) { dump_planes<4 * CB, LayC5, NTHR>(act, a.dbg_out); return; }
+        }
     } else if constexpr (EXACT) {
         constexpr int T1M = S::T1M, T1N = S::T1N, T2M = S::T2M, T2N = S::T2N, T4M = S::T4M, T4N = S::T4N;
         static_assert(NW == 8 && CB == 16, "Wino16 describes the 16-channel trunks on 8 waves");
diff --git a/affnet_amd/csrc/cnn_trunk_hardnet_c5.hip b/affnet_amd/csrc/cnn_trunk_hardnet_c5.hip
--- /dev/null
+++ b/affnet_amd/csrc/cnn_trunk_hardnet_c5.hip
@@ -0,0 +1,3 @@
+#include "cnn_trunk.h"
+
+TrunkKernel aff_trunk_hardnet_c5(int form, bool stamps) { return trunk_unit<AFFNET_NET_HARDNET, TRUNK_WINO_F43_C5>(form, stamps); }
diff --git a/affnet_amd/csrc/common.h b/affnet_amd/csrc/common.h
--- a/affnet_amd/csrc/common.h
+++ b/affnet_amd/csrc/common.h
@@ -104,7 +104,7 @@
     hipGraph_t graph = nullptr;
     hipGraphExec_t graph_exec = nullptr;
     float* derived_u = nullptr;
-    int desc_form = AFFNET_DESC_FORM_F43;
+    int desc_form = AFFNET_DESC_FORM_F43_CONV5;
     ~affnet_ctx() {
         if (derived_u) (void)hipFree(derived_u);
         if (graph_exec) (void)hipGraphExecDestroy(graph_exec);
@@ -224,7 +224,8 @@
 constexpr int TRUNK_SPLIT3 = 3;
 constexpr int TRUNK_WINO_F43 = 4;
 constexpr int TRUNK_WINO_POLY = 5;
-constexpr int TRUNK_FORMS = 6;
+constexpr int TRUNK_WINO_F43_C5 = 6;
+constexpr int TRUNK_FORMS = 7;
 
 __device__ __forceinline__ bool lazy_skip(const int32_t* skip_cnt, int skip_n, int image, int which = CNT_SURVIVED1) {
     if (!skip_cnt) return false;
@@ -256,6 +257,16 @@
 
 typedef void (*TrunkKernel)(CnnArgs, PyrSrc);
 
+struct Conv5Args {
+    float* io;
+    const float* U;
+    const float* bias;
+    const int32_t* count; int n_max;
+    int row_begin, row_end;
+    const int32_t* skip_cnt; int skip_n;
+    unsigned long long* dbg_time;
+};
+
 int aff_fail(affnet_ctx* ctx, int code, const char* fmt, ...);
 int aff_zero_async(affnet_ctx* ctx, void* dst, size_t bytes, hipStream_t st);
 int aff_zero_multi_async(affnet_ctx* ctx, const AffZeroSegs& z, hipStream_t st);
@@ -297,6 +308,8 @@
 
 TrunkKernel aff_trunk_affnet(int form, bool stamps), aff_trunk_affnet_poly(int form, bool stamps), aff_trunk_orinet(int form, bool stamps);
 TrunkKernel aff_trunk_hardnet(int form, bool stamps), aff_trunk_hardnet_poly(int form, bool stamps), aff_trunk_hardnet_f43(int form, bool stamps);
+TrunkKernel aff_trunk_hardnet_c5(int form, bool stamps);
+int aff_hardnet_conv5_f43(affnet_ctx* ctx, const Conv5Args& a, int groups, int B, bool stamps, hipStream_t st);
 int aff_derived_u_ensure(affnet_ctx* ctx);
 int aff_derive_u(affnet_ctx* ctx, int kind, int form, const float* packed, const NetLayout& L, hipStream_t st, const float** region);
 
diff --git a/affnet_amd/csrc/context.hip b/affnet_amd/csrc/context.hip
--- a/affnet_amd/csrc/context.hip
+++ b/affnet_amd/csrc/context.hip
@@ -226,7 +226,7 @@
 
 extern "C" int affnet_set_desc_form(affnet_ctx* ctx, int form) {
     if (!ctx) return AFFNET_ERR_INVALID;
-    if (form != AFFNET_DESC_FORM_DIRECT && form != AFFNET_DESC_FORM_POLYPHASE && form != AFFNET_DESC_FORM_F43) return aff_fail(ctx, AFFNET_ERR_INVALID, "descriptor form=%d (AFFNET_DESC_FORM_*)", form);
+    if (form != AFFNET_DESC_FORM_DIRECT && form != AFFNET_DESC_FORM_POLYPHASE && form != AFFNET_DESC_FORM_F43 && form != AFFNET_DESC_FORM_F43_CONV5) return aff_fail(ctx, AFFNET_ERR_INVALID, "descriptor form=%d (AFFNET_DESC_FORM_*)", form);
     ctx->desc_form = form;
     return AFFNET_OK;
 }
diff --git a/affnet_amd/csrc/debug.hip b/affnet_amd/csrc/debug.hip
--- a/affnet_amd/csrc/debug.hip
+++ b/affnet_amd/csrc/debug.hip
@@ -157,3 +157,36 @@
     if (!ctx || !d_packed || !d_out || (layer != 1 && layer != 3)) return aff_fail(ctx, AFFNET_ERR_INVALID, "probe_hardnet_f43_u: layer 1 or 3");
     return probe_derived_u(ctx, AFFNET_NET_HARDNET, TRUNK_WINO_F43, d_packed, F43::BASE + F43::offset(layer), F43::floats(layer), d_out, stream);
 }
+
+extern "C" int affnet_probe_hardnet_c5_trunk_layer(affnet_ctx* ctx, const float* d_packed, const float* d_patch, int layer, float* d_out, void* stream) {
+    AFF_DEVICE(ctx);
+    if (!ctx || !d_packed || !d_patch || !d_out || layer < 0 || layer > 4) return aff_fail(ctx, AFFNET_ERR_INVALID, "probe_hardnet_c5_trunk_layer: layer 0 .. 4");
+    return aff_hardnet_poly_patches(ctx, d_packed, d_patch, 1, d_out, nullptr, layer, (hipStream_t)stream, AFFNET_DESC_FORM_F43_CONV5);
+}
+
+extern "C" int affnet_probe_hardnet_c5_forward(affnet_ctx* ctx, const float* d_packed, const float* d_patches, int n, float* d_out, float* d_scratch, void* stream) {
+    AFF_DEVICE(ctx);
+    if (!ctx || !d_packed || !d_patches || !d_out || !d_scratch || n < 1 || n > 65535) return aff_fail(ctx, AFFNET_ERR_INVALID, "probe_hardnet_c5_forward: bad argument");
+    return aff_hardnet_poly_patches(ctx, d_packed, d_patches, n, d_out, d_scratch, -1, (hipStream_t)stream, AFFNET_DESC_FORM_F43_CONV5);
+}
+
+extern "C" int affnet_probe_hardnet_c5_layer(affnet_ctx* ctx, const float* d_packed, float* d_slots, int n, void* stream) {
+    AFF_DEVICE(ctx);
+    if (!ctx || !d_packed || !d_slots || n < 1 || n > 65535) return aff_fail(ctx, AFFNET_ERR_INVALID, "probe_hardnet_c5_layer: bad argument");
+    if (ctx->arith != AFFNET_ARITH_FP32_MFMA) return aff_fail(ctx, AFFNET_ERR_INVALID, "probe_hardnet_c5_layer: AFFNET_ARITH_FP32_MFMA only");
+    const NetLayout L = net_layout(AFFNET_NET_HARDNET);
+    const float* u;
+    const int rc = aff_derive_u(ctx, AFFNET_NET_HARDNET, TRUNK_WINO_F43_C5, d_packed, L, (hipStream_t)stream, &u);
+    if (rc) return rc;
+    Conv5Args v;
+    v.io = d_slots; v.U = u + F43C5::BASE; v.bias = d_packed + L.b_off[5];
+    v.count = nullptr; v.n_max = n; v.row_begin = 0; v.row_end = n;
+    v.skip_cnt = nullptr; v.skip_n = 0; v.dbg_time = nullptr;
+    return aff_hardnet_conv5_f43(ctx, v, aff_cdiv(n, 4), 1, false, (hipStream_t)stream);
+}
+
+extern "C" int affnet_probe_hardnet_c5_u(affnet_ctx* ctx, const float* d_packed, float* d_out, void* stream) {
+    AFF_DEVICE(ctx);
+    if (!ctx || !d_packed || !d_out) return aff_fail(ctx, AFFNET_ERR_INVALID, "probe_hardnet_c5_u: null argument");
+    return probe_derived_u(ctx, AFFNET_NET_HARDNET, TRUNK_WINO_F43_C5, d_packed, F43C5::BASE, F43C5::FLOATS, d_out, stream);
+}
diff --git a/affnet_amd/csrc/derive_u.hip b/affnet_amd/csrc/derive_u.hip
--- a/affnet_amd/csrc/derive_u.hip
+++ b/affnet_amd/csrc/derive_u.hip
@@ -11,7 +11,7 @@
 }
 
 static DerivedTable table_of(int kind, int form) {
-    if (kind == AFFNET_NET_HARDNET) return form == TRUNK_WINO ? derived_hardnet_poly() : (form == TRUNK_WINO_F43 ? derived_hardnet_form2() : DerivedTable{});
+    if (kind == AFFNET_NET_HARDNET) return form == TRUNK_WINO ? derived_hardnet_poly() : (form == TRUNK_WINO_F43 ? derived_hardnet_form2() : (form == TRUNK_WINO_F43_C5 ? derived_hardnet_form3() : DerivedTable{}));
     const bool wino = kind == AFFNET_NET_ORINET ? form == TRUNK_EXACT : (form == TRUNK_WINO || form == TRUNK_WINO_POLY);
     return wino ? derived_trunk16() : DerivedTable{};
 }
diff --git a/affnet_amd/csrc/hardnet_conv5_f43.hip b/affnet_amd/csrc/hardnet_conv5_f43.hip
--- /dev/null
+++ b/affnet_amd/csrc/hardnet_conv5_f43.hip
@@ -0,0 +1,114 @@
+#include "cnn_mfma.h"
+
+#define C5_STAMP(k)                                                                                                      \
+    do {                                                                                                                 \
+        if (STAMPS && a.dbg_time && lane == 0) a.dbg_time[(pidx0 * 8 + wave) * 32 + (k)] = __builtin_readcyclecounter(); \
+    } while (0)
+
+template <bool STAMPS>
+__global__ __launch_bounds__(512, 2) void hardnet_conv5_f43_kernel(Conv5Args a) {
+    constexpr int CIN = 128, COUT = 128, DU = 6, DV = 6;
+    static_assert(F43_XI % DU == 0 && F43_XI % DV == 0 && DU % 2 == 0 && DV % 2 == 0, "the sets roll with compile-time indices");
+    __shared__ __attribute__((aligned(16))) float lds[F43C5L::TOTAL];
+    const int tid = threadIdx.x, wave = tid >> 6, lane = tid & 63;
+    const int n = a.count ? min(a.count[blockIdx.y], a.n_max) : a.n_max;
+    const int r0 = a.row_begin + 4 * blockIdx.x, rend = min(n, a.row_end);
+    if (r0 >= rend || lazy_skip(a.skip_cnt, a.skip_n, blockIdx.y, CNT_SURVIVED)) return;
+    const int nreal = min(4, rend - r0);
+    const size_t pidx0 = (size_t)blockIdx.y * a.n_max + r0;
+    float* slot = a.io + pidx0 * (64 * CIN);
+    __builtin_amdgcn_s_setprio(3);
+    C5_STAMP(24);
+
+    const __amdgpu_buffer_rsrc_t wrsrc = weight_rsrc(a.U, F43_XI * CIN * COUT);
+    const int u_lane = ((lane >> 4) * COUT + wave * 16 + (lane & 15)) * 16;
+    f32x4 Ur[DU], Vr[DV];
+#pragma unroll
+    for (int k = 0; k < DU; ++k) Ur[k] = wino_load_u<CIN, COUT>(wrsrc, u_lane, k, 0);
+
+    f32x4 in[4];
+    const float* src[4];
+#pragma unroll
+    for (int i = 0; i < 4; ++i) src[i] = slot + min(i, nreal - 1) * (64 * CIN) + (wave * 64 + lane) * 4;
+    auto request = [&](int Q) {
+#pragma unroll
+        for (int i = 0; i < 4; ++i) in[i] = *reinterpret_cast<const f32x4*>(src[i] + Q * (8 * 64 * 4));
+    };
+    request(0);
+    for (int i = tid; i < 32 * 36; i += 512) {
+        const int pc = i / 36, hp = i - pc * 36;
+        const int y = hp < 10 ? 0 : (hp < 20 ? 9 : 1 + ((hp - 20) >> 1)), x = hp < 10 ? hp : (hp < 20 ? hp - 10 : ((hp - 20) & 1) * 9);
+        *reinterpret_cast<f32x4*>(&lds[F43C5L::IN + (pc >> 3) * F43C5L::PS + (pc & 7) * F43C5L::CGS + (y * F43C5L::WPI + x) * 4]) = (f32x4){0.f, 0.f, 0.f, 0.f};
+    }
+    float* in_w = &lds[F43C5L::IN + wave * F43C5L::CGS + (((lane >> 3) + 1) * F43C5L::WPI + (lane & 7) + 1) * 4];
+    const int te = lane & 3, ttx = (lane >> 2) & 1, tp = (lane >> 3) & 3, tty = lane >> 5;
+    const float* t_in = &lds[F43C5L::IN + tp * F43C5L::PS + wave * F43C5L::CGS + (4 * tty * F43C5L::WPI + 4 * ttx) * 4 + te];
+    float* t_v = &lds[F43C5L::V + (wave >> 2) * (F43_XI * 256) + ((wave & 3) * 16 + 4 * tp + 2 * tty + ttx) * 4 + te];
+    const unsigned v0 = lds_byte_addr(lds + F43C5L::V) + lane * 16;
+
+    f32x4 acc[F43_XI];
+#pragma unroll
+    for (int k = 0; k < F43_XI; ++k) acc[k] = (f32x4){0.f, 0.f, 0.f, 0.f};
+
+#pragma unroll 1
+    for (int Q = 0; Q < 4; ++Q) {
+#pragma unroll
+        for (int i = 0; i < 4; ++i) *reinterpret_cast<f32x4*>(in_w + i * F43C5L::PS) = i < nreal ? in[i] : (f32x4){0.f, 0.f, 0.f, 0.f};
+        __syncthreads();
+        if (Q == 0) C5_STAMP(25);
+        if (Q < 3) request(Q + 1);
+        f43c5_transform(t_in, t_v);
+        __syncthreads();
+        if (Q == 0) C5_STAMP(26);
+        if (Q == 3) C5_STAMP(28);
+        __builtin_amdgcn_s_setprio(0);
+#pragma unroll
+        for (int k = 0; k < DV; ++k) Vr[k] = lds_read4(v0 + k * 1024);
+#pragma unroll 1
+        for (int Gq = 0; Gq < 2; ++Gq) {
+            const int G = 2 * Q + Gq, Gn = G == CIN / 16 - 1 ? G : G + 1;
+            unsigned vcur = v0 + Gq * (F43_XI * 1024), vnext = v0 + (1 - Gq) * (F43_XI * 1024);
+            asm("" : "+v"(vcur));
+            asm("" : "+v"(vnext));
+            __builtin_amdgcn_sched_barrier(0);
+#pragma unroll
+            for (int k = 0; k < F43_XI; k += 2) {
+#pragma unroll
+                for (int s4 = 0; s4 < 4; ++s4) {
+                    acc[k] = __builtin_amdgcn_mfma_f32_16x16x4f32(Ur[k % DU][s4], Vr[k % DV][s4], acc[k], 0, 0, 0);
+                    acc[k + 1] = __builtin_amdgcn_mfma_f32_16x16x4f32(Ur[(k + 1) % DU][s4], Vr[(k + 1) % DV][s4], acc[k + 1], 0, 0, 0);
+                }
+#pragma unroll
+                for (int kk = k; kk < k + 2; ++kk) {
+                    const int ku = kk + DU, kv = kk + DV;
+                    Ur[kk % DU] = ku < F43_XI ? wino_load_u<CIN, COUT>(wrsrc, u_lane, ku, G) : wino_load_u<CIN, COUT>(wrsrc, u_lane, ku - F43_XI, Gn);
+                    Vr[kk % DV] = kv < F43_XI ? lds_read4(vcur + kv * 1024) : lds_read4(vnext + (kv - F43_XI) * 1024);
+                }
+                __builtin_amdgcn_sched_barrier(0);
+            }
+        }
+        __builtin_amdgcn_s_setprio(3);
+        if (Q == 0) C5_STAMP(27);
+        if (Q == 3) C5_STAMP(29);
+    }
+
+    __syncthreads();
+    f32x4 y[16];
+    f43c5_output(acc, y);
+    const f32x4 bias = *reinterpret_cast<const f32x4*>(&a.bias[wave * 16 + 4 * (lane >> 4)]);
+    C5_STAMP(30);
+    const int m = lane & 15, op = m >> 2, oy = 4 * ((m >> 1) & 1), ox = 4 * (m & 1);
+    if (op < nreal) {
+        float* dst = slot + op * (64 * COUT) + wave * 16 + 4 * (lane >> 4);
+#pragma unroll
+        for (int k = 0; k < 16; ++k) *reinterpret_cast<f32x4*>(dst + ((oy + (k >> 2)) * 8 + ox + (k & 3)) * COUT) = bias_relu(y[k], bias);
+    }
+    C5_STAMP(31);
+}
+
+int aff_hardnet_conv5_f43(affnet_ctx* ctx, const Conv5Args& a, int groups, int B, bool stamps, hipStream_t st) {
+    if (groups <= 0) return AFFNET_OK;
+    hipLaunchKernelGGL(stamps ? hardnet_conv5_f43_kernel<true> : hardnet_conv5_f43_kernel<false>, dim3(groups, B), dim3(512), 0, st, a);
+    AFF_LAUNCH_CHECK(ctx);
+    return AFFNET_OK;
+}
diff --git a/affnet_amd/csrc/pack_check.cpp b/affnet_amd/csrc/pack_check.cpp
--- a/affnet_amd/csrc/pack_check.cpp
+++ b/affnet_amd/csrc/pack_check.cpp
@@ -92,6 +92,7 @@
 static_assert(Wino16::offset(1) == 0 && Wino16::offset(3) == 4096 && Wino16::offset(5) == 20480 && Wino16::offset(2) == 86016 && Wino16::offset(4) == 98816 && Wino16::FLOATS == 150016 && Wino16::PAIRS == 7936, "Wino16");
 static_assert(Poly32::offset(2) == 0 && Poly32::offset(4) == 51200 && Poly32::FLOATS == 256000 && Poly32::PAIRS == 10240, "Poly32");
 static_assert(F43::BASE == 256000 && F43::offset(1) == 0 && F43::offset(3) == 36864 && F43::FLOATS == 184320 && F43::PAIRS == 5120, "F43");
+static_assert(F43C5::BASE == 440320 && F43C5::FLOATS == 589824 && derived_hardnet_form3().pairs == 15360 + 16384, "F43C5");
 
 static int check_derived(const char* name, int kind, const DerivedTable& t, int want_sections, size_t want_floats) {
     const NetLayout L = net_layout(kind); const NetOffsets off = to_offsets(L);
@@ -130,9 +131,11 @@
 
 static int check_regions() {
     const size_t t16 = derived_trunk16().floats, poly = derived_hardnet_poly().floats, f43 = derived_hardnet_f43().floats;
-    CHECK(DerivedU::AFFNET == 0 && DerivedU::ORINET == t16 && DerivedU::HARDNET == 2 * t16 && DerivedU::HARDNET_F43 == 2 * t16 + poly && DerivedU::FLOATS == 2 * t16 + poly + f43);
+    const size_t c5 = F43C5::FLOATS;
+    CHECK(DerivedU::AFFNET == 0 && DerivedU::ORINET == t16 && DerivedU::HARDNET == 2 * t16 && DerivedU::HARDNET_F43 == 2 * t16 + poly && DerivedU::HARDNET_C5 == 2 * t16 + poly + f43 &&
+          DerivedU::FLOATS == 2 * t16 + poly + f43 + c5);
     CHECK(DerivedU::region(AFFNET_NET_AFFNET) == DerivedU::AFFNET && DerivedU::region(AFFNET_NET_ORINET) == DerivedU::ORINET && DerivedU::region(AFFNET_NET_HARDNET) == DerivedU::HARDNET);
-    CHECK(derived_hardnet_form2().floats == poly + f43);
+    CHECK(derived_hardnet_form2().floats == poly + f43 && derived_hardnet_form3().floats == poly + f43 + c5);
     return 0;
 }
 
@@ -141,7 +144,8 @@
         if (check_kind(kind)) return 1;
     if (check_derived("AffNet", AFFNET_NET_AFFNET, derived_trunk16(), 5, 150016) || check_derived("OriNet", AFFNET_NET_ORINET, derived_trunk16(), 5, 150016) ||
         check_derived("HardNet polyphase", AFFNET_NET_HARDNET, derived_hardnet_poly(), 2, 256000) || check_derived("HardNet F(4x4, 3x3)", AFFNET_NET_HARDNET, derived_hardnet_f43(), 2, 184320) ||
-        check_derived("HardNet form 2", AFFNET_NET_HARDNET, derived_hardnet_form2(), 4, 256000 + 184320) || check_regions())
+        check_derived("HardNet form 2", AFFNET_NET_HARDNET, derived_hardnet_form2(), 4, 256000 + 184320) ||
+        check_derived("HardNet form 3", AFFNET_NET_HARDNET, derived_hardnet_form3(), 5, 256000 + 184320 + 589824) || check_regions())
         return 1;
     return 0;
 }
diff --git a/affnet_amd/csrc/weights_layout.h b/affnet_amd/csrc/weights_layout.h
--- a/affnet_amd/csrc/weights_layout.h
+++ b/affnet_amd/csrc/weights_layout.h
@@ -193,6 +193,7 @@
 constexpr DerivedTable derived_hardnet_poly() { return derived_add(derived_add(DerivedTable{}, 32, 2, DERIVED_POLY), 32, 4, DERIVED_POLY); }
 constexpr DerivedTable derived_hardnet_f43() { return derived_add(derived_add(DerivedTable{}, 32, 1, DERIVED_F43), 32, 3, DERIVED_F43); }
 constexpr DerivedTable derived_hardnet_form2() { return derived_add(derived_add(derived_hardnet_poly(), 32, 1, DERIVED_F43), 32, 3, DERIVED_F43); }
+constexpr DerivedTable derived_hardnet_form3() { return derived_add(derived_hardnet_form2(), 32, 5, DERIVED_F43); }
 constexpr DerivedSection derived_layer(const DerivedTable& t, int layer) {
     for (int i = 0; i < t.n; ++i)
         if (t.s[i].layer == layer) return t.s[i];
@@ -208,7 +209,7 @@
     return i == t.n || (t.s[i].pair0 % 256 == 0 && t.s[i].cin * t.s[i].cout % 256 == 0 && derived_by_workgroups(t, i + 1));
 }
 static_assert(derived_by_workgroups(derived_trunk16()) && derived_by_workgroups(derived_hardnet_poly()) && derived_by_workgroups(derived_hardnet_f43()) &&
-              derived_by_workgroups(derived_hardnet_form2()), "a 256-thread workgroup of derive_u_kernel stays within one section");
+              derived_by_workgroups(derived_hardnet_form2()) && derived_by_workgroups(derived_hardnet_form3()), "a 256-thread workgroup of derive_u_kernel stays within one section");
 
 template <DerivedTable (*T)()>
 struct DerivedView {
@@ -221,18 +222,23 @@
 struct F43 : DerivedView<derived_hardnet_f43> { static constexpr int BASE = Poly32::FLOATS; };
 static_assert(derived_hardnet_form2().s[2].dst == F43::BASE + F43::offset(1) && derived_hardnet_form2().s[3].dst == F43::BASE + F43::offset(3) &&
               derived_hardnet_form2().floats == F43::BASE + F43::FLOATS, "form 2's table = Poly32 with F43 at F43::BASE");
+struct F43C5 {
+    static constexpr int BASE = derived_hardnet_form2().floats, FLOATS = F43_XI * 128 * 128;
+};
+static_assert(derived_hardnet_form3().n == 5 && derived_hardnet_form3().s[4].dst == F43C5::BASE && derived_hardnet_form3().floats == F43C5::BASE + F43C5::FLOATS, "form 3's table = form 2's with conv5 at F43C5::BASE");
 
 struct DerivedU {
     static constexpr int AFFNET = 0, ORINET = AFFNET + Wino16::FLOATS;
     static constexpr int HARDNET = ORINET + Wino16::FLOATS;
     static constexpr int HARDNET_F43 = HARDNET + F43::BASE;
-    static constexpr int FLOATS = HARDNET_F43 + F43::FLOATS;
+    static constexpr int HARDNET_C5 = HARDNET + F43C5::BASE;
+    static constexpr int FLOATS = HARDNET_C5 + F43C5::FLOATS;
     static constexpr int region(int kind) { return kind == AFFNET_NET_AFFNET ? AFFNET : (kind == AFFNET_NET_ORINET ? ORINET : HARDNET); }
 };
 static_assert(DerivedU::AFFNET == 0 && DerivedU::ORINET - DerivedU::AFFNET == derived_trunk16().floats && DerivedU::HARDNET - DerivedU::ORINET == derived_trunk16().floats &&
-              DerivedU::FLOATS - DerivedU::HARDNET == derived_hardnet_form2().floats && DerivedU::FLOATS == 2 * Wino16::FLOATS + Poly32::FLOATS + F43::FLOATS,
+              DerivedU::FLOATS - DerivedU::HARDNET == derived_hardnet_form3().floats && DerivedU::FLOATS == 2 * Wino16::FLOATS + Poly32::FLOATS + F43::FLOATS + F43C5::FLOATS,
               "the regions are disjoint, in this order, and fill the buffer");
-static_assert(DerivedU::ORINET % 64 == 0 && DerivedU::HARDNET % 64 == 0 && DerivedU::HARDNET_F43 % 64 == 0, "every region starts on a 256-byte boundary, as an allocation of its own would");
+static_assert(DerivedU::ORINET % 64 == 0 && DerivedU::HARDNET % 64 == 0 && DerivedU::HARDNET_F43 % 64 == 0 && DerivedU::HARDNET_C5 % 64 == 0, "every region starts on a 256-byte boundary, as an allocation of its own would");
 static_assert(w_tap_index(7, 21, 13, 32, 64) == 7 * 32 * 64 + w_tap_index(0, 21, 13, 32, 64) && w_tap_index(35, 63, 63, 64, 64) == 35 * 64 * 64 + w_tap_index(0, 63, 63, 64, 64),
               "a position is a plane of cin * cout floats");
 AFF_HOST_DEVICE inline void derive_u_pair(const DerivedTable& t, int e, const float* packed, const int (&w_off)[6], float* U) {
diff --git a/affnet_amd/engine.py b/affnet_amd/engine.py
--- a/affnet_amd/engine.py
+++ b/affnet_amd/engine.py
@@ -44,7 +44,7 @@
                                          onepass=onepass, lazy_shape_rows=lazy_shape_rows, arith=arith)
         self.arith = _lib.arith_code(arith)
         self.shape_form = _lib.SHAPE_FORM_WINOGRAD
-        self.desc_form = _lib.DESC_FORM_F43
+        self.desc_form = _lib.DESC_FORM_F43_CONV5
         self.device = device
         self.handle = C.c_void_p()
         idx = device.index if device.index is not None else torch.cuda.current_device()
diff --git a/include/affnet_hip.h b/include/affnet_hip.h
--- a/include/affnet_hip.h
+++ b/include/affnet_hip.h
@@ -77,6 +77,7 @@
 #define AFFNET_DESC_FORM_DIRECT 0
 #define AFFNET_DESC_FORM_POLYPHASE 1
 #define AFFNET_DESC_FORM_F43 2
+#define AFFNET_DESC_FORM_F43_CONV5 3
 int affnet_set_desc_form(affnet_ctx* ctx, int form);
 int affnet_get_desc_form(const affnet_ctx* ctx);
 
diff --git a/include/affnet_hip_probes.h b/include/affnet_hip_probes.h
--- a/include/affnet_hip_probes.h
+++ b/include/affnet_hip_probes.h
@@ -32,6 +32,11 @@
 int affnet_probe_hardnet_f43_forward(affnet_ctx* ctx, const float* d_packed, const float* d_patches, int n, float* d_out, float* d_scratch, void* stream);
 int affnet_probe_hardnet_f43_u(affnet_ctx* ctx, const float* d_packed, int layer, float* d_out, void* stream);
 
+int affnet_probe_hardnet_c5_trunk_layer(affnet_ctx* ctx, const float* d_packed, const float* d_patch, int layer, float* d_out, void* stream);
+int affnet_probe_hardnet_c5_forward(affnet_ctx* ctx, const float* d_packed, const float* d_patches, int n, float* d_out, float* d_scratch, void* stream);
+int affnet_probe_hardnet_c5_layer(affnet_ctx* ctx, const float* d_packed, float* d_slots, int n, void* stream);
+int affnet_probe_hardnet_c5_u(affnet_ctx* ctx, const float* d_packed, float* d_out, void* stream);
+
 #ifdef __cplusplus
 }
 #endif
```
